# meyer-lab/cmtf-pls

Hardware: AMD Instinct MI355X
Metric: nipals_iters_per_sec (higher is better)
Workload: dtype f32

## Files before the change

cmtf_pls_amd/_lib.py:

```python
from __future__ import annotations

import ctypes
import os
from ctypes import c_char_p, c_double, c_int, c_int64, c_size_t, c_uint32, c_uint64, c_void_p

_HERE = os.path.dirname(os.path.abspath(__file__))
LIB_PATH = os.environ.get("CMTFPLS_LIB") or os.path.join(_HERE, "lib", "libcmtfpls.so")

_P = c_void_p

class XcovBlock(ctypes.Structure):
    _fields_ = [("S", _P), ("S2", _P), ("colcnt", _P), ("n_samples", c_double), ("order", c_int), ("A", c_int), ("B", c_int),
                ("n_squarings", c_int), ("Z", _P), ("wA", _P), ("wB", _P), ("info", _P)]


class KfoldState(ctypes.Structure):
    _fields_ = [("I", c_int), ("A", c_int), ("B", c_int), ("M", c_int), ("K", c_int), ("R", c_int)] + [
        (name, _P) for name in ("fold_of", "S", "mean", "Yk", "Gy", "WA", "WB", "Q", "Wa", "Wb", "T", "Gt", "coef", "Rm", "tm",
                                "Tout", "vec", "n_iter", "status", "part")]


class CvCoupledBlock(ctypes.Structure):
    _fields_ = [("X", _P), ("order", c_int), ("A", c_int), ("B", c_int)]


class LooCoupledBlock(ctypes.Structure):
    _fields_ = [("X", _P), ("colsum", _P), ("order", c_int), ("A", c_int), ("B", c_int)]


SIGNATURES = {
    "cmtfpls_xcov_iterate_blocks_f64": (c_int, [ctypes.POINTER(XcovBlock), c_int, c_int, _P, _P, _P, _P, _P, c_int, _P, c_size_t, _P]),
    "cmtfpls_abi_version": (c_int, []),
    "cmtfpls_last_error": (c_char_p, []),
    "cmtfpls_clear_error": (c_int, []),
    "cmtfpls_status_to_host": (c_int, [_P, _P, c_size_t, _P, _P]),
    "cmtfpls_colstats_workspace_bytes": (c_size_t, [c_int64, c_int64]),
    "cmtfpls_colstats_f32": (c_int, [_P, c_int64, c_int64, _P, _P, _P, c_size_t, _P]),
    "cmtfpls_colstats_f64": (c_int, [_P, c_int64, c_int64, _P, _P, _P, c_size_t, _P]),
    "cmtfpls_sweep_partials": (c_int, []),
    "cmtfpls_center_f32": (c_int, [_P, c_int64, c_int64, _P, _P, _P, _P]),
    "cmtfpls_center_f64": (c_int, [_P, c_int64, c_int64, _P, _P, _P, _P]),
    "cmtfpls_mode0_contract_workspace_bytes": (c_size_t, [c_int64, c_int64]),
    "cmtfpls_mode0_contract_f32": (c_int, [_P, c_int64, c_int64, _P, _P, c_int, _P, c_size_t, _P]),
    "cmtfpls_mode0_contract_f64": (c_int, [_P, c_int64, c_int64, _P, _P, c_int, _P, c_size_t, _P]),
    "cmtfpls_mode0_contract_yq_f32": (c_int, [_P, c_int64, c_int64, _P, c_int, c_int, _P, _P, c_int, _P, c_size_t, _P]),
    "cmtfpls_mode0_contract_yq_f64": (c_int, [_P, c_int64, c_int64, _P, c_int, c_int, _P, _P, c_int, _P, c_size_t, _P]),
    "cmtfpls_colscale_f64": (c_int, [_P, c_int64, _P, c_double, _P]),
    "cmtfpls_rank1_workspace_bytes": (c_size_t, [c_int, c_int]),
    "cmtfpls_rank1_score_f64": (c_int, [_P, c_int, c_int, _P, _P, _P, c_int, _P, c_int, _P, _P, c_size_t, _P]),
    "cmtfpls_rank1_f64": (c_int, [_P, c_int, c_int, _P, _P, _P, _P, c_int, _P, c_size_t, _P]),
    "cmtfpls_rank1_launches_f64": (c_int, [_P, c_int, c_int, _P, _P, _P, _P, c_int, _P, c_size_t, _P]),
    "cmtfpls_rank1_chain_enable": (None, [c_int]),
    "cmtfpls_rank1_chain_enabled": (c_int, []),
    "cmtfpls_normalize_f64": (c_int, [_P, c_int64, _P, _P]),
    "cmtfpls_rank1_tensor_workspace_bytes": (c_size_t, [_P, c_int]),
    "cmtfpls_rank1_tensor_f64": (c_int, [_P, _P, c_int, c_double, _P, c_int, _P, c_int, _P, c_size_t, _P]),
    "cmtfpls_kron_f64": (c_int, [_P, c_int, _P, c_int, _P, _P]),
    "cmtfpls_xcov_workspace_bytes": (c_size_t, [c_int64, c_int64, c_int]),
    "cmtfpls_xcov_f32": (c_int, [_P, c_int64, c_int64, _P, c_int, c_int, _P, c_int, _P, c_size_t, _P]),
    "cmtfpls_xcov_f64": (c_int, [_P, c_int64, c_int64, _P, c_int, c_int, _P, c_int, _P, c_size_t, _P]),
    "cmtfpls_xcov_bf16": (c_int, [_P, c_int64, c_int64, _P, c_int, c_int, _P, c_int, _P, c_size_t, _P]),
    "cmtfpls_xcov_f16": (c_int, [_P, c_int64, c_int64, _P, c_int, c_int, _P, c_int, _P, c_size_t, _P]),
    "cmtfpls_quadform_f64": (c_int, [_P, c_int, _P, _P, _P, _P]),
    "cmtfpls_xcov_iterate_f64": (c_int, [_P, c_int, c_int, c_int, _P, _P, _P, _P, _P, c_int, _P, _P, _P, c_int, _P, c_size_t, _P, c_size_t, _P]),
    "cmtfpls_s_downdate_f64": (c_int, [_P, c_int, c_int, c_int, _P, _P, _P, _P, _P, _P]),
    "cmtfpls_project_rows_f32": (c_int, [_P, c_int64, c_int, c_int, c_int, _P, _P, _P, _P, c_int, _P]),
    "cmtfpls_project_rows_f64": (c_int, [_P, c_int64, c_int, c_int, c_int, _P, _P, _P, _P, c_int, _P]),
    "cmtfpls_project_rows2_f32": (c_int, [_P, c_int, c_int, _P, _P, _P, _P, c_int, c_int, _P, _P, _P, c_int64, c_int, _P, c_int, _P]),
    "cmtfpls_project_rows2_f64": (c_int, [_P, c_int, c_int, _P, _P, _P, _P, c_int, c_int, _P, _P, _P, c_int64, c_int, _P, c_int, _P]),
    "cmtfpls_project_rows_idx_f32": (c_int, [_P, _P, c_int64, c_int, c_int, c_int, _P, _P, _P, _P, c_int, _P]),
    "cmtfpls_project_rows_idx_f64": (c_int, [_P, _P, c_int64, c_int, c_int, c_int, _P, _P, _P, _P, c_int, _P]),
    "cmtfpls_project_rows2_idx_f32": (c_int, [_P, c_int, c_int, _P, _P, _P, _P, c_int, c_int, _P, _P, _P, _P, c_int64, c_int, _P, c_int, _P]),
    "cmtfpls_project_rows2_idx_f64": (c_int, [_P, c_int, c_int, _P, _P, _P, _P, c_int, c_int, _P, _P, _P, _P, c_int64, c_int, _P, c_int, _P]),
    "cmtfpls_allreduce_sum_f64": (c_int, [_P, _P, c_size_t, _P]),
    "cmtfpls_allreduce_sum_f32": (c_int, [_P, _P, c_size_t, _P]),
    "cmtfpls_axpy_scalar_f64": (c_int, [_P, c_int64, _P, _P, _P]),
    "cmtfpls_xcov_deflate_f32": (c_int, [_P, c_int64, c_int, c_int, _P, c_int, c_int, _P, _P, _P, _P, _P, _P, c_size_t, _P]),
    "cmtfpls_xcov_deflate_f64": (c_int, [_P, c_int64, c_int, c_int, _P, c_int, c_int, _P, _P, _P, _P, _P, _P, c_size_t, _P]),
    "cmtfpls_xcov_stats_workspace_bytes": (c_size_t, [c_int64, c_int64, c_int]),
    "cmtfpls_xcov_stats_f32": (c_int, [_P, c_int64, c_int64, _P, c_int, c_int, _P, _P, _P, c_size_t, _P]),
    "cmtfpls_xcov_stats_f64": (c_int, [_P, c_int64, c_int64, _P, c_int, c_int, _P, _P, _P, c_size_t, _P]),
    "cmtfpls_xcov_stats_bf16": (c_int, [_P, c_int64, c_int64, _P, c_int, c_int, _P, _P, _P, c_size_t, _P]),
    "cmtfpls_xcov_stats_f16": (c_int, [_P, c_int64, c_int64, _P, c_int, c_int, _P, _P, _P, c_size_t, _P]),
    "cmtfpls_xcov_ssq_workspace_bytes": (c_size_t, [c_int64, c_int64, c_int]),
    "cmtfpls_xcov_ssq_f32": (c_int, [_P, c_int64, c_int64, _P, c_int, c_int, _P, _P, _P, _P, c_size_t, _P]),
    "cmtfpls_xcov_ssq_f64": (c_int, [_P, c_int64, c_int64, _P, c_int, c_int, _P, _P, _P, _P, c_size_t, _P]),
    "cmtfpls_score_contract_workspace_bytes": (c_size_t, [c_int64, c_int64]),
    "cmtfpls_score_contract_f32": (c_int, [_P, c_int64, c_int, c_int, _P, _P, _P, _P, _P, c_double, _P, _P, _P, _P, c_size_t, _P]),
    "cmtfpls_score_contract_f64": (c_int, [_P, c_int64, c_int, c_int, _P, _P, _P, _P, _P, c_double, _P, _P, _P, _P, c_size_t, _P]),
    "cmtfpls_score_contract_bf16": (c_int, [_P, c_int64, c_int, c_int, _P, _P, _P, _P, _P, c_double, _P, _P, _P, _P, c_size_t, _P]),
    "cmtfpls_score_contract_f16": (c_int, [_P, c_int64, c_int, c_int, _P, _P, _P, _P, _P, c_double, _P, _P, _P, _P, c_size_t, _P]),
    "cmtfpls_kr_axpy_f64": (c_int, [_P, c_int, c_int, _P, _P, c_int, c_int, _P, _P]),
    "cmtfpls_xcov_f32_mixed": (c_int, [_P, c_int64, c_int64, _P, c_int, c_int, _P, c_int, _P, c_size_t, _P]),
    "cmtfpls_mttkrp_f32_mixed": (c_int, [_P, c_int64, c_int, c_int, _P, _P, c_int, _P, c_int, _P]),
    "cmtfpls_mttkrp_f32": (c_int, [_P, c_int64, c_int, c_int, _P, _P, c_int, _P, c_int, _P]),
    "cmtfpls_mttkrp_f64": (c_int, [_P, c_int64, c_int, c_int, _P, _P, c_int, _P, c_int, _P]),
    "cmtfpls_mttkrp_bf16": (c_int, [_P, c_int64, c_int, c_int, _P, _P, c_int, _P, c_int, _P]),
    "cmtfpls_mttkrp_f16": (c_int, [_P, c_int64, c_int, c_int, _P, _P, c_int, _P, c_int, _P]),
    "cmtfpls_score_f32": (c_int, [_P, c_int64, c_int, c_int, _P, _P, _P, _P, _P]),
    "cmtfpls_score_f64": (c_int, [_P, c_int64, c_int, c_int, _P, _P, _P, _P, _P]),
    "cmtfpls_score_s_f64": (c_int, [_P, c_int, c_int, c_int, _P, _P, _P, _P]),
    "cmtfpls_deflate_contract_workspace_bytes": (c_size_t, [c_int64, c_int64]),
    "cmtfpls_deflate_contract_yq_f32": (c_int, [_P, c_int64, c_int, c_int, _P, _P, _P, _P, c_int, c_int, _P, _P, c_int, _P, _P, c_size_t, _P]),
    "cmtfpls_deflate_contract_yq_f64": (c_int, [_P, c_int64, c_int, c_int, _P, _P, _P, _P, c_int, c_int, _P, _P, c_int, _P, _P, c_size_t, _P]),
    "cmtfpls_score_gram_f32": (c_int, [_P, c_int64, c_int, c_int, _P, _P, _P, _P, _P, c_int, c_int, _P, _P]),
    "cmtfpls_score_gram_f64": (c_int, [_P, c_int64, c_int, c_int, _P, _P, _P, _P, _P, c_int, c_int, _P, _P]),
    "cmtfpls_q_update_f64": (c_int, [_P, c_int, c_int, _P, c_int, _P, _P, _P, _P]),
    "cmtfpls_deflate_f32": (c_int, [_P, c_int64, c_int, c_int, _P, _P, _P, _P, _P]),
    "cmtfpls_deflate_f64": (c_int, [_P, c_int64, c_int, c_int, _P, _P, _P, _P, _P]),
    "cmtfpls_score_deflate_f32": (c_int, [_P, c_int64, c_int, c_int, _P, _P, _P, _P, _P, _P]),
    "cmtfpls_score_deflate_f64": (c_int, [_P, c_int64, c_int, c_int, _P, _P, _P, _P, _P, _P]),
    "cmtfpls_sweep_form": (c_int, [c_char_p, c_int, c_int64, c_int, c_int, c_int, c_int, c_int, c_char_p, c_size_t]),
    "cmtfpls_sweep_form_list": (c_int, [c_char_p, c_int, c_char_p, c_size_t]),
    "cmtfpls_small_workspace_bytes": (c_size_t, []),
    "cmtfpls_gram_tn_f64": (c_int, [_P, c_int, c_int, _P, c_int, c_int, c_int64, _P, _P, c_size_t, _P]),
    "cmtfpls_rowdot_f64": (c_int, [_P, c_int, c_int, c_int64, _P, _P, _P, _P, _P, c_size_t, _P]),
    "cmtfpls_scores_mean_f64": (c_int, [_P, c_int, c_int64, _P, _P]),
    "cmtfpls_y_deflate_f64": (c_int, [_P, c_int, c_int, c_int64, _P, c_int, c_int, _P, _P, _P, _P, c_size_t, _P]),
    "cmtfpls_sum_f64": (c_int, [_P, c_int64, _P, _P]),
    "cmtfpls_normal_solve_f64": (c_int, [_P, _P, c_int, _P, c_int, _P]),
    "cmtfpls_normal_solve_workspace_bytes": (c_size_t, [c_int]),
    "cmtfpls_normal_solve_ws_f64": (c_int, [_P, _P, c_int, _P, c_int, _P, c_size_t, _P]),
    "cmtfpls_unit_upper_solve_rows_f64": (c_int, [_P, c_int64, c_int, c_int, _P, _P, _P, _P]),
    "cmtfpls_kr_gram_row_f64": (c_int, [_P, c_int, c_int, c_int, _P, c_int, _P]),
    "cmtfpls_kr_gram_f64": (c_int, [_P, c_int, c_int, _P, c_int, c_double, _P]),
    "cmtfpls_khatri_rao_f64": (c_int, [_P, c_int, _P, c_int, c_int, _P, _P]),
    "cmtfpls_predict_rows_f64": (c_int, [_P, c_int64, c_int, c_int, _P, c_int, _P, _P, c_int, _P]),
    "cmtfpls_recon_f32": (c_int, [_P, c_int64, c_int, c_int, _P, _P, c_int, c_int, _P, _P, _P]),
    "cmtfpls_recon_f64": (c_int, [_P, c_int64, c_int, c_int, _P, _P, c_int, c_int, _P, _P, _P]),
    "cmtfpls_recon_r2_workspace_bytes": (c_size_t, [c_int64, c_int64]),
    "cmtfpls_recon_r2_f32": (c_int, [_P, _P, c_int64, c_int, c_int, _P, _P, c_int, c_int, _P, _P, _P, c_size_t, _P]),
    "cmtfpls_recon_r2_f64": (c_int, [_P, _P, c_int64, c_int, c_int, _P, _P, c_int, c_int, _P, _P, _P, c_size_t, _P]),
    "cmtfpls_recon_r2_bf16": (c_int, [_P, _P, c_int64, c_int, c_int, _P, _P, c_int, c_int, _P, _P, _P, c_size_t, _P]),
    "cmtfpls_recon_r2_f16": (c_int, [_P, _P, c_int64, c_int, c_int, _P, _P, c_int, c_int, _P, _P, _P, c_size_t, _P]),
    "cmtfpls_resid_rows_workspace_bytes": (c_size_t, [c_int64, c_int64]),
    "cmtfpls_resid_rows_f32": (c_int, [_P, _P, c_int64, c_int, c_int, _P, _P, c_int, c_int, _P, _P, _P, _P, c_size_t, _P]),
    "cmtfpls_resid_rows_f64": (c_int, [_P, _P, c_int64, c_int, c_int, _P, _P, c_int, c_int, _P, _P, _P, _P, c_size_t, _P]),
    "cmtfpls_resid_rows_bf16": (c_int, [_P, _P, c_int64, c_int, c_int, _P, _P, c_int, c_int, _P, _P, _P, _P, c_size_t, _P]),
    "cmtfpls_resid_rows_f16": (c_int, [_P, _P, c_int64, c_int, c_int, _P, _P, c_int, c_int, _P, _P, _P, _P, c_size_t, _P]),
    "cmtfpls_contrib_rows_f32": (c_int, [_P, c_int64, _P, c_int, _P, c_int, c_int, _P, _P, c_int, c_int, _P, _P, c_int64, _P, _P, _P, _P, _P]),
    "cmtfpls_contrib_rows_f64": (c_int, [_P, c_int64, _P, c_int, _P, c_int, c_int, _P, _P, c_int, c_int, _P, _P, c_int64, _P, _P, _P, _P, _P]),
    "cmtfpls_contrib_rows_bf16": (c_int, [_P, c_int64, _P, c_int, _P, c_int, c_int, _P, _P, c_int, c_int, _P, _P, c_int64, _P, _P, _P, _P, _P]),
    "cmtfpls_contrib_rows_f16": (c_int, [_P, c_int64, _P, c_int, _P, c_int, c_int, _P, _P, c_int, c_int, _P, _P, c_int64, _P, _P, _P, _P, _P]),
    "cmtfpls_selectivity_cols_workspace_bytes": (c_size_t, [c_int64, c_int64, c_int]),
    "cmtfpls_selectivity_cols_f32": (c_int, [_P, c_int64, c_int64, _P, c_int, c_int, _P, c_int, _P, _P, _P, _P, _P, c_size_t, _P]),
    "cmtfpls_selectivity_cols_f64": (c_int, [_P, c_int64, c_int64, _P, c_int, c_int, _P, c_int, _P, _P, _P, _P, _P, c_size_t, _P]),
    "cmtfpls_selectivity_cols_bf16": (c_int, [_P, c_int64, c_int64, _P, c_int, c_int, _P, c_int, _P, _P, _P, _P, _P, c_size_t, _P]),
    "cmtfpls_selectivity_cols_f16": (c_int, [_P, c_int64, c_int64, _P, c_int, c_int, _P, c_int, _P, _P, _P, _P, _P, c_size_t, _P]),
    "cmtfpls_holdout_mask_workspace_bytes": (c_size_t, [c_int64]),
    "cmtfpls_holdout_mask_f32": (c_int, [_P, _P, c_int64, c_double, c_uint64, c_uint32, c_uint64, _P, _P, c_size_t, _P]),
    "cmtfpls_holdout_mask_f64": (c_int, [_P, _P, c_int64, c_double, c_uint64, c_uint32, c_uint64, _P, _P, c_size_t, _P]),
    "cmtfpls_heldout_resid_workspace_bytes": (c_size_t, [c_int64, c_int64, c_int]),
    "cmtfpls_heldout_resid_f32": (c_int, [_P, c_int64, c_int, c_int, _P, c_int, c_int, _P, _P, _P, c_double, c_uint64, c_uint32, c_uint64,
                                          _P, _P, c_size_t, _P]),
    "cmtfpls_heldout_resid_f64": (c_int, [_P, c_int64, c_int, c_int, _P, c_int, c_int, _P, _P, _P, c_double, c_uint64, c_uint32, c_uint64,
                                          _P, _P, c_size_t, _P]),
    "cmtfpls_impute_workspace_bytes": (c_size_t, [c_int64, c_int64]),
    "cmtfpls_impute_f32": (c_int, [_P, _P, c_int64, c_int, c_int, _P, c_int, c_int, _P, _P, _P, _P, _P, c_size_t, _P]),
    "cmtfpls_impute_f64": (c_int, [_P, _P, c_int64, c_int, c_int, _P, c_int, c_int, _P, _P, _P, _P, _P, c_size_t, _P]),
    "cmtfpls_loo_fold_workspace_bytes": (c_size_t, [c_int, c_int, c_int, c_int, c_int]),
    "cmtfpls_loo_tpls_f64": (c_int, [_P, _P, _P, _P, c_int, c_int, c_int, c_int, c_int, c_double, c_int, c_int, c_int, _P, _P, _P, c_size_t, _P]),
    "cmtfpls_loo_xcov_fold_workspace_bytes": (c_size_t, [c_int, c_int, c_int, c_int, c_int]),
    "cmtfpls_kfold_xcov_workspace_bytes": (c_size_t, [c_int64, c_int64, c_int, c_int]),
    "cmtfpls_kfold_xcov_f32": (c_int, [_P, c_int64, c_int, c_int, _P, c_int, _P, _P, c_int, _P, _P, _P, _P, _P, c_size_t, _P]),
    "cmtfpls_kfold_xcov_f64": (c_int, [_P, c_int64, c_int, c_int, _P, c_int, _P, _P, c_int, _P, _P, _P, _P, _P, c_size_t, _P]),
    "cmtfpls_kfold_xcov_bf16": (c_int, [_P, c_int64, c_int, c_int, _P, c_int, _P, _P, c_int, _P, _P, _P, _P, _P, c_size_t, _P]),
    "cmtfpls_kfold_xcov_f16": (c_int, [_P, c_int64, c_int, c_int, _P, c_int, _P, _P, c_int, _P, _P, _P, _P, _P, c_size_t, _P]),
    "cmtfpls_kfold_row_tiles": (c_int, [c_int64]),
    "cmtfpls_kfold_part_stride": (c_int, []),
    "cmtfpls_kfold_inner_workspace_bytes": (c_size_t, [c_int, c_int, c_int]),
    "cmtfpls_kfold_inner_f64": (c_int, [ctypes.POINTER(KfoldState), c_int, c_double, c_int, _P, c_size_t, _P]),
    "cmtfpls_kfold_inner_tensor_workspace_bytes": (c_size_t, [c_int, c_int, c_int, c_int]),
    "cmtfpls_kfold_inner_tensor_lds_bytes": (c_size_t, [c_int, c_int, c_int, c_int]),
    "cmtfpls_kfold_inner_tensor_f64": (c_int, [ctypes.POINTER(KfoldState), _P, c_int, c_int, c_int, c_int, c_double, c_int, _P, _P, _P,
                                       c_size_t, _P]),
    "cmtfpls_kfold_epilogue_f64": (c_int, [ctypes.POINTER(KfoldState), c_int, c_int, _P, _P]),
    "cmtfpls_kfold_inner_coupled_workspace_bytes": (c_size_t, [ctypes.POINTER(KfoldState), c_int]),
    "cmtfpls_kfold_inner_coupled_f64": (c_int, [ctypes.POINTER(KfoldState), c_int, c_int, c_double, c_int, _P, c_size_t, _P]),
    "cmtfpls_kfold_inner_coupled_tensor_workspace_bytes": (c_size_t, [ctypes.POINTER(KfoldState), c_int, ctypes.POINTER(c_int)]),
    "cmtfpls_kfold_inner_coupled_tensor_lds_bytes": (c_size_t, [ctypes.POINTER(KfoldState), c_int, ctypes.POINTER(c_int)]),
    "cmtfpls_kfold_inner_coupled_tensor_f64": (c_int, [ctypes.POINTER(KfoldState), c_int, ctypes.POINTER(c_int), _P, c_int, c_int, c_double,
                                                       c_int, _P, _P, _P, c_size_t, _P]),
    "cmtfpls_kfold_combine_scores_f64": (c_int, [_P, c_int, c_int64, _P, _P]),
    "cmtfpls_kfold_wide_xcov_workspace_bytes": (c_size_t, [c_int64, c_int64, c_int, c_int]),
    "cmtfpls_kfold_wide_xcov_f32": (c_int, [_P, c_int64, c_int, c_int, _P, c_int, _P, _P, c_int, _P, _P, _P, _P, _P, c_size_t, _P]),
    "cmtfpls_kfold_wide_xcov_f64": (c_int, [_P, c_int64, c_int, c_int, _P, c_int, _P, _P, c_int, _P, _P, _P, _P, _P, c_size_t, _P]),
    "cmtfpls_kfold_wide_xcov_bf16": (c_int, [_P, c_int64, c_int, c_int, _P, c_int, _P, _P, c_int, _P, _P, _P, _P, _P, c_size_t, _P]),
    "cmtfpls_kfold_wide_xcov_f16": (c_int, [_P, c_int64, c_int, c_int, _P, c_int, _P, _P, c_int, _P, _P, _P, _P, _P, c_size_t, _P]),
    "cmtfpls_kfold_inner_grouped_f64": (c_int, [ctypes.POINTER(KfoldState), _P, c_int, c_int, c_double, c_int, _P, c_size_t, _P]),
    "cmtfpls_kfold_inner_coupled_grouped_f64": (c_int, [ctypes.POINTER(KfoldState), c_int, _P, c_int, c_int, c_double, c_int, _P, c_size_t,
                                                        _P]),
    "cmtfpls_kfold_epilogue_grouped_f64": (c_int, [ctypes.POINTER(KfoldState), _P, c_int, c_int, c_int, _P, _P]),
    "cmtfpls_kfold_epilogue_splits_f64": (c_int, [ctypes.POINTER(KfoldState), c_int, c_int, c_int, _P, _P]),
    "cmtfpls_kfold_weighted_xcov_workspace_bytes": (c_size_t, [c_int64, c_int64, c_int, c_int]),
    "cmtfpls_kfold_weighted_xcov_f32": (c_int, [_P, c_int64, c_int, c_int, _P, c_int, c_int, _P, _P, _P, _P, c_size_t, _P]),
    "cmtfpls_kfold_weighted_xcov_f64": (c_int, [_P, c_int64, c_int, c_int, _P, c_int, c_int, _P, _P, _P, _P, c_size_t, _P]),
    "cmtfpls_kfold_weighted_xcov_bf16": (c_int, [_P, c_int64, c_int, c_int, _P, c_int, c_int, _P, _P, _P, _P, c_size_t, _P]),
    "cmtfpls_kfold_weighted_xcov_f16": (c_int, [_P, c_int64, c_int, c_int, _P, c_int, c_int, _P, _P, _P, _P, c_size_t, _P]),
    "cmtfpls_kfold_epilogue_weighted_f64": (c_int, [ctypes.POINTER(KfoldState), c_int, c_int, _P, _P]),
    "cmtfpls_press_rows_workspace_bytes": (c_size_t, [c_int, c_int64, c_int, c_int]),
    "cmtfpls_press_rows_f64": (c_int, [_P, _P, _P, _P, _P, _P, c_int, c_int64, c_int, c_int, _P, _P, _P, c_size_t, _P]),
    "cmtfpls_loo_xcov_f64": (c_int, [_P, _P, _P, _P, c_int, c_int, c_int, c_int, c_int, c_double, c_int, c_int, c_int, _P, _P, _P, c_size_t, _P]),
    "cmtfpls_loo_xcov_tensor_fold_workspace_bytes": (c_size_t, [c_int, c_int, c_int, c_int, c_int, c_int]),
    "cmtfpls_loo_xcov_tensor_lds_bytes": (c_size_t, [c_int, c_int, c_int, c_int, c_int]),
    "cmtfpls_loo_xcov_tensor_f64": (c_int, [_P, _P, _P, _P, c_int, c_int, c_int, c_int, c_int, c_int, c_double, c_int, c_int, c_int, _P, _P, _P,
                                            c_size_t, _P]),
    "cmtfpls_loo_xcov_coupled_fold_workspace_bytes": (c_size_t, [ctypes.POINTER(LooCoupledBlock), c_int, c_int, c_int, c_int]),
    "cmtfpls_loo_xcov_coupled_lds_bytes": (c_size_t, [ctypes.POINTER(LooCoupledBlock), c_int, c_int, c_int, c_int]),
    "cmtfpls_loo_xcov_coupled_f64": (c_int, [ctypes.POINTER(LooCoupledBlock), c_int, _P, _P, c_int, c_int, c_int, c_double, c_int, c_int, c_int,
                                             _P, _P, _P, c_size_t, _P]),
    "cmtfpls_loo_xcov_coupled_tensor_fold_workspace_bytes": (c_size_t, [ctypes.POINTER(LooCoupledBlock), c_int, ctypes.POINTER(c_int), c_int,
                                                                       c_int, c_int]),
    "cmtfpls_loo_xcov_coupled_tensor_lds_bytes": (c_size_t, [ctypes.POINTER(LooCoupledBlock), c_int, ctypes.POINTER(c_int), c_int, c_int,
                                                            c_int]),
    "cmtfpls_loo_xcov_coupled_tensor_f64": (c_int, [ctypes.POINTER(LooCoupledBlock), c_int, ctypes.POINTER(c_int), _P, _P, c_int, c_int, c_int,
                                                    c_double, c_int, c_int, c_int, _P, _P, _P, c_size_t, _P]),
    "cmtfpls_cv_masked_fold_workspace_bytes": (c_size_t, [c_int, c_int, c_int, c_int, c_int]),
    "cmtfpls_cv_masked_f64": (c_int, [_P, _P, _P, c_int, _P, _P, _P, c_int, c_int, c_int, c_int, c_int, c_double, c_int, c_int,
                                      c_int, _P, _P, _P, _P, _P, c_size_t, _P]),
    "cmtfpls_cv_masked_model_workspace_bytes": (c_size_t, [c_int, c_int, c_int, c_int, c_int]),
    "cmtfpls_cv_masked_models_f64": (c_int, [_P, _P, _P, _P, c_int, c_int, c_int, c_int, c_int, c_int, c_double, c_int, c_int, c_int]
                                     + [_P] * 8 + [_P, c_size_t, _P]),
    "cmtfpls_cv_masked_tensor_fold_workspace_bytes": (c_size_t, [c_int] * 6),
    "cmtfpls_cv_masked_tensor_lds_bytes": (c_size_t, [c_int] * 6),
    "cmtfpls_cv_masked_tensor_f64": (c_int, [_P, _P, _P, c_int, _P, _P, _P, c_int, c_int, c_int, c_int, c_int, c_int, c_double, c_int,
                                             c_int, c_int, _P, _P, _P, _P, _P, c_size_t, _P]),
    "cmtfpls_cv_masked_tensor_model_workspace_bytes": (c_size_t, [c_int] * 6),
    "cmtfpls_cv_masked_tensor_models_f64": (c_int, [_P, _P, _P, _P, c_int, c_int, c_int, c_int, c_int, c_int, c_int, c_double, c_int,
                                                    c_int, c_int] + [_P] * 9 + [_P, c_size_t, _P]),
    "cmtfpls_cv_masked_coupled_workspace_bytes": (c_size_t, [ctypes.POINTER(CvCoupledBlock), c_int, c_int, c_int, c_int]),
    "cmtfpls_cv_masked_coupled_lds_bytes": (c_size_t, [ctypes.POINTER(CvCoupledBlock), c_int, c_int, c_int, c_int]),
    "cmtfpls_cv_masked_coupled_f64": (c_int, [ctypes.POINTER(CvCoupledBlock), c_int, _P, _P, _P, c_int, c_int, c_int, c_int, c_double,
                                              c_int, c_int, c_int] + [_P] * 8 + [_P, c_size_t, _P]),
    "cmtfpls_cv_masked_coupled_tensor_workspace_bytes": (c_size_t, [ctypes.POINTER(CvCoupledBlock), c_int, _P, c_int, c_int, c_int]),
    "cmtfpls_cv_masked_coupled_tensor_lds_bytes": (c_size_t, [ctypes.POINTER(CvCoupledBlock), c_int, _P, c_int, c_int, c_int]),
    "cmtfpls_cv_masked_coupled_tensor_f64": (c_int, [ctypes.POINTER(CvCoupledBlock), c_int, _P, _P, _P, _P, c_int, c_int, c_int, c_int,
                                                     c_double, c_int, c_int, c_int] + [_P] * 10 + [_P, c_size_t, _P]),
    "cmtfpls_fit_small_workspace_bytes": (c_size_t, [c_int, c_int, c_int, c_int]),
    "cmtfpls_fit_small_f64": (c_int, [_P, _P, c_int, c_int, c_int, c_int, c_int, c_double, c_int] + [_P] * 11 + [_P, c_size_t, _P]),
    "cmtfpls_add_noise_f32": (c_int, [_P, c_int64, c_double, c_uint64, c_uint64, c_double, _P]),
    "cmtfpls_add_noise_f64": (c_int, [_P, c_int64, c_double, c_uint64, c_uint64, c_double, _P]),
    "cmtfpls_ceiling_max_blocks": (c_int, []),
    "cmtfpls_ceiling_read": (c_int, [_P, c_size_t, c_int64, c_int, _P, c_int, _P]),
    "cmtfpls_ceiling_rmw": (c_int, [_P, c_size_t, c_int64, c_int, c_int, _P]),
    "cmtfpls_ceiling_copy": (c_int, [_P, _P, c_size_t, c_int64, c_int, c_int, _P]),
}

_lib = None


class CmtfplsError(RuntimeError):
    pass


def load():
    global _lib
    if _lib is not None:
        return _lib
    if not os.path.exists(LIB_PATH):
        raise CmtfplsError(
            f"{LIB_PATH} not found: build the HIP extension first (python -c 'import __graft_entry__ as g; g.build()'). "
            "cmtf_pls_amd has no CPU fallback."
        )
    lib = ctypes.CDLL(LIB_PATH)
    for name, (res, args) in SIGNATURES.items():
        fn = getattr(lib, name)
        fn.restype = res
        fn.argtypes = args
    _lib = lib
    return lib


# ... 5 lines not shown
```

cmtf_pls_amd/backend.py:

```python
from __future__ import annotations

import ctypes
from typing import Optional, Tuple

import torch

from . import _lib
from .storage import HALF_DTYPES, HALF_ENTRIES, SUFFIX, entry_name

_HALF_ENTRIES = tuple(dict.fromkeys(e for group in HALF_ENTRIES.values() for e in group))


def _ptr(t: Optional[torch.Tensor]):
    return None if t is None else t.data_ptr()


def _int_pairs(pairs):
    flat = [int(v) for p in pairs for v in p]
    return (ctypes.c_int * len(flat))(*flat)


def _scratch(nbytes: int, device) -> torch.Tensor:
    return torch.empty(max(int(nbytes), 256), dtype=torch.uint8, device=device)

# ... 152 lines not shown
              info: Optional[torch.Tensor] = None, n_squarings: Optional[int] = None, launches: bool = False) -> None:
        ws = self._workspace("rank1", self.lib.cmtfpls_rank1_workspace_bytes(A, B))
        fn = self.lib.cmtfpls_rank1_launches_f64 if launches else self.lib.cmtfpls_rank1_f64
        _lib.check(fn(_ptr(Z), A, B, _ptr(wA), _ptr(wB), None, _ptr(info), int(n_squarings or self.rank1_squarings),
                      _ptr(ws), ws.numel(), self._stream()), "rank1")

    def rank1_chain_gave_up(self) -> None:
        self.lib.cmtfpls_rank1_chain_enable(0)
        self.rank1_chain_side = 0

    def rank1_tensor(self, Z: torch.Tensor, dims, tol: float, factors: torch.Tensor,
                     info: Optional[torch.Tensor] = None, n_squarings: Optional[int] = None) -> None:
        arr = (ctypes.c_int * len(dims))(*[int(d) for d in dims])
        ws = self._workspace("rank1t", self.lib.cmtfpls_rank1_tensor_workspace_bytes(arr, len(dims)))
        _lib.check(self.lib.cmtfpls_rank1_tensor_f64(_ptr(Z), arr, len(dims), float(tol), _ptr(factors), factors.stride(0), _ptr(info),
                                                     int(n_squarings or self.rank1_squarings), _ptr(ws), ws.numel(), self._stream()),
                   "rank1_tensor")

    def kron(self, a: torch.Tensor, b: torch.Tensor, out: torch.Tensor) -> torch.Tensor:
        _lib.check(self.lib.cmtfpls_kron_f64(_ptr(a), a.numel(), _ptr(b), b.numel(), _ptr(out), self._stream()), "kron")
        return out

    def normalize(self, v: torch.Tensor) -> None:
        _lib.check(self.lib.cmtfpls_normalize_f64(_ptr(v), v.numel(), None, self._stream()), "normalize")

    def xcov(self, X2: torch.Tensor, Y: torch.Tensor, masked: bool, out: Optional[torch.Tensor] = None,
             mixed: bool = False) -> Optional[torch.Tensor]:
        I, P = X2.shape
        M = Y.shape[1]
        fn = self._read_fn("xcov", X2, mixed)
        if fn is None:
            return None
        ws = self._workspace("contract", self.lib.cmtfpls_xcov_workspace_bytes(I, P, M))
        S = out if out is not None else self.empty(M, P)
        _lib.check(fn(_ptr(X2), I, P, _ptr(Y), Y.stride(0), M, _ptr(S), int(masked), _ptr(ws), ws.numel(), self._stream()), "xcov")
        return S

    def xcov_deflate(self, X2: torch.Tensor, A: int, B: int, Y: torch.Tensor, t: torch.Tensor, wA: torch.Tensor, wB: torch.Tensor,
                     out: torch.Tensor) -> Optional[torch.Tensor]:
        I, P = X2.shape
        M = Y.shape[1]
        if M > 64 or P % 4 != 0 or P != A * B:
            return None
        ws = self._workspace("contract", self.lib.cmtfpls_xcov_ssq_workspace_bytes(I, P, M))
        ssq = self.empty(1)
        rc = self._fn("xcov_deflate", X2)(_ptr(X2), I, A, B, _ptr(Y), Y.stride(0), M, _ptr(t), _ptr(wA), _ptr(wB), _ptr(out), _ptr(ssq),
                                          _ptr(ws), ws.numel(), self._stream())
        return self._form(rc, "xcov_deflate", ssq)

    def rank1_score(self, Z: torch.Tensor, A: int, B: int, wA: torch.Tensor, wB: torch.Tensor, S: torch.Tensor, tq: torch.Tensor,
                    info: Optional[torch.Tensor] = None, n_squarings: Optional[int] = None) -> torch.Tensor:
        M = S.shape[0]
        assert S.is_contiguous() and S.shape[1] == A * B and tq.numel() >= M
        ws = self._workspace("rank1", self.lib.cmtfpls_rank1_workspace_bytes(A, B))
        _lib.check(self.lib.cmtfpls_rank1_score_f64(_ptr(Z), A, B, _ptr(wA), _ptr(wB), _ptr(info),
                                                    int(n_squarings if n_squarings is not None else self.rank1_squarings),
                                                    _ptr(S), M, _ptr(tq), _ptr(ws), ws.numel(), self._stream()), "rank1_score")
        return tq

    def xcov_ssq(self, X2: torch.Tensor, Y: torch.Tensor, mean: torch.Tensor, out: torch.Tensor):
        I, P = X2.shape
        M = Y.shape[1]
        ws = self._workspace("contract", self.lib.cmtfpls_xcov_ssq_workspace_bytes(I, P, M))
        ssq = self.empty(1)
        assert mean.is_contiguous() and mean.numel() == P and mean.dtype == torch.float64
        _lib.check(self._fn("xcov_ssq", X2)(_ptr(X2), I, P, _ptr(Y), Y.stride(0), M, _ptr(out), _ptr(mean), _ptr(ssq), _ptr(ws), ws.numel(),
                                            self._stream()), "xcov_ssq")
        return out, ssq

    def xcov_stats(self, X2: torch.Tensor, Y: torch.Tensor, out: torch.Tensor):
        I, P = X2.shape
        M = Y.shape[1]
        fn = self._read_fn("xcov_stats", X2) if M <= 64 and X2.is_contiguous() else None
        if fn is None:
            return None
        ws = self._workspace("contract", self.lib.cmtfpls_xcov_stats_workspace_bytes(I, P, M))
        stats = self.empty(2 * P)
        rc = fn(_ptr(X2), I, P, _ptr(Y), Y.stride(0), M, _ptr(out), _ptr(stats), _ptr(ws), ws.numel(), self._stream())
        return self._form(rc, "xcov_stats", (out, stats))

    def status_snapshot(self, status: torch.Tensor, slot: int, slots: Optional[dict] = None):
        slots = self._status_slots if slots is None else slots
        ent = slots.get((slot, status.numel()))
        if ent is None:
            host, ev = torch.empty(status.numel(), dtype=torch.float64, pin_memory=True), torch.cuda.Event()
            ev.record(torch.cuda.current_stream(self.device))
            ent = slots[(slot, status.numel())] = (host, ev, host.numpy(), host.data_ptr(), ev.cuda_event, status.numel() * 8)
        rc = self.lib.cmtfpls_status_to_host(status.data_ptr(), ent[3], ent[5], ent[4], self._stream())
        if rc:
            _lib.check(rc, "status_to_host")
        return ent

    def status_wait(self, token) -> "np.ndarray":
        token[1].synchronize()
        return token[2]

    def xcov_iterate_plan(self, S: torch.Tensor, A: int, B: int, q_cur: torch.Tensor, Z: torch.Tensor, wA: torch.Tensor,
                          wB: torch.Tensor, status: torch.Tensor, q_new: torch.Tensor, G: torch.Tensor):
        M, P = S.shape
        wc = self._workspace("contract", self.lib.cmtfpls_mode0_contract_workspace_bytes(M, P))
        wr = self._workspace("rank1", self.lib.cmtfpls_rank1_workspace_bytes(A, B))
        keep = (S, q_cur, Z, wA, wB, status, q_new, G, wc, wr)
        fn = self.lib.cmtfpls_xcov_iterate_f64
        head = (_ptr(S), M, A, B, _ptr(q_cur), _ptr(Z), _ptr(wA), _ptr(wB), status[1:3].data_ptr())
        tail = (_ptr(wc), wc.numel(), _ptr(wr), wr.numel())
        qn, Gp, du2 = _ptr(q_new), _ptr(G), status[0:1].data_ptr()
        stream = self._stream

        def enqueue(n_squarings: int, first: bool, _keep=keep) -> None:
            rc = fn(*head, n_squarings, qn, Gp, du2, 1 if first else 0, *tail, stream())
            if rc:
                _lib.check(rc, "xcov_iterate")
        return enqueue

    def xcov_iterate(self, S: torch.Tensor, A: int, B: int, q_cur: torch.Tensor, Z: torch.Tensor, wA: torch.Tensor,
                     wB: torch.Tensor, info: torch.Tensor, n_squarings: int, q_new: torch.Tensor, G: torch.Tensor,
                     du2: torch.Tensor, first: bool) -> None:
        M, P = S.shape
        wc = self._workspace("contract", self.lib.cmtfpls_mode0_contract_workspace_bytes(M, P))
        wr = self._workspace("rank1", self.lib.cmtfpls_rank1_workspace_bytes(A, B))
        _lib.check(self.lib.cmtfpls_xcov_iterate_f64(_ptr(S), M, A, B, _ptr(q_cur), _ptr(Z), _ptr(wA), _ptr(wB), _ptr(info),
                                                     int(n_squarings), _ptr(q_new), _ptr(G), _ptr(du2), int(first),
                                                     _ptr(wc), wc.numel(), _ptr(wr), wr.numel(), self._stream()), "xcov_iterate")

    def xcov_blocks_plan(self, blocks, M: int, q_cur: torch.Tensor, tq: torch.Tensor, q_new: torch.Tensor, G: torch.Tensor,
                         status: torch.Tensor):
        nb = len(blocks)
        if M > 64 or any(b["order"] not in (2, 3) for b in blocks) or tq.numel() != nb * M or not tq.is_contiguous():
            return None
        arr = (_lib.XcovBlock * nb)()
        need = 256
        for i, b in enumerate(blocks):
            for name in ("S", "S2", "colcnt", "Z", "wA", "wB"):
                t = b.get(name)
                assert t is None or (t.is_contiguous() and t.dtype == torch.float64 and t.device == self.device), name
                setattr(arr[i], name, _ptr(t))
            arr[i].n_samples, arr[i].order, arr[i].A, arr[i].B = float(b["n_samples"]), int(b["order"]), int(b["A"]), int(b["B"])
            arr[i].info = status[1 + 2 * i: 3 + 2 * i].data_ptr()
            if b["order"] == 3:
                need = max(need, self.lib.cmtfpls_rank1_workspace_bytes(b["A"], b["B"]))
        wr = self._workspace("rank1", need)
        keep = (blocks, q_cur, tq, q_new, G, status, wr, arr)
        fn, stream = self.lib.cmtfpls_xcov_iterate_blocks_f64, self._stream
        args = (nb, M, _ptr(q_cur), _ptr(tq), _ptr(q_new), _ptr(G), status[0:1].data_ptr())
        tail = (_ptr(wr), wr.numel())

        def enqueue(n_squarings, first: bool, _keep=keep) -> None:
            for i in range(nb):
                arr[i].n_squarings = int(n_squarings[i])
            rc = fn(arr, *args, 1 if first else 0, *tail, stream())
            if rc:
                _lib.check(rc, "xcov_iterate_blocks")
        return enqueue

    def s_downdate(self, S: torch.Tensor, A: int, B: int, ya: torch.Tensor, wA: torch.Tensor, wB: torch.Tensor,
                   q: torch.Tensor, v: torch.Tensor) -> None:
        assert S.is_contiguous() and S.shape[1] == A * B
        _lib.check(self.lib.cmtfpls_s_downdate_f64(_ptr(S), S.shape[0], A, B, _ptr(ya), _ptr(wA), _ptr(wB), _ptr(q), _ptr(v),
                                                   self._stream()), "s_downdate")

    def kr_axpy(self, v: torch.Tensor, A: int, B: int, WA: torch.Tensor, WB: torch.Tensor, k: int, coef: torch.Tensor) -> torch.Tensor:
        assert WA.is_contiguous() and WB.is_contiguous() and WA.shape[1] == WB.shape[1] and coef.numel() >= k
        _lib.check(self.lib.cmtfpls_kr_axpy_f64(_ptr(v), A, B, _ptr(WA), _ptr(WB), WA.shape[1], int(k), _ptr(coef), self._stream()), "kr_axpy")
        return v

    def axpy_scalar(self, y: torch.Tensor, a: torch.Tensor, x: Optional[torch.Tensor] = None) -> torch.Tensor:
        assert y.is_contiguous() and y.dtype == torch.float64 and a.numel() >= 1 and (x is None or (x.is_contiguous() and x.numel() == y.numel()))
        _lib.check(self.lib.cmtfpls_axpy_scalar_f64(_ptr(y), y.numel(), _ptr(a), _ptr(x), self._stream()), "axpy_scalar")
        return y

    def total(self, v: torch.Tensor) -> torch.Tensor:
        assert v.is_contiguous() and v.dtype == torch.float64
        return self._close_partials(v)

    def quadform(self, G: torch.Tensor, q: torch.Tensor, q_old: torch.Tensor, out: torch.Tensor) -> torch.Tensor:
        _lib.check(self.lib.cmtfpls_quadform_f64(_ptr(G), G.shape[0], _ptr(q), _ptr(q_old), _ptr(out), self._stream()), "quadform")
        return out

    def mttkrp(self, X2: torch.Tensor, A: int, B: int, WA: torch.Tensor, WB: torch.Tensor, out: torch.Tensor,
               mixed: bool = False) -> Optional[torch.Tensor]:
        R = WA.shape[1]
        assert WA.is_contiguous() and WB.is_contiguous() and out.stride(1) == 1
        fn = self._read_fn("mttkrp", X2, mixed)
        if fn is None:
            return None
        rc = fn(_ptr(X2), X2.shape[0], A, B, _ptr(WA), _ptr(WB), R, _ptr(out), out.stride(0), self._stream())
        return self._form(rc, "mttkrp", out)

    def score(self, X2, A, B, wA, wB, rowcnt, out) -> torch.Tensor:
        _lib.check(self._fn("score", X2)(_ptr(X2), X2.shape[0], A, B, _ptr(wA), _ptr(wB), _ptr(rowcnt), _ptr(out), self._stream()), "score")
        return out

    def score_s(self, S, A, B, wA, wB, out) -> torch.Tensor:
        assert S.dtype == torch.float64 and S.is_contiguous()
        _lib.check(self.lib.cmtfpls_score_s_f64(_ptr(S), S.shape[0], A, B, _ptr(wA), _ptr(wB), _ptr(out), self._stream()), "score_s")
        return out

    def score_contract(self, X2, A, B, wA, wB, shift, t, Z, sub_own=None, add_other=None, alpha: float = 1.0,
                       csum: Optional[torch.Tensor] = None) -> Optional[torch.Tensor]:
        I, P = X2.shape
        fn = self._read_fn("score_contract", X2) if X2.is_contiguous() and P == A * B else None
        if fn is None:
            return None
        for v in (sub_own, add_other):
            assert v is None or (v.is_contiguous() and v.numel() == I and v.dtype == torch.float64)
        nbytes = self.lib.cmtfpls_score_contract_workspace_bytes(I, P)
        ws = self._workspace("score_contract", max(nbytes, 256))
        rc = fn(_ptr(X2), I, A, B, _ptr(wA), _ptr(wB), _ptr(shift), _ptr(sub_own), _ptr(add_other), float(alpha),
                                            _ptr(t), _ptr(Z), _ptr(csum), _ptr(ws), ws.numel(), self._stream())
        return self._form(rc, "score_contract", Z)

    def score_gram(self, X2, A, B, wA, wB, rowcnt, out, Y: torch.Tensor, qpart: torch.Tensor) -> Optional[torch.Tensor]:
        assert qpart.numel() >= self.n_partials * Y.shape[1] and qpart.is_contiguous()
        rc = self._fn("score_gram", X2)(_ptr(X2), X2.shape[0], A, B, _ptr(wA), _ptr(wB), _ptr(rowcnt), _ptr(out),
                                        _ptr(Y), Y.stride(0), Y.shape[1], _ptr(qpart), self._stream())
        return self._form(rc, "score_gram", out)

    def q_update(self, q: torch.Tensor, qpart: Optional[torch.Tensor] = None, normalize: bool = True,
                 G: Optional[torch.Tensor] = None, q_prev: Optional[torch.Tensor] = None,
                 du2: Optional[torch.Tensor] = None, nparts: Optional[int] = None) -> None:
        M = q.numel()
        nrows = (nparts or self.n_partials) if qpart is not None else 0
        assert qpart is None or (qpart.is_contiguous() and qpart.numel() >= nrows * M)
        _lib.check(self.lib.cmtfpls_q_update_f64(_ptr(qpart), nrows, M, _ptr(q), int(normalize),
                                                 _ptr(G), _ptr(q_prev), _ptr(du2), self._stream()), "q_update")

    def deflate(self, X2, A, B, t, wA, wB) -> torch.Tensor:
        part = self.empty(self.n_partials)
        _lib.check(self._fn("deflate", X2)(_ptr(X2), X2.shape[0], A, B, _ptr(t), _ptr(wA), _ptr(wB), _ptr(part), self._stream()), "deflate")
        return self._close_partials(part)

    def deflate_contract_yq(self, X2, A, B, t, wA, wB, Y: torch.Tensor, q: torch.Tensor, masked: bool,
                            out: torch.Tensor) -> Optional[torch.Tensor]:
        I, P = X2.shape
        ws = self._workspace("deflate_contract", self.lib.cmtfpls_deflate_contract_workspace_bytes(I, P))
        ssq = self.empty(1)
        rc = self._fn("deflate_contract_yq", X2)(_ptr(X2), I, A, B, _ptr(t), _ptr(wA), _ptr(wB), _ptr(Y), Y.stride(0), Y.shape[1],
                                                 _ptr(q), _ptr(out), int(masked), _ptr(ssq), _ptr(ws), ws.numel(), self._stream())
        return self._form(rc, "deflate_contract_yq", ssq)

    def score_deflate(self, X2, A, B, wA, wB, rowcnt, out) -> Optional[torch.Tensor]:
        part = self.empty(self.n_partials)
        rc = self._fn("score_deflate", X2)(_ptr(X2), X2.shape[0], A, B, _ptr(wA), _ptr(wB), _ptr(rowcnt), _ptr(out), _ptr(part), self._stream())
        if self._form(rc, "score_deflate") is None:
            return None
        return self._close_partials(part)

    def gram_tn(self, A: torch.Tensor, B: torch.Tensor, out: Optional[torch.Tensor] = None) -> torch.Tensor:
        if A.dim() == 1:
            A = A.unsqueeze(1)
        if B.dim() == 1:
            B = B.unsqueeze(1)
        assert A.stride(1) == 1 and B.stride(1) == 1 and A.shape[0] == B.shape[0]
        a, b = A.shape[1], B.shape[1]
        ws = self._workspace("small", self.lib.cmtfpls_small_workspace_bytes())
        C = out if out is not None else self.empty(a, b)
        assert C.numel() == a * b and C.is_contiguous()
        _lib.check(self.lib.cmtfpls_gram_tn_f64(_ptr(A), A.stride(0), a, _ptr(B), B.stride(0), b, A.shape[0], _ptr(C),
                                                _ptr(ws), ws.numel(), self._stream()), "gram_tn")
        return C

    def rowdot(self, Y: torch.Tensor, q: torch.Tensor, u_out: torch.Tensor, u_old: Optional[torch.Tensor],
               du2: Optional[torch.Tensor] = None) -> Optional[torch.Tensor]:
        ws = self._workspace("small", self.lib.cmtfpls_small_workspace_bytes())
        if u_old is not None and du2 is None:
            du2 = self.empty(1)
        _lib.check(self.lib.cmtfpls_rowdot_f64(_ptr(Y), Y.stride(0), Y.shape[1], Y.shape[0], _ptr(q), _ptr(u_out), _ptr(u_old),
                                               _ptr(du2) if u_old is not None else None,
                                               _ptr(ws), ws.numel(), self._stream()), "rowdot")
        return du2 if u_old is not None else None

    def normal_solve(self, G: torch.Tensor, g: torch.Tensor, out: Optional[torch.Tensor] = None) -> torch.Tensor:
        k = G.shape[0]
        assert G.is_contiguous() and G.shape == (k, k) and g.numel() == k
        b = out if out is not None else self.empty(k)
        if k <= 64:
            _lib.check(self.lib.cmtfpls_normal_solve_f64(_ptr(G), _ptr(g), k, _ptr(b), 1, self._stream()), "normal_solve")
        else:
            ws = self._workspace("normal_solve", self.lib.cmtfpls_normal_solve_workspace_bytes(k))
            _lib.check(self.lib.cmtfpls_normal_solve_ws_f64(_ptr(G), _ptr(g), k, _ptr(b), 1, _ptr(ws), ws.numel(), self._stream()),
                       "normal_solve")
        return b

    def unit_upper_solve_rows(self, M: torch.Tensor, U: torch.Tensor, shift: Optional[torch.Tensor] = None,
                              nan_flag: Optional[torch.Tensor] = None) -> torch.Tensor:
        I, R = M.shape
        assert M.stride(1) == 1 and U.is_contiguous() and U.shape == (R, R)
        assert shift is None or (shift.is_contiguous() and shift.numel() == R and shift.dtype == torch.float64)
        assert nan_flag is None or nan_flag.dtype == torch.int32
        _lib.check(self.lib.cmtfpls_unit_upper_solve_rows_f64(_ptr(M), I, M.stride(0), R, _ptr(U), _ptr(shift), _ptr(nan_flag),
                                                              self._stream()), "unit_upper_solve_rows")
        return M

    def kr_gram_row(self, L: torch.Tensor, a: int, g: torch.Tensor, first: bool) -> torch.Tensor:
        assert L.is_contiguous() and g.is_contiguous() and g.numel() >= a
        _lib.check(self.lib.cmtfpls_kr_gram_row_f64(_ptr(L), L.shape[0], L.shape[1], int(a), _ptr(g), int(first), self._stream()), "kr_gram_row")
        return g

    def kr_gram(self, L: torch.Tensor, G: torch.Tensor, first: bool) -> torch.Tensor:
        n, R = L.shape
        assert L.is_contiguous() and G.is_contiguous() and G.numel() == R * R
        _lib.check(self.lib.cmtfpls_kr_gram_f64(_ptr(L), n, R, _ptr(G), int(first), 1.0, self._stream()), "kr_gram")
        return G

    def khatri_rao(self, Am: torch.Tensor, Bm: torch.Tensor) -> torch.Tensor:
        na, R = Am.shape
# ... 489 lines not shown
```

cmtf_pls_amd/csrc/small.hip:

```cpp
#include "common.hpp"

namespace cmtfpls {

void launch_reduce_rows(const double* part, int nrows, int64_t P, double* out, hipStream_t st);

constexpr int kSmallBlocks = 128;
constexpr int kMaxGramDim = 64;
constexpr size_t kSmallWsBytes = (size_t)kSmallBlocks * kMaxGramDim * kMaxGramDim * sizeof(double);

__global__ __launch_bounds__(256) void gram_tn_kernel(const double* __restrict__ A, int lda, int a,
                                                     const double* __restrict__ B, int ldb, int b,
                                                     int64_t I, double* __restrict__ part, int TR) {
  extern __shared__ double lds[];
  double* As = lds;
  double* Bs = lds + TR * a;
  const int ab = a * b;
  const int64_t rows_per = (I + gridDim.x - 1) / gridDim.x;
  const int64_t r0 = (int64_t)blockIdx.x * rows_per;
  const int64_t r1 = (r0 + rows_per < I) ? r0 + rows_per : I;
  double acc[16];
#pragma unroll
  for (int s = 0; s < 16; ++s) acc[s] = 0.0;
  for (int64_t rb = r0; rb < r1; rb += TR) {
    const int nr = (int)((r1 - rb < TR) ? r1 - rb : TR);
    if (lda == a) {
      for (int idx = threadIdx.x; idx < nr * a; idx += 256) As[idx] = A[rb * a + idx];
    } else {
      for (int idx = threadIdx.x; idx < nr * a; idx += 256) As[idx] = A[(rb + idx / a) * lda + idx % a];
    }
    if (ldb == b) {
      for (int idx = threadIdx.x; idx < nr * b; idx += 256) Bs[idx] = B[rb * b + idx];
    } else {
      for (int idx = threadIdx.x; idx < nr * b; idx += 256) Bs[idx] = B[(rb + idx / b) * ldb + idx % b];
    }
    __syncthreads();
#pragma unroll
    for (int s = 0; s < 16; ++s) {
      const int o = threadIdx.x + s * 256;
      if (o < ab) {
        const int p = o / b, q = o % b;
        double v = acc[s];
        for (int r = 0; r < nr; ++r) v = fma(As[r * a + p], Bs[r * b + q], v);
        acc[s] = v;
      }
    }
    __syncthreads();
  }
#pragma unroll
  for (int s = 0; s < 16; ++s) {
    const int o = threadIdx.x + s * 256;
    if (o < ab) part[(int64_t)blockIdx.x * ab + o] = acc[s];
  }
}

__global__ __launch_bounds__(256) void reduce_block_kernel(const double* __restrict__ part, int nblk, int ac, int bc,
                                                          double* __restrict__ C, int ldc) {
  const int o = blockIdx.x * 4 + (threadIdx.x >> 6);
  const int lane = threadIdx.x & 63;
  if (o >= ac * bc) return;
  double s = 0.0;
  for (int r = lane; r < nblk; r += 64) s += part[(int64_t)r * ac * bc + o];
  s = wave_sum(s);
  if (lane == 0) C[(int64_t)(o / bc) * ldc + (o % bc)] = s;
}

__global__ __launch_bounds__(256) void gemv_t_kernel(const double* __restrict__ A, int lda, int a0, int ac,
                                                    const double* __restrict__ v, int ldv, int64_t I,
                                                    double* __restrict__ part, int a_total) {
  __shared__ double red[4][16];
  double acc[16];
#pragma unroll
  for (int e = 0; e < 16; ++e) acc[e] = 0.0;
  for (int64_t i = (int64_t)blockIdx.x * 256 + threadIdx.x; i < I; i += (int64_t)gridDim.x * 256) {
    const double vi = v[i * ldv];
    const double* ar = A + i * lda + a0;
#pragma unroll
    for (int e = 0; e < 16; ++e)
      if (e < ac) acc[e] = fma(ar[e], vi, acc[e]);
  }
  const int lane = threadIdx.x & 63, wv = threadIdx.x >> 6;
#pragma unroll
  for (int e = 0; e < 16; ++e) {
    const double w = wave_sum(acc[e]);
    if (lane == 0) red[wv][e] = w;
  }
  __syncthreads();
  if (threadIdx.x < ac) {
    const int e = threadIdx.x;
    part[(int64_t)blockIdx.x * a_total + a0 + e] = ((red[0][e] + red[1][e]) + red[2][e]) + red[3][e];
  }
}

__global__ __launch_bounds__(256) void rowdot_kernel(const double* __restrict__ Y, int ldy, int M, int64_t I,
                                                    const double* __restrict__ q, double* __restrict__ u,
                                                    const double* __restrict__ u_old, double* __restrict__ part) {
  __shared__ double red[16];
  double d2 = 0.0;
  for (int64_t i = (int64_t)blockIdx.x * 256 + threadIdx.x; i < I; i += (int64_t)gridDim.x * 256) {
    const double* yr = Y + i * ldy;
    double s = 0.0;
    for (int m = 0; m < M; ++m) s = fma(yr[m], q[m], s);
    if (u_old) { const double d = u_old[i] - s; d2 = fma(d, d, d2); }
    u[i] = s;
  }
  if (part) {
    const double s = block_sum(d2, red);
    if (threadIdx.x == 0) part[blockIdx.x] = s;
  }
}

__global__ __launch_bounds__(256) void y_deflate_kernel(double* __restrict__ Y, int ldy, int M, int64_t I,
                                                       const double* __restrict__ T, int ldt, int R,
                                                       const double* __restrict__ b, const double* __restrict__ q,
                                                       double* __restrict__ part) {
  __shared__ double red[16];
  double ssq = 0.0;
  for (int64_t i = (int64_t)blockIdx.x * 256 + threadIdx.x; i < I; i += (int64_t)gridDim.x * 256) {
    double s = 0.0;
    for (int r = 0; r < R; ++r) s = fma(T[i * ldt + r], b[r], s);
    double* yr = Y + i * ldy;
    for (int m = 0; m < M; ++m) {
      const double v = yr[m] - s * q[m];
      yr[m] = v;
      ssq = fma(v, v, ssq);
    }
  }
  const double s = block_sum(ssq, red);
  if (threadIdx.x == 0) part[blockIdx.x] = s;
}

__global__ __launch_bounds__(1024) void sum_kernel(const double* __restrict__ in, int64_t n, double* __restrict__ out) {
  __shared__ double red[16];
  double s = 0.0;
  for (int64_t i = threadIdx.x; i < n; i += 1024) s += in[i];
  s = block_sum(s, red);
  if (threadIdx.x == 0) out[0] = s;
}

__global__ __launch_bounds__(1024) void normalize_kernel(double* __restrict__ v, int64_t n, double* __restrict__ nrm) {
  __shared__ double red[16];
  double s = 0.0;
  for (int64_t i = threadIdx.x; i < n; i += 1024) s = fma(v[i], v[i], s);
  s = sqrt(block_sum(s, red));
  for (int64_t i = threadIdx.x; i < n; i += 1024) v[i] = v[i] / s;
  if (nrm && threadIdx.x == 0) nrm[0] = s;
}

__global__ __launch_bounds__(1024) void normalize_to_kernel(const double* __restrict__ in, double* __restrict__ out, int64_t n) {
  __shared__ double red[16];
  double s = 0.0;
  for (int64_t i = threadIdx.x; i < n; i += 1024) s = fma(in[i], in[i], s);
  s = sqrt(block_sum(s, red));
  for (int64_t i = threadIdx.x; i < n; i += 1024) out[i] = in[i] / s;
}

__global__ __launch_bounds__(1024) void s_vector_block_kernel(const double* __restrict__ S, const double* __restrict__ S2,
                                                            const double* __restrict__ colcnt, double n_samples, int M, int P,
                                                            const double* __restrict__ q, double* __restrict__ Z,
                                                            double* __restrict__ wB, double* __restrict__ tq) {
  extern __shared__ double wl[];
  __shared__ double red[16];
  const int lane = threadIdx.x & 63, wv = threadIdx.x >> 6;
  double ssq = 0.0;
  for (int c = threadIdx.x; c < P; c += 1024) {
    double z = 0.0;
#pragma unroll 8
    for (int m = 0; m < M; ++m) z = fma(q[m], S[(int64_t)m * P + c], z);
    if (colcnt) z = (colcnt[c] > 0.0) ? z / colcnt[c] * n_samples : 0.0;
    Z[c] = z;
    wl[c] = z;
    ssq = fma(z, z, ssq);
  }
  const double nrm = sqrt(block_sum(ssq, red));
  for (int c = threadIdx.x; c < P; c += 1024) {
    const double w = wl[c] / nrm;
    wl[c] = w;
    wB[c] = w;
  }
  __syncthreads();
  for (int m = wv; m < M; m += 16) {
    double acc = 0.0;
    for (int c = lane; c < P; c += 64) acc = fma(S2[(int64_t)m * P + c], wl[c], acc);
    acc = wave_sum(acc);
    if (lane == 0) tq[m] = acc;
  }
}

__global__ __launch_bounds__(1024) void q_update_kernel(const double* __restrict__ qpart, int nblk, int M,
                                                       double* __restrict__ q, int normalize,
                                                       const double* __restrict__ G, const double* __restrict__ q_prev,
                                                       double* __restrict__ du2) {
  __shared__ double part[64][17];
  __shared__ double qs[64];
  __shared__ double dq[64];
  __shared__ double red[16];
  const int tid = threadIdx.x, lane = tid & 63;
  const int Mp = (M <= 16) ? 16 : (M <= 32) ? 32 : 64;
  const int ngrp = 1024 / Mp;
  const int m = tid & (Mp - 1), grp = tid / Mp;
  double* pflat = &part[0][0];
  if (qpart) {
    double sacc = 0.0;
    const int msafe = (m < M) ? m : 0;
    for (int b0 = grp; b0 < nblk; b0 += 16 * ngrp) {
      double v[16];
#pragma unroll
      for (int k = 0; k < 16; ++k) {
        const int b = b0 + k * ngrp;
        v[k] = qpart[(int64_t)((b < nblk) ? b : nblk - 1) * M + msafe];
      }
#pragma unroll
      for (int k = 0; k < 16; ++k) sacc += (b0 + k * ngrp < nblk) ? v[k] : 0.0;
    }
    if (m >= M) sacc = 0.0;
    pflat[grp * (Mp + 1) + m] = sacc;
    __syncthreads();
    if (tid < M) {
      double tot = 0.0;
      for (int g = 0; g < ngrp; ++g) tot += pflat[g * (Mp + 1) + tid];
      qs[tid] = tot;
    }
  } else if (tid < M) {
    qs[tid] = q[tid];
  }
  __syncthreads();
  if (tid < 64) {
    double v = (lane < M) ? qs[lane] : 0.0;
    if (normalize) {
      const double nrm = sqrt(wave_sum(v * v));
      v = v / nrm;
    }
    if (lane < M) {
      q[lane] = v;
      if (G) dq[lane] = v - q_prev[lane];
    }
  }
  if (G) {
    __syncthreads();
    double sacc = 0.0;
    for (int idx = tid; idx < M * M; idx += 1024) {
      const int i = idx / M, j = idx - i * M;
      sacc = fma(dq[i] * G[idx], dq[j], sacc);
    }
    sacc = block_sum(sacc, red);
    if (tid == 0) du2[0] = sacc;
  }
}

__global__ __launch_bounds__(256) void s_downdate_kernel(double* __restrict__ S, int M, int64_t P, int B,
                                                        const double* __restrict__ ya, const double* __restrict__ wA,
                                                        const double* __restrict__ wB, const double* __restrict__ q,
                                                        const double* __restrict__ v) {
  const int64_t c = (int64_t)blockIdx.x * 256 + threadIdx.x;
  if (c >= P) return;
  const double w = wA[c / B] * wB[c % B];
  const double vc = v[c];
  for (int m = 0; m < M; ++m) {
    double sv = S[(int64_t)m * P + c];
    sv = fma(-ya[m], w, sv);
    sv = fma(-q[m], vc, sv);
    S[(int64_t)m * P + c] = sv;
  }
}

__global__ __launch_bounds__(256) void s_contract_kernel(const double* __restrict__ S, int M, int64_t P, const double* __restrict__ q,
                                                        double* __restrict__ Z) {
  const int64_t c = (int64_t)blockIdx.x * 256 + threadIdx.x;
  if (c >= P) return;
  double acc = 0.0;
#pragma unroll 8
  for (int m = 0; m < M; ++m) acc = fma(q[m], S[(int64_t)m * P + c], acc);
  Z[c] = acc;
}

__global__ __launch_bounds__(256) void axpy_scalar_kernel(double* __restrict__ y, int64_t n, const double* __restrict__ a,
                                                         const double* __restrict__ x) {
  const double av = a[0];
  for (int64_t i = (int64_t)blockIdx.x * 256 + threadIdx.x; i < n; i += (int64_t)gridDim.x * 256) y[i] = fma(-av, x ? x[i] : 1.0, y[i]);
}

__global__ __launch_bounds__(256) void kr_axpy_kernel(double* __restrict__ v, int64_t P, int B, const double* __restrict__ WA,
                                                     const double* __restrict__ WB, int ld, int k, const double* __restrict__ coef) {
  __shared__ double cs[64];
  for (int j = threadIdx.x; j < k; j += 256) cs[j] = coef[j];
  __syncthreads();
  const int64_t c = (int64_t)blockIdx.x * 256 + threadIdx.x;
  if (c >= P) return;
  const double* __restrict__ wa = WA + (c / B) * ld;
  const double* __restrict__ wb = WB + (c % B) * ld;
  double s = 0.0;
  for (int j = 0; j < k; ++j) s = fma(cs[j] * wa[j], wb[j], s);
  v[c] -= s;
}

__global__ __launch_bounds__(256) void colscale_kernel(double* __restrict__ Z, int64_t P, const double* __restrict__ cnt, double n_samples) {
  const int64_t c = (int64_t)blockIdx.x * 256 + threadIdx.x;
  if (c < P) Z[c] = (cnt[c] > 0.0) ? Z[c] / cnt[c] * n_samples : 0.0;
}

__global__ __launch_bounds__(256) void scores_mean_kernel(const double* __restrict__ Ts, int nb, int64_t I, double* __restrict__ out) {
  const int64_t i = (int64_t)blockIdx.x * 256 + threadIdx.x;
  if (i >= I) return;
  double s = Ts[i];
  for (int b = 1; b < nb; ++b) s += Ts[(int64_t)b * I + i];
  out[i] = s / (double)nb;
}

}

using namespace cmtfpls;

extern "C" {

size_t cmtfpls_small_workspace_bytes(void) { return kSmallWsBytes; }

int cmtfpls_gram_tn_f64(const double* A, int lda, int a, const double* B, int ldb, int b, int64_t I,
                        double* C, void* ws, size_t ws_bytes, void* stream) {
  if (!A || !B || !C || a <= 0 || b <= 0 || lda < a || ldb < b || I <= 0) {
    set_error("gram_tn: bad argument");
    return CMTFPLS_EINVAL;
  }
  if (!ws || ws_bytes < kSmallWsBytes) { set_error("gram_tn: workspace too small"); return CMTFPLS_EWORKSPACE; }
  hipStream_t st = (hipStream_t)stream;
  double* part = static_cast<double*>(ws);
  if (b == 1 && (size_t)kSmallBlocks * a * sizeof(double) <= kSmallWsBytes) {
    for (int a0 = 0; a0 < a; a0 += 16) {
      const int ac = (a - a0 < 16) ? a - a0 : 16;
      hipLaunchKernelGGL(gemv_t_kernel, dim3(kSmallBlocks), dim3(256), 0, st, A, lda, a0, ac, B, ldb, I, part, a);
    }
    hipLaunchKernelGGL(reduce_block_kernel, dim3((a + 3) / 4), dim3(256), 0, st, part, kSmallBlocks, a, 1, C, 1);
    return check_launch("gram_tn");
  }
  for (int a0 = 0; a0 < a; a0 += kMaxGramDim)
    for (int b0 = 0; b0 < b; b0 += kMaxGramDim) {
      const int ac = (a - a0 < kMaxGramDim) ? a - a0 : kMaxGramDim;
      const int bc = (b - b0 < kMaxGramDim) ? b - b0 : kMaxGramDim;
      const int tr = (ac + bc <= 32) ? 128 : (ac + bc <= 64) ? 64 : 32;
      const size_t lds = (size_t)tr * (ac + bc) * sizeof(double);
      hipLaunchKernelGGL(gram_tn_kernel, dim3(kSmallBlocks), dim3(256), lds, st, A + a0, lda, ac, B + b0, ldb, bc, I, part, tr);
      hipLaunchKernelGGL(reduce_block_kernel, dim3((ac * bc + 3) / 4), dim3(256), 0, st, part, kSmallBlocks, ac, bc,
                         C + (size_t)a0 * b + b0, b);
    }
  return check_launch("gram_tn");
}

int cmtfpls_rowdot_f64(const double* Y, int ldy, int M, int64_t I, const double* q, double* u,
                       const double* u_old, double* du2, void* ws, size_t ws_bytes, void* stream) {
  if (!Y || !q || !u || M <= 0 || ldy < M || I <= 0 || (u_old && !du2)) { set_error("rowdot: bad argument"); return CMTFPLS_EINVAL; }
  if (u_old && (!ws || ws_bytes < kSmallBlocks * sizeof(double))) { set_error("rowdot: workspace too small"); return CMTFPLS_EWORKSPACE; }
  hipStream_t st = (hipStream_t)stream;
  double* part = u_old ? static_cast<double*>(ws) : nullptr;
  hipLaunchKernelGGL(rowdot_kernel, dim3(kSmallBlocks), dim3(256), 0, st, Y, ldy, M, I, q, u, u_old, part);
  if (u_old) hipLaunchKernelGGL(sum_kernel, dim3(1), dim3(1024), 0, st, part, (int64_t)kSmallBlocks, du2);
  return check_launch("rowdot");
}

int cmtfpls_y_deflate_f64(double* Y, int ldy, int M, int64_t I, const double* T, int ldt, int R,
                          const double* b, const double* q, double* ssq, void* ws, size_t ws_bytes, void* stream) {
  if (!Y || !T || !b || !q || !ssq || M <= 0 || ldy < M || R <= 0 || ldt < R || I <= 0) { set_error("y_deflate: bad argument"); return CMTFPLS_EINVAL; }
  if (!ws || ws_bytes < kSmallBlocks * sizeof(double)) { set_error("y_deflate: workspace too small"); return CMTFPLS_EWORKSPACE; }
  hipStream_t st = (hipStream_t)stream;
  double* part = static_cast<double*>(ws);
  hipLaunchKernelGGL(y_deflate_kernel, dim3(kSmallBlocks), dim3(256), 0, st, Y, ldy, M, I, T, ldt, R, b, q, part);
  hipLaunchKernelGGL(sum_kernel, dim3(1), dim3(1024), 0, st, part, (int64_t)kSmallBlocks, ssq);
  return check_launch("y_deflate");
}

int cmtfpls_sum_f64(const double* in, int64_t n, double* out, void* stream) {
  if (!in || !out || n <= 0) { set_error("sum: bad argument"); return CMTFPLS_EINVAL; }
  hipLaunchKernelGGL(sum_kernel, dim3(1), dim3(1024), 0, (hipStream_t)stream, in, n, out);
  return check_launch("sum");
}

int cmtfpls_normalize_f64(double* v, int64_t n, double* nrm, void* stream) {
  if (!v || n <= 0) { set_error("normalize: bad argument"); return CMTFPLS_EINVAL; }
  hipLaunchKernelGGL(normalize_kernel, dim3(1), dim3(1024), 0, (hipStream_t)stream, v, n, nrm);
  return check_launch("normalize");
}

int cmtfpls_q_update_f64(const double* qpart, int nblk, int M, double* q, int normalize, const double* G, const double* q_prev,
                         double* du2, void* stream) {
  if (!q || M <= 0 || (qpart && nblk <= 0) || (G && (!q_prev || !du2))) { set_error("q_update: bad argument"); return CMTFPLS_EINVAL; }
  if (M > 64) { set_error("q_update: more than 64 responses; use gram_tn + normalize + rowdot"); return CMTFPLS_EUNSUPPORTED; }
  hipLaunchKernelGGL(q_update_kernel, dim3(1), dim3(1024), 0, (hipStream_t)stream, qpart, nblk, M, q, normalize, G, q_prev, du2);
  return check_launch("q_update");
}

int cmtfpls_s_downdate_f64(double* S, int M, int A, int B, const double* ya, const double* wA, const double* wB,
                           const double* q, const double* v, void* stream) {
  if (!S || !ya || !wA || !wB || !q || !v || M <= 0 || A <= 0 || B <= 0) { set_error("s_downdate: bad argument"); return CMTFPLS_EINVAL; }
  const int64_t P = (int64_t)A * B;
  hipLaunchKernelGGL(s_downdate_kernel, dim3((unsigned)((P + 255) / 256)), dim3(256), 0, (hipStream_t)stream, S, M, P, B, ya, wA, wB, q, v);
  return check_launch("s_downdate");
}

int cmtfpls_axpy_scalar_f64(double* y, int64_t n, const double* a, const double* x, void* stream) {
  if (!y || !a || n <= 0) { set_error("axpy_scalar: bad argument"); return CMTFPLS_EINVAL; }
  int64_t blocks = (n + 255) / 256;
  if (blocks > 1024) blocks = 1024;
  hipLaunchKernelGGL(axpy_scalar_kernel, dim3((unsigned)blocks), dim3(256), 0, (hipStream_t)stream, y, n, a, x);
  return check_launch("axpy_scalar");
}

int cmtfpls_kr_axpy_f64(double* v, int A, int B, const double* WA, const double* WB, int ld, int k, const double* coef, void* stream) {
  if (!v || !WA || !WB || !coef || A <= 0 || B <= 0 || k < 0 || ld < k) { set_error("kr_axpy: bad argument"); return CMTFPLS_EINVAL; }
  if (k > 64) { set_error("kr_axpy: more than 64 terms"); return CMTFPLS_EUNSUPPORTED; }
  if (k == 0) return CMTFPLS_OK;
  const int64_t P = (int64_t)A * B;
  hipLaunchKernelGGL(kr_axpy_kernel, dim3((unsigned)((P + 255) / 256)), dim3(256), 0, (hipStream_t)stream, v, P, B, WA, WB, ld, k, coef);
  return check_launch("kr_axpy");
}

int cmtfpls_xcov_iterate_f64(const double* S, int M, int A, int B, const double* q_cur, double* Z, double* wA, double* wB,
                             double* info, int n_squarings, double* q_new, const double* G, double* du2, int first,
                             void* ws_contract, size_t ws_contract_bytes, void* ws_rank1, size_t ws_rank1_bytes, void* stream) {
  if (!S || !q_cur || !Z || !wA || !wB || !q_new || !G || !du2 || M <= 0 || A <= 0 || B <= 0) {
    set_error("xcov_iterate: bad argument");
    return CMTFPLS_EINVAL;
  }
  if (M > 64) { set_error("xcov_iterate: more than 64 responses"); return CMTFPLS_EUNSUPPORTED; }
  const int64_t P = (int64_t)A * B;
  int rc = CMTFPLS_OK;
  if (first) {
    hipLaunchKernelGGL(s_contract_kernel, dim3((unsigned)((P + 255) / 256)), dim3(256), 0, (hipStream_t)stream, S, M, P, q_cur, Z);
    rc = check_launch("xcov_iterate: s_contract");
  }
  if (rc == CMTFPLS_OK) rc = cmtfpls_rank1_score_f64(Z, A, B, wA, wB, info, n_squarings, S, M, q_new, ws_rank1, ws_rank1_bytes, stream);
  if (rc == CMTFPLS_OK) rc = cmtfpls_q_update_f64(nullptr, 0, M, q_new, 1, G, q_cur, du2, stream);
  return rc;
}

int cmtfpls_xcov_iterate_blocks_f64(const cmtfpls_xcov_block* blocks, int nb, int M, const double* q_cur, double* tq, double* q_new,
                                    const double* G, double* du2, int first, void* ws_rank1, size_t ws_rank1_bytes, void* stream) {
  if (!blocks || nb <= 0 || !q_cur || !tq || !q_new || !G || !du2 || M <= 0) { set_error("xcov_iterate_blocks: bad argument"); return CMTFPLS_EINVAL; }
  if (M > 64) { set_error("xcov_iterate_blocks: more than 64 responses"); return CMTFPLS_EUNSUPPORTED; }
  hipStream_t st = (hipStream_t)stream;
  int rc = CMTFPLS_OK;
  for (int b = 0; b < nb && rc == CMTFPLS_OK; ++b) {
    const cmtfpls_xcov_block& k = blocks[b];
    if (!k.S || !k.Z || !k.wA || !k.wB || k.A <= 0 || k.B <= 0 || (k.order != 2 && k.order != 3) || (k.order == 2 && k.A != 1) ||
        (k.order == 3 && !k.info)) {
      set_error("xcov_iterate_blocks: bad block");
      return CMTFPLS_EINVAL;
    }
    const int64_t P = (int64_t)k.A * k.B;
// ... 40 lines not shown
```

cmtf_pls_amd/csrc/solve.hip:

```cpp
#include "common.hpp"

namespace cmtfpls {

constexpr int kSolveMax = 64;

__global__ __launch_bounds__(kSolveMax) void normal_solve_kernel(const double* __restrict__ G, const double* __restrict__ g, int k,
                                                                double* __restrict__ b, int incb) {
  __shared__ double A[kSolveMax][kSolveMax + 1];
  __shared__ double d[kSolveMax], y[kSolveMax];
  __shared__ int dep[kSolveMax];
  const int i = threadIdx.x;
  if (i < k) {
    const double gii = G[(int64_t)i * k + i];
    d[i] = (gii > 0.0 && isfinite(gii)) ? 1.0 / sqrt(gii) : 0.0;
    dep[i] = 0;
  }
  __syncthreads();
  if (i < k) {
    for (int j = 0; j < k; ++j) A[i][j] = G[(int64_t)i * k + j] * d[i] * d[j];
    y[i] = g[i] * d[i];
  }
  __syncthreads();
  const double tiny = (double)k * 2.220446049250313e-16;
  for (int c = 0; c < k; ++c) {
    const double piv = A[c][c];
    const bool ok = piv > tiny;
    __syncthreads();
    if (ok) {
      const double l = sqrt(piv);
      if (i == c) A[c][c] = l;
      if (i > c && i < k) A[i][c] = A[i][c] / l;
    } else {
      if (i == c) { A[c][c] = 1.0; dep[c] = 1; }
      if (i > c && i < k) A[i][c] = 0.0;
    }
    __syncthreads();
    if (ok && i > c && i < k) {
      const double lic = A[i][c];
      for (int j = c + 1; j <= i; ++j) A[i][j] -= lic * A[j][c];
    }
    __syncthreads();
  }
  if (i == 0) {
    for (int r = 0; r < k; ++r) {
      double s = y[r];
      for (int j = 0; j < r; ++j) s -= A[r][j] * y[j];
      y[r] = dep[r] ? 0.0 : s / A[r][r];
    }
    for (int r = k - 1; r >= 0; --r) {
      double s = y[r];
      for (int j = r + 1; j < k; ++j) s -= A[j][r] * y[j];
      y[r] = dep[r] ? 0.0 : s / A[r][r];
    }
  }
  __syncthreads();
  if (i < k) b[(int64_t)i * incb] = y[i] * d[i];
}

constexpr int kSolveBigMax = 1024;
__global__ __launch_bounds__(256) void normal_solve_big_kernel(const double* __restrict__ G, const double* __restrict__ g, int k,
                                                               double* __restrict__ b, int incb, double* __restrict__ Aw) {
  const int ld = k + 1;
  double* d = Aw + (size_t)k * ld;
  double* y = d + k;
  double* depf = y + k;
  __shared__ double s_piv;
  const int t = threadIdx.x;
  for (int i = t; i < k; i += 256) {
    const double gii = G[(int64_t)i * k + i];
    d[i] = (gii > 0.0 && isfinite(gii)) ? 1.0 / sqrt(gii) : 0.0;
    depf[i] = 0.0;
  }
  __syncthreads();
  for (int i = t; i < k; i += 256) {
    for (int j = 0; j < k; ++j) Aw[(size_t)i * ld + j] = G[(int64_t)i * k + j] * d[i] * d[j];
    y[i] = g[i] * d[i];
  }
  __syncthreads();
  const double tiny = (double)k * 2.220446049250313e-16;
  for (int c = 0; c < k; ++c) {
    if (t == 0) s_piv = Aw[(size_t)c * ld + c];
    __syncthreads();
    const double piv = s_piv;
    const bool ok = piv > tiny;
    const double l = ok ? sqrt(piv) : 1.0;
    for (int i = c + t; i < k; i += 256) {
      if (i == c) { Aw[(size_t)c * ld + c] = l; if (!ok) depf[c] = 1.0; }
      else Aw[(size_t)i * ld + c] = ok ? Aw[(size_t)i * ld + c] / l : 0.0;
    }
    __syncthreads();
    if (ok)
      for (int i = c + 1 + t; i < k; i += 256) {
        const double lic = Aw[(size_t)i * ld + c];
        for (int j = c + 1; j <= i; ++j) Aw[(size_t)i * ld + j] -= lic * Aw[(size_t)j * ld + c];
      }
    __syncthreads();
  }
  for (int r = 0; r < k; ++r) {
    if (t == 0) y[r] = (depf[r] != 0.0) ? 0.0 : y[r] / Aw[(size_t)r * ld + r];
    __syncthreads();
    const double yr = y[r];
    for (int j = r + 1 + t; j < k; j += 256) y[j] -= Aw[(size_t)j * ld + r] * yr;
    __syncthreads();
  }
  for (int r = k - 1; r >= 0; --r) {
    if (t == 0) y[r] = (depf[r] != 0.0) ? 0.0 : y[r] / Aw[(size_t)r * ld + r];
    __syncthreads();
    const double yr = y[r];
    for (int j = t; j < r; j += 256) y[j] -= Aw[(size_t)r * ld + j] * yr;
    __syncthreads();
  }
  for (int i = t; i < k; i += 256) b[(int64_t)i * incb] = y[i] * d[i];
}

__global__ __launch_bounds__(256) void unit_upper_solve_rows_kernel(double* __restrict__ Mx, int64_t I, int ld, int R,
                                                                   const double* __restrict__ U, const double* __restrict__ shift,
                                                                   int* __restrict__ nan_flag) {
  __shared__ double Us[kSolveMax * kSolveMax];
  __shared__ double sh[kSolveMax];
  for (int idx = threadIdx.x; idx < R * R; idx += 256) Us[idx] = U[idx];
  for (int idx = threadIdx.x; idx < R; idx += 256) sh[idx] = shift ? shift[idx] : 0.0;
  __syncthreads();
  const int64_t i = (int64_t)blockIdx.x * 256 + threadIdx.x;
  if (i >= I) return;
  double* row = Mx + i * ld;
  bool bad = false;
#pragma unroll 1
  for (int a = 0; a < R; ++a) {
    double s = row[a];
    bad |= (s != s);
    s -= sh[a];
    for (int j = 0; j < a; ++j) s -= row[j] * Us[j * R + a];
    row[a] = s;
  }
  if (bad && nan_flag) *nan_flag = 1;
}

__global__ __launch_bounds__(256) void kr_gram_kernel(const double* __restrict__ L, int n, int R, double* __restrict__ G,
                                                     int first, double scale) {
  for (int o = threadIdx.x; o < R * R; o += 256) {
    const int r = o / R, s = o % R;
    double acc = 0.0;
    for (int j = 0; j < n; ++j) acc = fma(L[(int64_t)j * R + r], L[(int64_t)j * R + s], acc);
    G[o] = (first ? 1.0 : G[o]) * scale * acc;
  }
}

__global__ __launch_bounds__(256) void kr_gram_row_kernel(const double* __restrict__ L, int n, int R, int a, double* __restrict__ g, int first) {
  for (int j = threadIdx.x; j < a; j += 256) {
    double acc = 0.0;
    int i = 0;
    for (; i + 16 <= n; i += 16) {
      double x[16], y[16];
#pragma unroll
      for (int u = 0; u < 16; ++u) {
        x[u] = L[(int64_t)(i + u) * R + j];
        y[u] = L[(int64_t)(i + u) * R + a];
      }
#pragma unroll
      for (int u = 0; u < 16; ++u) acc = fma(x[u], y[u], acc);
    }
    for (; i < n; ++i) acc = fma(L[(int64_t)i * R + j], L[(int64_t)i * R + a], acc);
    g[j] = (first ? 1.0 : g[j]) * acc;
  }
}

__global__ __launch_bounds__(256) void khatri_rao_kernel(const double* __restrict__ Am, int na, const double* __restrict__ Bm, int nb,
                                                        int R, double* __restrict__ out) {
  const int64_t idx = (int64_t)blockIdx.x * 256 + threadIdx.x;
  const int64_t tot = (int64_t)na * nb * R;
  if (idx >= tot) return;
  const int r = (int)(idx % R);
  const int64_t jk = idx / R;
  out[idx] = Am[(jk / nb) * R + r] * Bm[(jk % nb) * R + r];
}

__global__ __launch_bounds__(256) void predict_rows_kernel(const double* __restrict__ S, int lds_, int R, const double* __restrict__ Bm,
                                                          const double* __restrict__ mean, double* __restrict__ out, int ldo, int64_t I, int M) {
  extern __shared__ double sb[];
  for (int idx = threadIdx.x; idx < R * M; idx += 256) sb[idx] = Bm[idx];
  for (int idx = threadIdx.x; idx < M; idx += 256) sb[R * M + idx] = mean ? mean[idx] : 0.0;
  __syncthreads();
  const int64_t o = (int64_t)blockIdx.x * 256 + threadIdx.x;
  if (o >= I * M) return;
  const int64_t i = o / M;
  const int m = (int)(o % M);
  double acc = 0.0;
  for (int a = 0; a < R; ++a) acc = fma(S[i * lds_ + a], sb[a * M + m], acc);
  out[i * ldo + m] = acc + sb[R * M + m];
}

}

using namespace cmtfpls;

extern "C" {

int cmtfpls_normal_solve_f64(const double* G, const double* g, int k, double* b, int incb, void* stream) {
  if (!G || !g || !b || k <= 0 || incb <= 0) { set_error("normal_solve: bad argument"); return CMTFPLS_EINVAL; }
  if (k > kSolveMax) { set_error("normal_solve: more than 64 components; use cmtfpls_normal_solve_ws_f64"); return CMTFPLS_EUNSUPPORTED; }
  hipLaunchKernelGGL(normal_solve_kernel, dim3(1), dim3(kSolveMax), 0, (hipStream_t)stream, G, g, k, b, incb);
  return check_launch("normal_solve");
}

size_t cmtfpls_normal_solve_workspace_bytes(int k) {
  if (k <= kSolveMax || k > kSolveBigMax) return 0;
  return ((size_t)k * (k + 1) + 3 * (size_t)k) * sizeof(double);
}

int cmtfpls_normal_solve_ws_f64(const double* G, const double* g, int k, double* b, int incb, void* ws, size_t ws_bytes, void* stream) {
  if (k <= kSolveMax) return cmtfpls_normal_solve_f64(G, g, k, b, incb, stream);
  if (!G || !g || !b || incb <= 0) { set_error("normal_solve: bad argument"); return CMTFPLS_EINVAL; }
  if (k > kSolveBigMax) { set_error("normal_solve: more than 1024 components"); return CMTFPLS_EUNSUPPORTED; }
  if (!ws || ws_bytes < cmtfpls_normal_solve_workspace_bytes(k)) { set_error("normal_solve: workspace too small"); return CMTFPLS_EWORKSPACE; }
  hipLaunchKernelGGL(normal_solve_big_kernel, dim3(1), dim3(256), 0, (hipStream_t)stream, G, g, k, b, incb, static_cast<double*>(ws));
  return check_launch("normal_solve");
}

int cmtfpls_unit_upper_solve_rows_f64(double* Mx, int64_t I, int ld, int R, const double* U, const double* shift, int* nan_flag,
                                      void* stream) {
  if (!Mx || !U || I <= 0 || R <= 0 || ld < R) { set_error("unit_upper_solve_rows: bad argument"); return CMTFPLS_EINVAL; }
  if (R > kSolveMax) { set_error("unit_upper_solve_rows: more than 64 components"); return CMTFPLS_EUNSUPPORTED; }
  hipLaunchKernelGGL(unit_upper_solve_rows_kernel, dim3((unsigned)((I + 255) / 256)), dim3(256), 0, (hipStream_t)stream, Mx, I, ld, R, U,
                     shift, nan_flag);
  return check_launch("unit_upper_solve_rows");
}

int cmtfpls_kr_gram_f64(const double* L, int n, int R, double* G, int first, double scale, void* stream) {
  if (!L || !G || n <= 0 || R <= 0) { set_error("kr_gram: bad argument"); return CMTFPLS_EINVAL; }
  hipLaunchKernelGGL(kr_gram_kernel, dim3(1), dim3(256), 0, (hipStream_t)stream, L, n, R, G, first, scale);
  return check_launch("kr_gram");
}

int cmtfpls_kr_gram_row_f64(const double* L, int n, int R, int a, double* g, int first, void* stream) {
  if (!L || !g || n <= 0 || R <= 0 || a < 0 || a >= R) { set_error("kr_gram_row: bad argument"); return CMTFPLS_EINVAL; }
  if (a == 0) return CMTFPLS_OK;
  hipLaunchKernelGGL(kr_gram_row_kernel, dim3(1), dim3(256), 0, (hipStream_t)stream, L, n, R, a, g, first);
  return check_launch("kr_gram_row");
}

int cmtfpls_predict_rows_f64(const double* S, int64_t I, int lds_, int R, const double* Bm, int M, const double* mean, double* out, int ldo,
                             void* stream) {
  if (!S || !Bm || !out || I <= 0 || R <= 0 || M <= 0 || lds_ < R || ldo < M) { set_error("predict_rows: bad argument"); return CMTFPLS_EINVAL; }
  const size_t lds_bytes = ((size_t)R * M + M) * sizeof(double);
  if (lds_bytes > 64 * 1024) { set_error("predict_rows: coef_ Q^T does not fit the LDS"); return CMTFPLS_EUNSUPPORTED; }
  const int64_t tot = I * M;
  hipLaunchKernelGGL(predict_rows_kernel, dim3((unsigned)((tot + 255) / 256)), dim3(256), lds_bytes, (hipStream_t)stream, S, lds_, R, Bm, mean,
                     out, ldo, I, M);
  return check_launch("predict_rows");
}

int cmtfpls_khatri_rao_f64(const double* Am, int na, const double* Bm, int nb, int R, double* out, void* stream) {
  if (!Am || !Bm || !out || na <= 0 || nb <= 0 || R <= 0) { set_error("khatri_rao: bad argument"); return CMTFPLS_EINVAL; }
  const int64_t tot = (int64_t)na * nb * R;
  hipLaunchKernelGGL(khatri_rao_kernel, dim3((unsigned)((tot + 255) / 256)), dim3(256), 0, (hipStream_t)stream, Am, na, Bm, nb, R, out);
  return check_launch("khatri_rao");
}

}
```

cmtf_pls_amd/fitrun.py:

```python
from __future__ import annotations

import math
from typing import Dict, List, Optional

import numpy as np
import torch

from .fitrun_xcov import XcovMixin
from .state import BlockState, FitState, split_trailing, validate_limits
from .storage import HALF_DTYPES, HALF_ENTRIES, dtype_name, fallback_text, half_route


class FitRun(XcovMixin):

    def __init__(self, eng: NipalsEngine, Xs: List[torch.Tensor], Y: torch.Tensor, n_components: int, coupled: bool,
                 algorithm: str = "direct", owned: Optional[List[bool]] = None, allow_raw: bool = True):
        be, comm = eng.be, eng.comm
        Xs = list(Xs)
        owned = [True] * len(Xs) if owned is None else list(owned)
        if algorithm not in ("direct", "xcov"):
            raise ValueError("algorithm must be 'direct' or 'xcov'")
        self.algorithm_requested = self.algorithm = algorithm
        self.notes: List[str] = []
        validate_limits([tuple(X.shape) for X in Xs], n_components)
# ... 118 lines not shown
        self._z_ready = False
        self._fused = (algorithm == "direct" and M <= 64
                       and all(hasattr(be, f) for f in ("mode0_contract_yq", "score_gram", "q_update")))
        if self._fused:
            self.Gy = be.empty(M, M)
            self.qbuf = [be.zeros(M), be.zeros(M)]
            self.qpart = be.empty(len(self.blocks), int(be.n_partials) * M)
        elif algorithm == "direct" and comm.sharded:
            self.Gy = be.empty(M, M)
            self.q_prev = be.zeros(M)
        if algorithm == "xcov":
            nb = len(self.blocks)
            self._s_pair = 2 * M <= 64 and eng.opt.xcov_pair_build
            self.S, self.S2, self.S12 = [], [], []
            for blk in self.blocks:
                if blk.has_miss and self._s_pair:
                    both = be.empty(2 * M, blk.A * blk.B)
                    self.S12.append(both)
                    self.S.append(both[:M])
                    self.S2.append(both[M:])
                else:
                    self.S12.append(None)
                    pre = self._s_prebuilt.get(len(self.S))
                    self.S.append(pre if pre is not None else be.empty(M, blk.A * blk.B))
                    self.S2.append(be.empty(M, blk.A * blk.B) if blk.has_miss else None)
            self.rowscale = [(float(blk.A * blk.B) / blk.rowcnt) if blk.has_miss else None for blk in self.blocks]
            any_miss = any(blk.has_miss for blk in self.blocks)
            self.Yw = be.empty(I, 2 * M if self._s_pair else M) if any_miss else None
            self.Gy = be.empty(M, M)
            self.Tq = be.empty(nb, M)
            self.qx = [be.zeros(M), be.zeros(M)]
            self.qc = self.qx[0]
            self.qn = self.Tq[0] if (nb == 1 and not coupled) else be.empty(M)
            self._s_carry = (not any(blk.has_miss for blk in self.blocks)
                             and all(hasattr(be, f) for f in ("s_downdate", "deflate_contract_yq")))
            self._s_ready = False
            self._nowrite = False
            if self.raw:
                self.zM = be.zeros(M)
                self.zA = [be.zeros(blk.A) for blk in self.blocks]
                self.zB = [be.zeros(blk.B) for blk in self.blocks]
            if self._s_carry:
                self.yhat = be.empty(I, 1)
                self.one = be.empty(1)
                self.one.fill_(1.0)
                self.vs = [be.empty(blk.A * blk.B) for blk in self.blocks]
                self._nowrite = eng.opt.xcov_nowrite and hasattr(be, "kr_axpy") and R <= 64
                if self._nowrite:
                    self.dot_log = be.zeros(R, 1 + len(self.blocks))
                    self.Gw = be.empty(R * R)
                    self._G_last = None
                    self._one_read = R > 1 and eng.opt.xcov_one_read and hasattr(be, "score_contract")
                    if self._one_read:
                        self._fused_b = max(range(len(self.blocks)), key=lambda b: self.blocks[b].A * self.blocks[b].B)
                        P0 = self.blocks[self._fused_b].A * self.blocks[self._fused_b].B
                        self.ps = be.empty(P0)
                        self.Rm = be.zeros(P0, R)
                        self.corr = be.empty(I)
                        self.csum = be.empty(1)
            assert self._nowrite or not self.raw, "an uncentred X needs the form of the loop that never writes it"

    def _half_declined(self, want_raw: bool, allow_raw: bool, shapes, M: int) -> Optional[str]:
        eng, be = self.eng, self.eng.be
        if self.algorithm != "xcov":
            return 'algorithm="direct" centres and deflates X in place'
        if not half_route(eng, None, HALF_ENTRIES["fit"])[0]:
            return "the backend has no 16-bit entries"
        if self.R > 64:
            return "more than 64 components"
        if M > 64:
            return "more than 64 responses (the statistics come out of the read that builds S, 64 responses per pass)"
        if not allow_raw:
            return "f32 matrix precision"
        if not (want_raw and eng.opt.xcov_ssq_with_s and eng.opt.xcov_stats_with_s and hasattr(be, "xcov_ssq")):
            return "the options switch off the uncentred cross-covariance form that never writes X"
        for shape, d in zip(shapes, self.half_storage):
            A, B = split_trailing(shape)
            if d is not None and (A + B) * 16 * 8 > 152 * 1024:
                return f"a block of trailing extents {A} x {B}: loadings beyond the LDS of the 16-bit score pass (MTTKRP)"
        return None

    def _half_reads_form(self, b: int) -> str:
        seen = self.half_reads.get(b, set())
        if "score_contract" in seen:
            return "one-read (score_contract)"
        if {"mttkrp", "xcov"} <= seen:
            return "two-read (mttkrp + xcov)"
        if "mttkrp" in seen:
            return "one read (mttkrp: a single component needs no down-date of S)"
        return "none"

    def _blocks_from_one_read(self, Xs: List[torch.Tensor]) -> Optional[List[BlockState]]:
        be, comm = self.eng.be, self.eng.comm
        blocks, n = [], float(self.n_total)
        for b, X in enumerate(Xs):
            I = X.shape[0]
            X2 = X.view(I, -1)
            P = X2.shape[1]
            out = be.xcov_stats(X2, self.Y, out=be.empty(self.M, P))
            if out is None:
                return None
            S, stats = out
            comm.allreduce(stats)
            colsum, colsq = stats[:P], stats[P:]
            ssq = (colsq - colsum * colsum / n).sum().reshape(1)
            if not bool(torch.isfinite(ssq).all().item()):
                return None
            A, B = split_trailing(X.shape)
            blocks.append(BlockState(shape=tuple(X.shape), A=A, B=B, mean=colsum / n, has_miss=False, colcnt=None, rowcnt=None,
                                     ssq0=float("nan"), dtype=X.dtype))
            self._s_prebuilt[b] = S
            self._ssq0_dev[b] = ssq
        return blocks

    def start_component(self, a: int) -> None:
        self._executed = 0
        be, comm = self.eng.be, self.eng.comm
        if self.algorithm == "direct":
            self.u.copy_(self.Y[:, 0])
            self._parity = 0
            if self._fused:
                self.qbuf[0].zero_()
                self.qbuf[0][0] = 1.0
            if self._fused or comm.sharded:
                be.gram_tn(self.Y, self.Y, out=self.Gy)
                comm.allreduce(self.Gy)
            return
        for b, blk in enumerate(self.blocks):
            if self._s_ready:
                break
            if self.S12[b] is not None:
                self.Yw[:, :self.M].copy_(self.Y)
                torch.mul(self.Y, self.rowscale[b][:, None], out=self.Yw[:, self.M:])
                be.xcov(self.X2[b], self.Yw, True, out=self.S12[b], mixed=self.mixed)
                comm.allreduce(self.S12[b])
                continue
            if b in self._s_prebuilt:
                del self._s_prebuilt[b]
            elif self.raw and self._ssq_with_s and b not in self._ssq0_dev:
                _, ssq = be.xcov_ssq(self.X2[b], self.Y, blk.mean, out=self.S[b])
                self._ssq0_dev[b] = comm.allreduce(ssq)
            else:
                be.xcov(self.X2[b], self.Y, blk.has_miss, out=self.S[b], mixed=self.mixed)
            comm.allreduce(self.S[b])
            if self.raw:
                ysum, _ = be.colstats(self.Y)
                comm.allreduce(ysum)
                be.s_downdate(self.S[b], blk.A, blk.B, self.zM, self.zA[b], self.zB[b], ysum, blk.mean)
            if blk.has_miss:
                torch.mul(self.Y, self.rowscale[b][:, None], out=self.Yw)
                be.xcov(self.X2[b], self.Yw, True, out=self.S2[b], mixed=self.mixed)
                comm.allreduce(self.S2[b])
        self._s_ready = False
        be.gram_tn(self.Y, self.Y, out=self.Gy)
        comm.allreduce(self.Gy)
        self._parity = 0
        self.qc = self.qx[0]
        self.qc.zero_()
        self.qc[0] = 1.0

    def inner_loop(self, a: int, max_iter: int, tol: float, verbose: int = 0) -> None:
        if max_iter > 0 and self._pipeline_ok():
            self._pipelined = True
            self._inner_loop_xcov_pipelined(a, max_iter, tol, verbose)
            return
        for it in range(max_iter):
            du = self.iterate(it)
            if du is not None and du < tol:
                if verbose:
                    print("Comp {}: converged after {} iterations".format(a, it))
                break

    def _update_budgets(self, host) -> bool:
        retry = False
        for b in range(len(self.blocks)):
            conv, used = host[1 + 2 * b] > 0.5, int(host[2 + 2 * b])
            if used < 0:
                self._chain_gave_up()
                retry = True
                continue
            if not conv and self.sq_budget[b] < self.sq_max:
                self.sq_budget[b] = self.sq_max
                retry = True
            elif conv and len(self.blocks[b].shape) == 3:
                if not self.use_graphs or used + 1 > self.sq_budget[b] or used + 3 < self.sq_budget[b]:
                    self.sq_budget[b] = min(self.sq_max, used + (1 if self.use_graphs else self.sq_spare[b]))
        return retry

    def _peer_failed(self, host, first_attempt: bool) -> bool:
        if not self.eng.comm.sharded:
            return False
        if first_attempt:
            self._nan_tails = 0
        if np.isfinite(float(host[0])) or self._nan_tails > int(getattr(self.eng.comm, "world", 1)):
            return False
        self._nan_tails += 1
        return True

    def _chain_gave_up(self) -> None:
        be = self.eng.be
        if hasattr(be, "rank1_chain_gave_up"):
            be.rank1_chain_gave_up()
        self._graphs.clear()
        self.sq_spare = [1] * len(self.blocks)
        note = "rank-1 chain of squarings in one launch switched off: a workgroup never became resident (GPU shared with another process)"
        if note not in self.notes:
            self.notes.append(note)

    def _read_status(self) -> np.ndarray:
        if self.status_host is None:
            return self.status.cpu().numpy()
        self.status_host.copy_(self.status, non_blocking=True)
        torch.cuda.current_stream(self.status.device).synchronize()
        return self.status_host.numpy()

    def _run(self, key, fn) -> None:
        if not self.use_graphs:
            fn()
            return
        g = self._graphs.get(key)
        if g is not None:
            g.replay()
            return
        fn()
        try:
            g = torch.cuda.CUDAGraph()
            with torch.cuda.graph(g, capture_error_mode="thread_local"):
                fn()
            self._graphs[key] = g
        except Exception as e:
            self.use_graphs = False
            self._graph_error = repr(e)
            self._after_failed_capture()

    def _run_with_collectives(self, key, fn) -> bool:
        if not (self.use_graphs and self.eng.opt.capture_collectives and self._collectives_captured is not False):
            return False
        if not getattr(self.eng.comm, "capturable", False):
            self._collectives_captured = False
            self.notes.append(f"all-reduces not captured into the iteration's graph: the {getattr(self.eng.comm, 'backend', None)} "
                              "backend stages through the host (only RCCL collectives are stream-ordered kernels)")
            return False
        g = self._graphs.get(key)
        if g is not None:
            g.replay()
            return True
        fn()
        try:
            torch.cuda.current_stream().synchronize()
            g = torch.cuda.CUDAGraph()
            with torch.cuda.graph(g, capture_error_mode="thread_local"):
                fn()
            self._graphs[key] = g
            self._collectives_captured = True
        except Exception as e:
            self._collectives_captured = False
            self.notes.append("all-reduces not captured into the iteration's graph: " + repr(e)[:200])
            self._after_failed_capture()
        return True

    def _after_failed_capture(self) -> None:
        try:
            torch.cuda.synchronize()
        except Exception:
            pass
        if hasattr(self.eng.be, "clear_error"):
            self.eng.be.clear_error()

    def iterate(self, it: int) -> Optional[float]:
        if self.algorithm == "xcov":
            return self._iterate_xcov(it)
        be, comm = self.eng.be, self.eng.comm
        if self._fused:
            return self._iterate_fused(it)
        self._executed += 1
        sharded = comm.sharded
        par = self._parity
        u, u_new = (self.u, self.u_new) if par == 0 else (self.u_new, self.u)

        def seg_contract():
            for b, blk in enumerate(self.blocks):
                be.mode0_contract(self.X2[b], u, blk.has_miss, out=self.Zs[b])

        def seg_colscale():
            for b, blk in enumerate(self.blocks):
                if blk.has_miss:
                    be.colscale(self.Zs[b], blk.colcnt, self.n_total)

        def seg_loadings_scores():
            for b, blk in enumerate(self.blocks):
                self.eng._rank1(blk, self.Zs[b], self.wA[b], self.wB[b], info=self.status[1 + 2 * b: 3 + 2 * b],
                                n_squarings=self.sq_budget[b], fac=self.fac[b], tol=self.tol)
                be.score(self.X2[b], blk.A, blk.B, self.wA[b], self.wB[b],
                         blk.rowcnt if blk.has_miss else None, self.Ts[b])
            if self.t.data_ptr() != self.Ts.data_ptr():
                be.scores_mean(self.Ts, self.t)
            be.gram_tn(self.Y, self.t, out=self.q)

        def seg_y_update():
            be.normalize(self.q)
            if sharded:
                be.rowdot(self.Y, self.q, u_new, None)
                be.quadform(self.Gy, self.q, self.q_prev if it > 0 else self.q, self.status[0:1])
            else:
                be.rowdot(self.Y, self.q, u_new, u if it > 0 else None, du2=self.status[0:1])

        first = True
        while True:
            budgets = tuple(self.sq_budget)
            if not sharded:
# ... 151 lines not shown
                blk.loadings[0][:, a].copy_(self.wA[b])
                blk.loadings[1][:, a].copy_(self.wB[b])
            else:
                for m, d in enumerate(blk.shape[1:]):
                    blk.loadings[m][:, a].copy_(self.fac[b][m, :d])
            if self.algorithm == "direct" and not self._fused:
                ssqs.append(be.deflate(self.X2[b], blk.A, blk.B, self.t, self.wA[b], self.wB[b]))
        if self.algorithm == "direct" and self._fused:
            self._finish_fused(a)
            return
        b_dev, _ = self._inner_regression(a)
        for b in range(len(self.blocks)):
            self.ssq_log[a, b].copy_(ssqs[b].reshape(()))
        ssqy = be.y_deflate(self.Y, self.T, a + 1, b_dev, self.q)
        self.ssq_log[a, len(self.blocks)].copy_(ssqy.reshape(()))

    def _inner_regression(self, a: int, extra: Optional[torch.Tensor] = None):
        be, comm = self.eng.be, self.eng.comm
        k = a + 1
        Ta = self.T[:, :k]
        G = be.gram_tn(Ta, Ta)
        g = be.gram_tn(Ta, self.u)
        if comm.sharded:
            packed = torch.cat([G.reshape(-1), g.reshape(-1)] + ([extra.reshape(-1)] if extra is not None else []))
            comm.allreduce(packed)
            G, g = packed[: k * k].view(k, k), packed[k * k: k * k + k]
            extra = packed[k * k + k:] if extra is not None else None
        b_dev = be.normal_solve(G, g.reshape(-1), out=self.b_dev[:k])
        self.coef_dev[:k, a].copy_(b_dev)
        self._G_last = G
        return b_dev, extra

    def _finish_fused(self, a: int) -> None:
        be, comm = self.eng.be, self.eng.comm
        k = a + 1
        b_dev, _ = self._inner_regression(a)
        ssqy = be.y_deflate(self.Y, self.T, k, b_dev, self.q)
        ssqs = []
        self._z_ready = False
        if k < self.R:
            q0 = self.qbuf[0]
            q0.zero_()
            q0[0] = 1.0
            ready = True
            for b, blk in enumerate(self.blocks):
                s_b = be.deflate_contract_yq(self.X2[b], blk.A, blk.B, self.t, self.wA[b], self.wB[b], self.Y, q0,
                                             blk.has_miss, out=self.Zs[b])
                if s_b is None:
                    s_b = be.deflate(self.X2[b], blk.A, blk.B, self.t, self.wA[b], self.wB[b])
                    ready = False
                ssqs.append(s_b)
            self._z_ready = ready
        else:
            for b, blk in enumerate(self.blocks):
                ssqs.append(be.deflate(self.X2[b], blk.A, blk.B, self.t, self.wA[b], self.wB[b]))
        self._log_ssq(a, ssqs, ssqy)

    def _log_ssq(self, a: int, ssqs, ssqy) -> None:
        for b in range(len(self.blocks)):
            self.ssq_log[a, b].copy_(ssqs[b].reshape(()))
        self.ssq_log[a, len(self.blocks)].copy_(ssqy.reshape(()))

    def _store_component(self, a: int) -> None:
        self.T[:, a].copy_(self.t)
        self.U[:, a].copy_(self.u)
        self.Q[:, a].copy_(self.q)
        self._store_loadings(a)

    def _store_loadings(self, a: int) -> None:
        for b, blk in enumerate(self.blocks):
            if len(blk.shape) == 2:
                blk.loadings[0][:, a].copy_(self.wB[b])
            elif len(blk.shape) == 3:
                blk.loadings[0][:, a].copy_(self.wA[b])
                blk.loadings[1][:, a].copy_(self.wB[b])
            else:
                for m, d in enumerate(blk.shape[1:]):
                    blk.loadings[m][:, a].copy_(self.fac[b][m, :d])

    def result(self) -> FitState:
        if getattr(self, "_state", None) is not None:
            return self._state
        nb = len(self.blocks)
        nowrite = self.algorithm == "xcov" and getattr(self, "_nowrite", False)
        for b, ssq in getattr(self, "_ssq0_dev", {}).items():
            self.blocks[b].ssq0 = float(ssq.item())
        self.eng.comm.allreduce(self.ssq_log)
        parts = [self.coef_dev.reshape(-1), self.ssq_log.reshape(-1)]
        if nowrite:
            self.eng.comm.allreduce(self.dot_log)
            parts.append(self.dot_log.reshape(-1))
        host = torch.cat(parts).cpu().numpy()
        R = self.R
        self.coef[...] = host[: R * R].reshape(R, R)
        ssq = host[R * R: R * R + R * (nb + 1)].reshape(R, nb + 1).copy()
        if nowrite:
            dots = host[R * R + R * (nb + 1):].reshape(R, 1 + nb)
            for b, blk in enumerate(self.blocks):
                run = blk.ssq0
                for a in range(len(self.n_iter)):
                    run = run - 2.0 * dots[a, 1 + b] + dots[a, 0]
                    ssq[a, b] = run
        for a in range(len(self.n_iter)):
            for b, blk in enumerate(self.blocks):
                blk.r2x[a] = 1.0 - ssq[a, b] / blk.ssq0
            self.r2y[a] = 1.0 - ssq[a, nb] / self.ssqy0
        self._state = FitState(coupled=self.coupled, n_components=self.R, blocks=self.blocks, T=self.T, U=self.U, Q=self.Q,
                               coef=self.coef, r2y=self.r2y, y_mean=self.y_mean, n_iter=self.n_iter,
                               n_samples_total=self.n_total, report=self.build_report())
        return self._state

    def build_report(self) -> Dict[str, object]:
        eng, comm, nb = self.eng, self.eng.comm, len(self.blocks)
        rep: Dict[str, object] = {
            "form": "regular", "algorithm_requested": self.algorithm_requested, "algorithm": self.algorithm,
            "shapes": [tuple(b.shape) for b in self.blocks], "storage": [dtype_name(b.dtype) for b in self.blocks],
            "missing": [bool(b.has_miss) for b in self.blocks], "responses": self.M,
            "sharded": bool(comm.sharded), "world": int(comm.world),
            "graphs": bool(self.use_graphs and self._graphs), "graph_error": self._graph_error,
            "collectives_in_graph": self._collectives_captured is True,
            "backend": getattr(eng.be, "name", type(eng.be).__name__),
        }
        if self.algorithm == "direct":
            rep["y_side"] = "fused into the sweeps" if self._fused else "separate launches"
            if not self._fused and self.M > 64:
                self.notes.append("Y side not fused into the sweeps: more than 64 responses")
            rep["x_passes_per_iteration"] = "2 reads"
            rep["x_passes_per_component"] = ("1 read + write (deflation fused with the next contraction)" if self._fused
                                             else "1 read + write (deflation)")
            rep["x_copy"] = "centred private copy"
        else:
            nowrite = bool(getattr(self, "_nowrite", False))
            one_read = nowrite and bool(getattr(self, "_one_read", False))
            any_miss = any(b.has_miss for b in self.blocks)
            rep["x_copy"] = "none: the caller's uncentred tensor is read in place" if self.raw else "centred private copy"
            rep["raw"] = bool(self.raw)
            rep["x_written"] = not nowrite
            rep["s_carried"] = bool(self._s_carry)
            rep["s_build"] = ("per component (missing values)" if any_miss else "first component only") + \
                             (f", {(self.M + 63) // 64} response tiles of <= 64" if self.M > 64 else "") + \
                             (", [Y, Y * rowscale] in one pass" if any(x is not None for x in self.S12) else "")
            rep["one_read"] = one_read
            rep["stats_with_s"] = bool(getattr(self, "_stats_with_s", False))
            if nowrite:
                rep["x_passes_per_component"] = ("1 read (largest block); 2 reads (other blocks)" if one_read and nb > 1 else
                                                 "1 read" if one_read else "2 reads")
            elif any_miss and nb == 1 and getattr(self, "_deflate_build_ok", True) and self.S12[0] is not None and eng.opt.xcov_deflate_build:
                rep["x_passes_per_component"] = "1 read + 1 read + write (deflation inside the rebuild of S)"
            elif any_miss:
                rep["x_passes_per_component"] = "1 read + write (score + deflation) + S rebuild reads"
            else:
                rep["x_passes_per_component"] = "1 read + 1 read + write"
            rep["pipelined"] = bool(getattr(self, "_pipelined", False))
            if rep["pipelined"]:
                rep["pipeline"] = dict(self.pipeline_stats)
            if not rep["pipelined"] and eng.opt.xcov_pipeline:
                why = ("graph replay requested" if self.use_graphs else "more than 64 responses" if self.M > 64 else
                       "a block of order > 3 or a backend without the single-call iteration")
                self.notes.append("inner loop on S not pipelined: " + why)
            if self.algorithm_requested == "xcov" and not self.raw and eng.opt.xcov_raw and not any_miss and not any("uncentred" in n for n in self.notes):
                self.notes.append("uncentred xcov form declined: " + ("more than 64 components" if self.R > 64 else
                                                                      "f32 matrix precision or a backend without its kernels"))
            if nowrite and eng.opt.xcov_one_read and self.R > 1 and not one_read:
                self.notes.append("one read per component declined: the row does not fit the registers of 1..16 workgroups "
                                  "(rows of 2048..131072 f32 -- 262144 when the last mode divides 4096 -- / 1024..131072 f64 elements, "
                                  "last mode a multiple of 4 / 2)")
        if any(d is not None for d in self.half_storage):
            rep["half_storage"] = {
                "in_place": self.half_fallback is None,
                "fallback": self.half_fallback,
                "reads": [None if d is None or self.half_fallback is not None else self._half_reads_form(b)
                          for b, d in enumerate(self.half_storage)],
            }
        rep["rank1_one_launch_chain"] = bool(getattr(eng.be, "rank1_chain_side", 0)) and any(
            len(blk.shape) == 3 and min(blk.A, blk.B) <= int(getattr(eng.be, "rank1_chain_side", 0)) for blk in self.blocks)
        rep["declined"] = list(self.notes)
        return rep
```

cmtf_pls_amd/fitrun_xcov.py:

```python
from __future__ import annotations

import math
from typing import Optional

import torch

from .storage import HALF_DTYPES


class XcovMixin:
    def _score_x0(self, b: int, out: torch.Tensor) -> None:
        be, blk, X2 = self.eng.be, self.blocks[b], self.X2[b]
        if X2.dtype in HALF_DTYPES:
            self.half_reads.setdefault(b, set()).add("mttkrp")
            if be.mttkrp(X2, blk.A, blk.B, self.wA[b].view(-1, 1), self.wB[b].view(-1, 1), out.view(-1, 1)) is None:
                raise RuntimeError("mttkrp refused a shape the 16-bit fit was planned for")
        else:
            be.score(X2, blk.A, blk.B, self.wA[b], self.wB[b], None, out)

    def _contract_x0(self, b: int, v: torch.Tensor, out: torch.Tensor) -> None:
        be, X2 = self.eng.be, self.X2[b]
        if X2.dtype in HALF_DTYPES:
            self.half_reads.setdefault(b, set()).add("xcov")
            if be.xcov(X2, v.view(-1, 1), False, out=out.view(1, -1)) is None:
# ... 59 lines not shown
            return False
        return self._single_composite() or (hasattr(be, "xcov_blocks_plan") and all(len(blk.shape) in (2, 3) for blk in self.blocks))

    def _inner_loop_xcov_pipelined(self, a: int, max_iter: int, tol: float, verbose: int) -> None:
        be = self.eng.be
        nb = len(self.blocks)
        single = self._single_composite()
        pp = getattr(self, "_pipe", None)
        if pp is None:
            M = self.M
            second = {"Z": [], "wA": [], "wB": []}
            for b, blk in enumerate(self.blocks):
                second["Z"].append(be.empty(blk.A * blk.B))
                second["wA"].append(self.wA[b].clone())
                second["wB"].append(be.empty(blk.B))
            pp = self._pipe = {
                "q": [self.qx[0], self.qx[1], be.zeros(M)],
                "Z": [list(self.Zs), second["Z"]], "wA": [list(self.wA), second["wA"]], "wB": [list(self.wB), second["wB"]],
                "status": [be.zeros(1 + 2 * nb), be.zeros(1 + 2 * nb)],
                "plans": {}, "slots": {},
            }
            for st in pp["status"]:
                st[1::2] = 1.0
        plans = pp["plans"]

        def make_plan(it: int):
            s = it & 1
            st, q_cur, q_new = pp["status"][s], pp["q"][it % 3], pp["q"][(it + 1) % 3]
            if single:
                blk0 = self.blocks[0]
                if hasattr(be, "xcov_iterate_plan"):
                    one = be.xcov_iterate_plan(self.S[0], blk0.A, blk0.B, q_cur, pp["Z"][s][0], pp["wA"][s][0], pp["wB"][s][0], st,
                                               q_new, self.Gy)
                    return lambda nsq, first: one(nsq[0], first)
                return lambda nsq, first: be.xcov_iterate(self.S[0], blk0.A, blk0.B, q_cur, pp["Z"][s][0], pp["wA"][s][0],
                                                          pp["wB"][s][0], st[1:3], nsq[0], q_new, self.Gy, st[0:1], first)
            descr = [dict(S=self.S[b], S2=self.S2[b] if blk.has_miss else None, colcnt=blk.colcnt if blk.has_miss else None,
                          n_samples=self.n_total, order=len(blk.shape), A=blk.A, B=blk.B,
                          Z=pp["Z"][s][b], wA=pp["wA"][s][b], wB=pp["wB"][s][b]) for b, blk in enumerate(self.blocks)]
            return be.xcov_blocks_plan(descr, self.M, q_cur, self.Tq, q_new, self.Gy, st)

        def enqueue(it: int, first: bool = True):
            plan = plans.get(it % 6)
            if plan is None:
                plan = plans[it % 6] = make_plan(it)
            plan([n if it > 0 else min(self.sq_max, n + 4) for n in self.sq_budget], first)
            return be.status_snapshot(pp["status"][it & 1], it & 1, slots=pp["slots"])

        stats = self.pipeline_stats
        it, tok = 0, enqueue(0)
        du_prev = du = None
        while True:
            ahead = None
            if it + 1 < max_iter:
                predicted = None if (du is None or du_prev is None or du_prev <= 0.0) else du * (du / du_prev)
                if it == 0 or predicted is None or predicted >= tol:
                    ahead = enqueue(it + 1)
                    stats["ahead"] += 1
            host = be.status_wait(tok)
            short = [b for b in range(nb) if not host[1 + 2 * b] > 0.5 and self.sq_budget[b] < self.sq_max]
            if any(host[2 + 2 * b] < 0 for b in range(nb)):
                self._chain_gave_up()
                pp["plans"].clear()
                tok = enqueue(it, first=False)
                stats["redone"] += 1
                continue
            if short:
                for b in short:
                    self.sq_budget[b] = self.sq_max
                tok = enqueue(it, first=False)
                stats["redone"] += 1
                continue
            for b, blk in enumerate(self.blocks):
                if len(blk.shape) == 3 and host[1 + 2 * b] > 0.5:
                    self.sq_budget[b] = min(self.sq_max, int(host[2 + 2 * b]) + self.sq_spare[b])
            self._executed += 1
            stats["iterations"] += 1
            du_prev, du = du, (None if it == 0 else math.sqrt(max(float(host[0]), 0.0)))
            if (du is not None and du < tol) or it + 1 >= max_iter:
                if verbose and du is not None and du < tol:
                    print("Comp {}: converged after {} iterations".format(a, it))
                stats["unused"] += ahead is not None
                break
            it += 1
            stats["waited"] += ahead is None
            tok = ahead if ahead is not None else enqueue(it)
        if it & 1:
            for b in range(nb):
                self.wA[b].copy_(pp["wA"][1][b])
                self.wB[b].copy_(pp["wB"][1][b])
        self.qc = pp["q"][(it + 1) % 3]
        self._parity = 0

    def _finish_xcov_masked_fused(self, a: int) -> bool:
        be, comm = self.eng.be, self.eng.comm
        blk, M = self.blocks[0], self.M
        if blk.A * blk.B % 4 != 0:
            self._deflate_build_ok = False
            return False
        self.q = self.qc
        be.score(self.X2[0], blk.A, blk.B, self.wA[0], self.wB[0], blk.rowcnt, self.t)
        be.rowdot(self.Y, self.q, self.u, None)
        self._store_component(a)
        b_dev, _ = self._inner_regression(a)
        ssqy = be.y_deflate(self.Y, self.T, a + 1, b_dev, self.q)
        self.Yw[:, :M].copy_(self.Y)
        torch.mul(self.Y, self.rowscale[0][:, None], out=self.Yw[:, M:])
        ssq = be.xcov_deflate(self.X2[0], blk.A, blk.B, self.Yw, self.t, self.wA[0], self.wB[0], out=self.S12[0])
        if ssq is None:
            self._deflate_build_ok = False
            ssq = be.deflate(self.X2[0], blk.A, blk.B, self.t, self.wA[0], self.wB[0])
        else:
            comm.allreduce(self.S12[0])
            self._s_ready = True
        self._log_ssq(a, [ssq], ssqy)
        return True

    def _finish_xcov_carry(self, a: int) -> None:
        be, comm = self.eng.be, self.eng.comm
        self.q = self.qc
        for b, blk in enumerate(self.blocks):
            be.score(self.X2[b], blk.A, blk.B, self.wA[b], self.wB[b], None, self.Ts[b])
        if self.t.data_ptr() != self.Ts.data_ptr():
            be.scores_mean(self.Ts, self.t)
        be.rowdot(self.Y, self.q, self.u, None)
        self._store_component(a)
        k = a + 1
        Ta = self.T[:, :k]
        ya = be.gram_tn(self.Y, self.t).reshape(-1)
        b_dev, ya_g = self._inner_regression(a, extra=ya)
        ssqs = []
        if k < self.R:
            be.rowdot(Ta, b_dev, self.yhat.view(-1), None)
        ssqy = be.y_deflate(self.Y, self.T, k, b_dev, self.q)
        if k < self.R:
            carried = True
            for b, blk in enumerate(self.blocks):
                s_b = be.deflate_contract_yq(self.X2[b], blk.A, blk.B, self.t, self.wA[b], self.wB[b], self.yhat, self.one,
                                             False, out=self.vs[b])
                if s_b is None:
                    s_b = be.deflate(self.X2[b], blk.A, blk.B, self.t, self.wA[b], self.wB[b])
                    carried = False
                ssqs.append(s_b)
            if carried:
                for b, blk in enumerate(self.blocks):
                    comm.allreduce(self.vs[b])
                    be.s_downdate(self.S[b], blk.A, blk.B, ya_g, self.wA[b], self.wB[b], self.q, self.vs[b])
            self._s_ready = carried
        else:
            for b, blk in enumerate(self.blocks):
                ssqs.append(be.deflate(self.X2[b], blk.A, blk.B, self.t, self.wA[b], self.wB[b]))
        self._log_ssq(a, ssqs, ssqy)

    def _finish_xcov_nowrite(self, a: int) -> None:
        be, comm = self.eng.be, self.eng.comm
        self.q = self.qc
        I, R, k = self.I, self.R, a + 1
        nb = len(self.blocks)
        self._store_loadings(a)
        fused_b = self._fused_b if (getattr(self, "_one_read", False) and k < R) else -1
        one_read = False
        for b in [x for x in range(nb) if x != fused_b] + ([fused_b] if fused_b >= 0 else []):
            blk = self.blocks[b]
            mw = None
            if self.raw:
                mw = be.score_s(blk.mean.view(1, -1), blk.A, blk.B, self.wA[b], self.wB[b], be.empty(1))
            g = None
            if a > 0 and hasattr(be, "kr_gram_row"):
                for m, L in enumerate(blk.loadings):
                    be.kr_gram_row(L, a, self.Gw, first=(m == 0))
                g = self.Gw[:a]
            elif a > 0:
                for m, L in enumerate(blk.loadings):
                    be.kr_gram(L, self.Gw, first=(m == 0))
                g = self.Gw.view(R, R)[a, :a]
            if b == fused_b:
                corr = others = None
                if a > 0:
                    be.rowdot(self.T[:, :a], g, self.corr, None)
                    corr = self.corr
                if nb == 2:
                    others = self.Ts[1 - b]
                elif nb > 2:
                    others = self.Ts[[x for x in range(nb) if x != b]].sum(dim=0)
                one_read = be.score_contract(self.X2[b], blk.A, blk.B, self.wA[b], self.wB[b], mw, self.Ts[b], self.ps,
                                             sub_own=corr, add_other=others, alpha=1.0 / nb,
                                             csum=self.csum if self.raw else None) is not None
                if one_read:
                    if self.X2[b].dtype in HALF_DTYPES:
                        self.half_reads.setdefault(b, set()).add("score_contract")
                    continue
                self._one_read = False
            self._score_x0(b, self.Ts[b])
            if mw is not None:
                be.axpy_scalar(self.Ts[b], mw)
            if a > 0:
                be.y_deflate(self.Ts[b].view(I, 1), self.T, a, g, self.one)
        single = self.t.data_ptr() == self.Ts.data_ptr()
        if not single:
            be.scores_mean(self.Ts, self.t)
        if one_read:
            comm.allreduce(self.ps)
            if self.raw:
                be.axpy_scalar(self.ps, comm.allreduce(self.csum), self.blocks[fused_b].mean)
            self.Rm[:, a].copy_(self.ps)
        be.rowdot(self.Y, self.q, self.u, None)
        be.gram_tn(self.t, self.t, out=self.dot_log[a, 0:1])
        for b in range(nb):
            if single:
                self.dot_log[a, 1 + b].copy_(self.dot_log[a, 0])
            else:
                be.gram_tn(self.Ts[b], self.t, out=self.dot_log[a, 1 + b: 2 + b])
        self.T[:, a].copy_(self.t)
        self.U[:, a].copy_(self.u)
        self.Q[:, a].copy_(self.q)
        Ta = self.T[:, :k]
        ya = be.gram_tn(self.Y, self.t).reshape(-1)
        b_dev, ya_g = self._inner_regression(a, extra=ya)
        if k < R and not (one_read and nb == 1):
            be.rowdot(Ta, b_dev, self.yhat.view(-1), None)
        ssqy = be.y_deflate(self.Y, self.T, k, b_dev, self.q)
        if k < R:
            c = be.gram_tn(self._G_last, b_dev).reshape(-1)
            for b, blk in enumerate(self.blocks):
                WA, WB = self.eng._kr_operands(blk, R)
                if one_read and b == fused_b:
                    be.rowdot(self.Rm[:, :k], b_dev, self.vs[b], None)
                else:
                    self._contract_x0(b, self.yhat.view(-1), self.vs[b])
                    comm.allreduce(self.vs[b])
                    if self.raw:
                        be.axpy_scalar(self.vs[b], comm.allreduce(be.total(self.yhat.view(-1))), blk.mean)
                be.kr_axpy(self.vs[b], blk.A, blk.B, WA, WB, k, c)
                be.s_downdate(self.S[b], blk.A, blk.B, ya_g, self.wA[b], self.wB[b], self.q, self.vs[b])
            self._s_ready = True
        self.ssq_log[a, nb].copy_(ssqy.reshape(()))
```

cmtf_pls_amd/options.py:

```python
from __future__ import annotations

from dataclasses import dataclass, replace
from typing import Optional


@dataclass(frozen=True)
class EngineOptions:
    small_fit: bool = True
    small_fit_elements: int = 1 << 15
    xcov_nowrite: bool = True
    xcov_raw: bool = True
    xcov_raw_max_offset: float = 1e4
    project_raw_max_offset: float = 1e4
    xcov_one_read: bool = True
    xcov_pair_build: bool = True
    xcov_ssq_with_s: bool = True
    xcov_stats_with_s: bool = True
    xcov_deflate_build: bool = True
    xcov_pipeline: bool = True
    capture_collectives: bool = False
    project_split_rows: bool = True
    masked_folds: bool = False
    masked_folds_coupled: bool = False
    coupled_permutations: bool = False
    tensor_folds: bool = False
    tensor_folds_coupled: bool = False
    masked_tensor_folds: bool = False
    tensor_resamples_coupled: bool = False
    masked_tensor_folds_coupled: bool = False
    half_folds: bool = False
    half_diagnostics: bool = False

    def but(self, **changes) -> "EngineOptions":
        return replace(self, **changes)


_DEFAULT_OPTIONS = EngineOptions()


def default_options() -> EngineOptions:
    return _DEFAULT_OPTIONS


def set_default_options(options: Optional[EngineOptions]) -> EngineOptions:
    global _DEFAULT_OPTIONS
    old, _DEFAULT_OPTIONS = _DEFAULT_OPTIONS, (options if options is not None else EngineOptions())
    return old
```

include/cmtfpls.h:

```cpp
#ifndef CMTFPLS_H
#define CMTFPLS_H

#include <stddef.h>
#include <stdint.h>

#ifdef __cplusplus
extern "C" {
#endif

#define CMTFPLS_OK 0
#define CMTFPLS_EINVAL 1
#define CMTFPLS_EWORKSPACE 2
#define CMTFPLS_EHIP 3
#define CMTFPLS_EUNSUPPORTED 4

int cmtfpls_abi_version(void);
const char* cmtfpls_last_error(void);
int cmtfpls_clear_error(void);
int cmtfpls_status_to_host(const void* src, void* dst_host, size_t bytes, void* event, void* stream);

size_t cmtfpls_colstats_workspace_bytes(int64_t I, int64_t P);
int cmtfpls_colstats_f32(const float* X, int64_t I, int64_t P, double* colsum, double* colcnt,
                         void* ws, size_t ws_bytes, void* stream);
int cmtfpls_colstats_f64(const double* X, int64_t I, int64_t P, double* colsum, double* colcnt,
// ... 4 lines not shown
int cmtfpls_center_f64(double* X, int64_t I, int64_t P, const double* mean, double* rowcnt,
                       double* ssq_part, void* stream);

size_t cmtfpls_mode0_contract_workspace_bytes(int64_t I, int64_t P);
int cmtfpls_mode0_contract_f32(const float* X, int64_t I, int64_t P, const double* u, double* Z,
                               int masked, void* ws, size_t ws_bytes, void* stream);
int cmtfpls_mode0_contract_f64(const double* X, int64_t I, int64_t P, const double* u, double* Z,
                               int masked, void* ws, size_t ws_bytes, void* stream);
int cmtfpls_mode0_contract_yq_f32(const float* X, int64_t I, int64_t P, const double* Y, int ldy, int M,
                                  const double* q, double* Z, int masked, void* ws, size_t ws_bytes, void* stream);
int cmtfpls_mode0_contract_yq_f64(const double* X, int64_t I, int64_t P, const double* Y, int ldy, int M,
                                  const double* q, double* Z, int masked, void* ws, size_t ws_bytes, void* stream);
int cmtfpls_colscale_f64(double* Z, int64_t P, const double* colcnt, double n_samples, void* stream);

size_t cmtfpls_rank1_workspace_bytes(int A, int B);
int cmtfpls_rank1_f64(const double* Z, int A, int B, double* wA, double* wB, double* sigma, double* info,
                      int n_squarings, void* ws, size_t ws_bytes, void* stream);
int cmtfpls_rank1_launches_f64(const double* Z, int A, int B, double* wA, double* wB, double* sigma, double* info,
                               int n_squarings, void* ws, size_t ws_bytes, void* stream);
void cmtfpls_rank1_chain_enable(int on);
int cmtfpls_rank1_chain_enabled(void);
int cmtfpls_rank1_score_f64(const double* Z, int A, int B, double* wA, double* wB, double* info, int n_squarings,
                            const double* S, int M, double* tq, void* ws, size_t ws_bytes, void* stream);
int cmtfpls_normalize_f64(double* v, int64_t n, double* nrm, void* stream);
size_t cmtfpls_rank1_tensor_workspace_bytes(const int* dims, int n);
int cmtfpls_rank1_tensor_f64(const double* Z, const int* dims, int n, double tol, double* factors, int ld,
                             double* info, int n_squarings, void* ws, size_t ws_bytes, void* stream);
int cmtfpls_kron_f64(const double* a, int na, const double* b, int nb, double* out, void* stream);

size_t cmtfpls_xcov_workspace_bytes(int64_t I, int64_t P, int M);
int cmtfpls_xcov_f32(const float* X, int64_t I, int64_t P, const double* Y, int ldy, int M, double* S,
                     int masked, void* ws, size_t ws_bytes, void* stream);
int cmtfpls_xcov_f64(const double* X, int64_t I, int64_t P, const double* Y, int ldy, int M, double* S,
                     int masked, void* ws, size_t ws_bytes, void* stream);
int cmtfpls_quadform_f64(const double* G, int M, const double* q, const double* q_old, double* out, void* stream);
int cmtfpls_xcov_bf16(const uint16_t* X, int64_t I, int64_t P, const double* Y, int ldy, int M, double* S,
                      int masked, void* ws, size_t ws_bytes, void* stream);
int cmtfpls_xcov_f16(const uint16_t* X, int64_t I, int64_t P, const double* Y, int ldy, int M, double* S,
                     int masked, void* ws, size_t ws_bytes, void* stream);
int cmtfpls_xcov_deflate_f32(float* X, int64_t I, int A, int B, const double* Y, int ldy, int M, const double* t, const double* wA,
                             const double* wB, double* S, double* ssq, void* ws, size_t ws_bytes, void* stream);
int cmtfpls_xcov_deflate_f64(double* X, int64_t I, int A, int B, const double* Y, int ldy, int M, const double* t, const double* wA,
                             const double* wB, double* S, double* ssq, void* ws, size_t ws_bytes, void* stream);
size_t cmtfpls_xcov_ssq_workspace_bytes(int64_t I, int64_t P, int M);
size_t cmtfpls_xcov_stats_workspace_bytes(int64_t I, int64_t P, int M);
int cmtfpls_xcov_stats_f32(const float* X, int64_t I, int64_t P, const double* Y, int ldy, int M, double* S, double* stats,
                           void* ws, size_t ws_bytes, void* stream);
int cmtfpls_xcov_stats_f64(const double* X, int64_t I, int64_t P, const double* Y, int ldy, int M, double* S, double* stats,
                           void* ws, size_t ws_bytes, void* stream);
int cmtfpls_xcov_stats_bf16(const uint16_t* X, int64_t I, int64_t P, const double* Y, int ldy, int M, double* S, double* stats,
                            void* ws, size_t ws_bytes, void* stream);
int cmtfpls_xcov_stats_f16(const uint16_t* X, int64_t I, int64_t P, const double* Y, int ldy, int M, double* S, double* stats,
                           void* ws, size_t ws_bytes, void* stream);
int cmtfpls_xcov_ssq_f32(const float* X, int64_t I, int64_t P, const double* Y, int ldy, int M, double* S, const double* mean,
                         double* ssq, void* ws, size_t ws_bytes, void* stream);
int cmtfpls_xcov_ssq_f64(const double* X, int64_t I, int64_t P, const double* Y, int ldy, int M, double* S, const double* mean,
                         double* ssq, void* ws, size_t ws_bytes, void* stream);
int cmtfpls_xcov_iterate_f64(const double* S, int M, int A, int B, const double* q_cur, double* Z, double* wA,
                             double* wB, double* info, int n_squarings, double* q_new, const double* G, double* du2,
                             int first, void* ws_contract, size_t ws_contract_bytes, void* ws_rank1,
                             size_t ws_rank1_bytes, void* stream);
typedef struct {
  const double* S;
  const double* S2;
  const double* colcnt;
  double n_samples;
  int order;
  int A, B;
  int n_squarings;
  double* Z;
  double* wA;
  double* wB;
  double* info;
} cmtfpls_xcov_block;
int cmtfpls_xcov_iterate_blocks_f64(const cmtfpls_xcov_block* blocks, int nb, int M, const double* q_cur, double* tq, double* q_new,
                                    const double* G, double* du2, int first, void* ws_rank1, size_t ws_rank1_bytes, void* stream);
int cmtfpls_s_downdate_f64(double* S, int M, int A, int B, const double* ya, const double* wA, const double* wB,
                           const double* q, const double* v, void* stream);
int cmtfpls_kr_axpy_f64(double* v, int A, int B, const double* WA, const double* WB, int ld, int k, const double* coef, void* stream);
int cmtfpls_axpy_scalar_f64(double* y, int64_t n, const double* a, const double* x, void* stream);
size_t cmtfpls_score_contract_workspace_bytes(int64_t I, int64_t P);
int cmtfpls_score_contract_f32(const float* X, int64_t I, int A, int B, const double* wA, const double* wB, const double* shift,
                               const double* sub_own, const double* add_other, double alpha, double* t, double* Z, double* csum,
                               void* ws, size_t ws_bytes, void* stream);
int cmtfpls_score_contract_f64(const double* X, int64_t I, int A, int B, const double* wA, const double* wB, const double* shift,
                               const double* sub_own, const double* add_other, double alpha, double* t, double* Z, double* csum,
                               void* ws, size_t ws_bytes, void* stream);
int cmtfpls_score_contract_bf16(const uint16_t* X, int64_t I, int A, int B, const double* wA, const double* wB, const double* shift,
                                const double* sub_own, const double* add_other, double alpha, double* t, double* Z, double* csum,
                                void* ws, size_t ws_bytes, void* stream);
int cmtfpls_score_contract_f16(const uint16_t* X, int64_t I, int A, int B, const double* wA, const double* wB, const double* shift,
                               const double* sub_own, const double* add_other, double alpha, double* t, double* Z, double* csum,
                               void* ws, size_t ws_bytes, void* stream);
int cmtfpls_xcov_f32_mixed(const float* X, int64_t I, int64_t P, const double* Y, int ldy, int M, double* S,
                           int masked, void* ws, size_t ws_bytes, void* stream);
int cmtfpls_mttkrp_f32_mixed(const float* X, int64_t I, int A, int B, const double* WA, const double* WB, int R,
                             double* out, int ldo, void* stream);

int cmtfpls_mttkrp_f32(const float* X, int64_t I, int A, int B, const double* WA, const double* WB, int R,
                       double* out, int ldo, void* stream);
int cmtfpls_mttkrp_f64(const double* X, int64_t I, int A, int B, const double* WA, const double* WB, int R,
                       double* out, int ldo, void* stream);
int cmtfpls_mttkrp_bf16(const uint16_t* X, int64_t I, int A, int B, const double* WA, const double* WB, int R,
                        double* out, int ldo, void* stream);
int cmtfpls_mttkrp_f16(const uint16_t* X, int64_t I, int A, int B, const double* WA, const double* WB, int R,
                       double* out, int ldo, void* stream);

int cmtfpls_score_f32(const float* X, int64_t I, int A, int B, const double* wA, const double* wB,
                      const double* rowcnt, double* t, void* stream);
int cmtfpls_score_f64(const double* X, int64_t I, int A, int B, const double* wA, const double* wB,
                      const double* rowcnt, double* t, void* stream);
int cmtfpls_score_s_f64(const double* S, int M, int A, int B, const double* wA, const double* wB, double* tq, void* stream);

size_t cmtfpls_deflate_contract_workspace_bytes(int64_t I, int64_t P);
int cmtfpls_deflate_contract_yq_f32(float* X, int64_t I, int A, int B, const double* t, const double* wA,
                                    const double* wB, const double* Y, int ldy, int M, const double* q, double* Z,
                                    int masked, double* ssq, void* ws, size_t ws_bytes, void* stream);
int cmtfpls_deflate_contract_yq_f64(double* X, int64_t I, int A, int B, const double* t, const double* wA,
                                    const double* wB, const double* Y, int ldy, int M, const double* q, double* Z,
                                    int masked, double* ssq, void* ws, size_t ws_bytes, void* stream);
int cmtfpls_score_gram_f32(const float* X, int64_t I, int A, int B, const double* wA, const double* wB,
                           const double* rowcnt, double* t, const double* Y, int ldy, int M, double* qpart,
                           void* stream);
int cmtfpls_score_gram_f64(const double* X, int64_t I, int A, int B, const double* wA, const double* wB,
                           const double* rowcnt, double* t, const double* Y, int ldy, int M, double* qpart,
                           void* stream);
int cmtfpls_q_update_f64(const double* qpart, int nblk, int M, double* q, int normalize, const double* G,
                         const double* q_prev, double* du2, void* stream);

int cmtfpls_deflate_f32(float* X, int64_t I, int A, int B, const double* t, const double* wA,
                        const double* wB, double* ssq_part, void* stream);
int cmtfpls_deflate_f64(double* X, int64_t I, int A, int B, const double* t, const double* wA,
                        const double* wB, double* ssq_part, void* stream);

int cmtfpls_score_deflate_f32(float* X, int64_t I, int A, int B, const double* wA, const double* wB,
                              const double* rowcnt, double* t, double* ssq_part, void* stream);
int cmtfpls_score_deflate_f64(double* X, int64_t I, int A, int B, const double* wA, const double* wB,
                              const double* rowcnt, double* t, double* ssq_part, void* stream);

int cmtfpls_sweep_form(const char* op, int elem_bytes, int64_t I, int A, int B, int masked, int M,
                       int aligned16, char* out, size_t n);
int cmtfpls_sweep_form_list(const char* op, int elem_bytes, char* out, size_t n);

size_t cmtfpls_small_workspace_bytes(void);
int cmtfpls_gram_tn_f64(const double* A, int lda, int a, const double* B, int ldb, int b, int64_t I,
                        double* C, void* ws, size_t ws_bytes, void* stream);
int cmtfpls_rowdot_f64(const double* Y, int ldy, int M, int64_t I, const double* q, double* u,
                       const double* u_old, double* du2, void* ws, size_t ws_bytes, void* stream);
int cmtfpls_scores_mean_f64(const double* Ts, int nb, int64_t I, double* out, void* stream);
int cmtfpls_y_deflate_f64(double* Y, int ldy, int M, int64_t I, const double* T, int ldt, int R,
                          const double* b, const double* q, double* ssq, void* ws, size_t ws_bytes,
                          void* stream);
int cmtfpls_sum_f64(const double* in, int64_t n, double* out, void* stream);

int cmtfpls_project_rows_f32(const float* X, int64_t I, int A, int B, int R, const double* WA, const double* WB,
                             const double* mean, double* scores, int ld, void* stream);
int cmtfpls_project_rows_f64(const double* X, int64_t I, int A, int B, int R, const double* WA, const double* WB,
                             const double* mean, double* scores, int ld, void* stream);
int cmtfpls_project_rows2_f32(const float* X0, int A0, int B0, const double* WA0, const double* WB0, const double* mean0,
                              const float* X1, int A1, int B1, const double* WA1, const double* WB1, const double* mean1,
                              int64_t I, int R, double* scores, int ld, void* stream);
int cmtfpls_project_rows2_f64(const double* X0, int A0, int B0, const double* WA0, const double* WB0, const double* mean0,
                              const double* X1, int A1, int B1, const double* WA1, const double* WB1, const double* mean1,
                              int64_t I, int R, double* scores, int ld, void* stream);
int cmtfpls_project_rows_idx_f32(const float* X, const int64_t* rows, int64_t n_rows, int A, int B, int R, const double* WA,
                                 const double* WB, const double* mean, double* scores, int ld, void* stream);
int cmtfpls_project_rows_idx_f64(const double* X, const int64_t* rows, int64_t n_rows, int A, int B, int R, const double* WA,
                                 const double* WB, const double* mean, double* scores, int ld, void* stream);
int cmtfpls_project_rows2_idx_f32(const float* X0, int A0, int B0, const double* WA0, const double* WB0, const double* mean0,
                                  const float* X1, int A1, int B1, const double* WA1, const double* WB1, const double* mean1,
                                  const int64_t* rows, int64_t n_rows, int R, double* scores, int ld, void* stream);
int cmtfpls_project_rows2_idx_f64(const double* X0, int A0, int B0, const double* WA0, const double* WB0, const double* mean0,
                                  const double* X1, int A1, int B1, const double* WA1, const double* WB1, const double* mean1,
                                  const int64_t* rows, int64_t n_rows, int R, double* scores, int ld, void* stream);

int cmtfpls_allreduce_sum_f64(void* comm, double* buf, size_t count, void* stream);
int cmtfpls_allreduce_sum_f32(void* comm, float* buf, size_t count, void* stream);

int cmtfpls_normal_solve_f64(const double* G, const double* g, int k, double* b, int incb, void* stream);
size_t cmtfpls_normal_solve_workspace_bytes(int k);
int cmtfpls_normal_solve_ws_f64(const double* G, const double* g, int k, double* b, int incb, void* ws, size_t ws_bytes,
                                void* stream);
int cmtfpls_unit_upper_solve_rows_f64(double* M, int64_t I, int ld, int R, const double* U, const double* shift, int* nan_flag,
                                      void* stream);
int cmtfpls_kr_gram_f64(const double* L, int n, int R, double* G, int first, double scale, void* stream);
int cmtfpls_kr_gram_row_f64(const double* L, int n, int R, int a, double* g, int first, void* stream);
int cmtfpls_khatri_rao_f64(const double* Am, int na, const double* Bm, int nb, int R, double* out, void* stream);
int cmtfpls_predict_rows_f64(const double* S, int64_t I, int lds, int R, const double* Bm, int M, const double* mean,
                             double* out, int ldo, void* stream);
int cmtfpls_recon_f32(const double* T, int64_t I, int ldt, int R, const double* WA, const double* WB, int A, int B,
                      const double* mean, float* out, void* stream);
int cmtfpls_recon_f64(const double* T, int64_t I, int ldt, int R, const double* WA, const double* WB, int A, int B,
                      const double* mean, double* out, void* stream);
size_t cmtfpls_recon_r2_workspace_bytes(int64_t I, int64_t P);
int cmtfpls_recon_r2_f32(const float* X, const double* T, int64_t I, int ldt, int R, const double* WA, const double* WB,
                         int A, int B, const double* mean, double* out, void* ws, size_t ws_bytes, void* stream);
int cmtfpls_recon_r2_f64(const double* X, const double* T, int64_t I, int ldt, int R, const double* WA, const double* WB,
                         int A, int B, const double* mean, double* out, void* ws, size_t ws_bytes, void* stream);
int cmtfpls_recon_r2_bf16(const uint16_t* X, const double* T, int64_t I, int ldt, int R, const double* WA, const double* WB,
                          int A, int B, const double* mean, double* out, void* ws, size_t ws_bytes, void* stream);
int cmtfpls_recon_r2_f16(const uint16_t* X, const double* T, int64_t I, int ldt, int R, const double* WA, const double* WB,
                         int A, int B, const double* mean, double* out, void* ws, size_t ws_bytes, void* stream);

size_t cmtfpls_resid_rows_workspace_bytes(int64_t I, int64_t P);
int cmtfpls_resid_rows_f32(const float* X, const double* T, int64_t I, int ldt, int R, const double* WA, const double* WB,
                           int A, int B, const double* mean, double* rows, double* cols, void* ws, size_t ws_bytes, void* stream);
int cmtfpls_resid_rows_f64(const double* X, const double* T, int64_t I, int ldt, int R, const double* WA, const double* WB,
                           int A, int B, const double* mean, double* rows, double* cols, void* ws, size_t ws_bytes, void* stream);
int cmtfpls_resid_rows_bf16(const uint16_t* X, const double* T, int64_t I, int ldt, int R, const double* WA, const double* WB,
                            int A, int B, const double* mean, double* rows, double* cols, void* ws, size_t ws_bytes, void* stream);
int cmtfpls_resid_rows_f16(const uint16_t* X, const double* T, int64_t I, int ldt, int R, const double* WA, const double* WB,
                           int A, int B, const double* mean, double* rows, double* cols, void* ws, size_t ws_bytes, void* stream);

int cmtfpls_contrib_rows_f32(const float* X, int64_t I, const double* T, int ldt, const double* H, int ldh, int R, const double* WA,
                             const double* WB, int A, int B, const double* mean, const int64_t* rows, int64_t n, double* speA, double* speB,
                             double* t2A, double* t2B, void* stream);
int cmtfpls_contrib_rows_f64(const double* X, int64_t I, const double* T, int ldt, const double* H, int ldh, int R, const double* WA,
                             const double* WB, int A, int B, const double* mean, const int64_t* rows, int64_t n, double* speA, double* speB,
                             double* t2A, double* t2B, void* stream);
int cmtfpls_contrib_rows_bf16(const uint16_t* X, int64_t I, const double* T, int ldt, const double* H, int ldh, int R, const double* WA,
                              const double* WB, int A, int B, const double* mean, const int64_t* rows, int64_t n, double* speA, double* speB,
                              double* t2A, double* t2B, void* stream);
int cmtfpls_contrib_rows_f16(const uint16_t* X, int64_t I, const double* T, int ldt, const double* H, int ldh, int R, const double* WA,
                             const double* WB, int A, int B, const double* mean, const int64_t* rows, int64_t n, double* speA, double* speB,
                             double* t2A, double* t2B, void* stream);

size_t cmtfpls_selectivity_cols_workspace_bytes(int64_t I, int64_t P, int M);
int cmtfpls_selectivity_cols_f32(const float* X, int64_t I, int64_t P, const double* Tau, int ldtau, int M, const double* mean,
                                 int masked, double* a, double* d, double* s, double* n, void* ws, size_t ws_bytes, void* stream);
int cmtfpls_selectivity_cols_f64(const double* X, int64_t I, int64_t P, const double* Tau, int ldtau, int M, const double* mean,
                                 int masked, double* a, double* d, double* s, double* n, void* ws, size_t ws_bytes, void* stream);
int cmtfpls_selectivity_cols_bf16(const uint16_t* X, int64_t I, int64_t P, const double* Tau, int ldtau, int M, const double* mean,
                                  int masked, double* a, double* d, double* s, double* n, void* ws, size_t ws_bytes, void* stream);
int cmtfpls_selectivity_cols_f16(const uint16_t* X, int64_t I, int64_t P, const double* Tau, int ldtau, int M, const double* mean,
                                 int masked, double* a, double* d, double* s, double* n, void* ws, size_t ws_bytes, void* stream);

size_t cmtfpls_holdout_mask_workspace_bytes(int64_t n);
int cmtfpls_holdout_mask_f32(const float* X, float* out, int64_t n, double fraction, uint64_t seed, uint32_t stream, uint64_t offset,
                             double* counts, void* ws, size_t ws_bytes, void* hipstream);
int cmtfpls_holdout_mask_f64(const double* X, double* out, int64_t n, double fraction, uint64_t seed, uint32_t stream, uint64_t offset,
                             double* counts, void* ws, size_t ws_bytes, void* hipstream);
size_t cmtfpls_heldout_resid_workspace_bytes(int64_t I, int64_t P, int R);
int cmtfpls_heldout_resid_f32(const float* X, int64_t I, int A, int B, const double* T, int ldt, int R, const double* WA, const double* WB,
                              const double* mean, double fraction, uint64_t seed, uint32_t stream, uint64_t offset, double* out,
                              void* ws, size_t ws_bytes, void* hipstream);
int cmtfpls_heldout_resid_f64(const double* X, int64_t I, int A, int B, const double* T, int ldt, int R, const double* WA, const double* WB,
                              const double* mean, double fraction, uint64_t seed, uint32_t stream, uint64_t offset, double* out,
                              void* ws, size_t ws_bytes, void* hipstream);
size_t cmtfpls_impute_workspace_bytes(int64_t I, int64_t P);
int cmtfpls_impute_f32(const float* X, float* out, int64_t I, int A, int B, const double* T, int ldt, int R, const double* WA,
                       const double* WB, const double* mean, double* count, void* ws, size_t ws_bytes, void* hipstream);
int cmtfpls_impute_f64(const double* X, double* out, int64_t I, int A, int B, const double* T, int ldt, int R, const double* WA,
                       const double* WB, const double* mean, double* count, void* ws, size_t ws_bytes, void* hipstream);

size_t cmtfpls_loo_fold_workspace_bytes(int I, int A, int B, int M, int R);
int cmtfpls_loo_tpls_f64(const double* X, const double* Y, const double* colsum_x, const double* colsum_y, int I, int A,
                         int B, int M, int R, double tol, int max_iter, int fold0, int nfolds, double* Ypred,
                         int* n_iter, void* ws, size_t ws_bytes, void* stream);
size_t cmtfpls_loo_xcov_fold_workspace_bytes(int I, int A, int B, int M, int R);
int cmtfpls_loo_xcov_f64(const double* X, const double* Y, const double* colsum_x, const double* colsum_y, int I, int A,
                         int B, int M, int R, double tol, int max_iter, int fold0, int nfolds, double* Ypred,
                         int* n_iter, void* ws, size_t ws_bytes, void* stream);
size_t cmtfpls_loo_xcov_tensor_fold_workspace_bytes(int I, int A, int B1, int B2, int M, int R);
size_t cmtfpls_loo_xcov_tensor_lds_bytes(int A, int B1, int B2, int M, int R);
int cmtfpls_loo_xcov_tensor_f64(const double* X, const double* Y, const double* colsum_x, const double* colsum_y, int I, int A,
                                int B1, int B2, int M, int R, double tol, int max_iter, int fold0, int nfolds, double* Ypred,
                                int* n_iter, void* ws, size_t ws_bytes, void* stream);
typedef struct {
  const double* X;
  const double* colsum;
  int order;
  int A, B;
} cmtfpls_loo_coupled_block;
size_t cmtfpls_loo_xcov_coupled_fold_workspace_bytes(const cmtfpls_loo_coupled_block* blocks, int nb, int I, int M, int R);
size_t cmtfpls_loo_xcov_coupled_lds_bytes(const cmtfpls_loo_coupled_block* blocks, int nb, int I, int M, int R);
int cmtfpls_loo_xcov_coupled_f64(const cmtfpls_loo_coupled_block* blocks, int nb, const double* Y, const double* colsum_y, int I,
                                 int M, int R, double tol, int max_iter, int fold0, int nfolds, double* Ypred, int* n_iter,
                                 void* ws, size_t ws_bytes, void* stream);
size_t cmtfpls_loo_xcov_coupled_tensor_fold_workspace_bytes(const cmtfpls_loo_coupled_block* blocks, int nb, const int* dims, int I,
                                                            int M, int R);
size_t cmtfpls_loo_xcov_coupled_tensor_lds_bytes(const cmtfpls_loo_coupled_block* blocks, int nb, const int* dims, int I, int M, int R);
int cmtfpls_loo_xcov_coupled_tensor_f64(const cmtfpls_loo_coupled_block* blocks, int nb, const int* dims, const double* Y,
                                        const double* colsum_y, int I, int M, int R, double tol, int max_iter, int fold0, int nfolds,
                                        double* Ypred, int* n_iter, void* ws, size_t ws_bytes, void* stream);
size_t cmtfpls_cv_masked_fold_workspace_bytes(int I, int A, int B, int M, int R);
int cmtfpls_cv_masked_f64(const double* X, const double* Y, const int* fold_of, int K, const double* colsum_x,
                          const double* colcnt_x, const double* colsum_y, int I, int A, int B, int M, int R, double tol,
                          int max_iter, int fold0, int nfolds, double* Ypred, int* n_iter, int* status, int* info, void* ws,
                          size_t ws_bytes, void* stream);
size_t cmtfpls_cv_masked_model_workspace_bytes(int I, int A, int B, int M, int R);
int cmtfpls_cv_masked_models_f64(const double* X, const double* Y, const int* counts, const int* yrow, int nm, int I, int A,
                                 int B, int M, int R, double tol, int max_iter, int model0, int nmodels, double* Ypred,
                                 double* Wa, double* Wb, double* coef, double* Q, int* n_iter, int* status, int* info,
                                 void* ws, size_t ws_bytes, void* stream);
size_t cmtfpls_cv_masked_tensor_lds_bytes(int I, int A, int B1, int B2, int M, int R);
size_t cmtfpls_cv_masked_tensor_fold_workspace_bytes(int I, int A, int B1, int B2, int M, int R);
int cmtfpls_cv_masked_tensor_f64(const double* X, const double* Y, const int* fold_of, int K, const double* colsum_x,
                                 const double* colcnt_x, const double* colsum_y, int I, int A, int B1, int B2, int M, int R,
                                 double tol, int max_iter, int fold0, int nfolds, double* Ypred, int* n_iter, int* status,
                                 int* info, void* ws, size_t ws_bytes, void* stream);
size_t cmtfpls_cv_masked_tensor_model_workspace_bytes(int I, int A, int B1, int B2, int M, int R);
int cmtfpls_cv_masked_tensor_models_f64(const double* X, const double* Y, const int* counts, const int* yrow, int nm, int I,
                                        int A, int B1, int B2, int M, int R, double tol, int max_iter, int model0, int nmodels,
                                        double* Ypred, double* Wa, double* Wk, double* Wl, double* coef, double* Q, int* n_iter,
                                        int* status, int* info, void* ws, size_t ws_bytes, void* stream);
typedef struct {
// ... 120 lines not shown
```

Before: 759.3.

## Batch component-boundary small kernels into native dependency-levelled job launches

Adds a native 'component boundary' path that plans the many small per-component operations (loading copies, KR gram row, rowdot, gram partials and reductions, normal solve, Y deflation, S down-date, next-q start) as a job table. Jobs at the same dependency level go into one batched launch, cutting the number of kernel launches and Python/ctypes calls between NIPALS components. It also lets the next component's setup begin in the tail, skipping the separate Gy/q initialisation. It applies only to a single unmasked, unsharded order-3 block with at most 64 responses and components, and adds a large block of planning code that could be wrong.

```diff
diff --git a/cmtf_pls_amd/_lib.py b/cmtf_pls_amd/_lib.py
--- a/cmtf_pls_amd/_lib.py
+++ b/cmtf_pls_amd/_lib.py
@@ -12,6 +12,12 @@
 class XcovBlock(ctypes.Structure):
     _fields_ = [("S", _P), ("S2", _P), ("colcnt", _P), ("n_samples", c_double), ("order", c_int), ("A", c_int), ("B", c_int),
                 ("n_squarings", c_int), ("Z", _P), ("wA", _P), ("wB", _P), ("info", _P)]
+
+
+class XcovBoundary(ctypes.Structure):
+    POINTERS = ("Y", "T", "U", "Q", "LA", "LB", "wA", "wB", "t", "u", "q", "q_next", "mean", "mw", "Gw", "corr", "ps", "csum", "Rm", "vs",
+                "S", "dot_log", "ssq_log", "coef", "b", "G", "g", "ya", "c", "Gy")
+    _fields_ = [("I", c_int64), ("A", c_int), ("B", c_int), ("M", c_int), ("R", c_int)] + [(name, _P) for name in POINTERS]
 
 
 class KfoldState(ctypes.Structure):
@@ -118,6 +124,15 @@
     "cmtfpls_scores_mean_f64": (c_int, [_P, c_int, c_int64, _P, _P]),
     "cmtfpls_y_deflate_f64": (c_int, [_P, c_int, c_int, c_int64, _P, c_int, c_int, _P, _P, _P, _P, c_size_t, _P]),
     "cmtfpls_sum_f64": (c_int, [_P, c_int64, _P, _P]),
+    "cmtfpls_xcov_boundary_launches": (c_int, [c_int, c_int, c_int, c_int, c_int64, c_int, c_int, c_int]),
+    "cmtfpls_xcov_boundary_launch_info": (c_int, [c_int, c_int, c_int, c_int, c_int64, c_int, c_int, c_int, c_int] + [ctypes.POINTER(c_int)] * 4),
+    "cmtfpls_xcov_boundary_job_info": (c_int, [c_int, c_int, c_int, c_int, c_int64, c_int, c_int, c_int, c_int, c_int]
+                                       + [ctypes.POINTER(c_int)] * 6),
+    "cmtfpls_xcov_boundary_buffer_info": (c_int, [c_int, c_char_p, c_size_t] + [ctypes.POINTER(c_int)] * 3),
+    "cmtfpls_xcov_boundary_head_workspace_bytes": (c_size_t, [c_int, c_int]),
+    "cmtfpls_xcov_boundary_tail_workspace_bytes": (c_size_t, [c_int, c_int]),
+    "cmtfpls_xcov_boundary_head_f64": (c_int, [ctypes.POINTER(XcovBoundary), c_int, c_int, _P, c_size_t, _P]),
+    "cmtfpls_xcov_boundary_tail_f64": (c_int, [ctypes.POINTER(XcovBoundary), c_int, c_int, _P, c_size_t, _P]),
     "cmtfpls_normal_solve_f64": (c_int, [_P, _P, c_int, _P, c_int, _P]),
     "cmtfpls_normal_solve_workspace_bytes": (c_size_t, [c_int]),
     "cmtfpls_normal_solve_ws_f64": (c_int, [_P, _P, c_int, _P, c_int, _P, c_size_t, _P]),
diff --git a/cmtf_pls_amd/backend.py b/cmtf_pls_amd/backend.py
--- a/cmtf_pls_amd/backend.py
+++ b/cmtf_pls_amd/backend.py
@@ -328,6 +328,23 @@
             if rc:
                 _lib.check(rc, "xcov_iterate_blocks")
         return enqueue
+
+    def xcov_boundary(self, I: int, A: int, B: int, M: int, R: int, **bufs: torch.Tensor):
+        for name, v in bufs.items():
+            assert name in _lib.XcovBoundary.POINTERS and v.dtype == torch.float64 and v.is_contiguous() and v.device == self.device, name
+        st = _lib.XcovBoundary(I=I, A=A, B=B, M=M, R=R, **{name: _ptr(v) for name, v in bufs.items()})
+        nbytes = max(self.lib.cmtfpls_xcov_boundary_head_workspace_bytes(M, R), self.lib.cmtfpls_xcov_boundary_tail_workspace_bytes(M, R))
+        ws = self._workspace("xcov_boundary", nbytes)
+        fns = (self.lib.cmtfpls_xcov_boundary_head_f64, self.lib.cmtfpls_xcov_boundary_tail_f64)
+        ref, wp, wn, stream = ctypes.byref(st), _ptr(ws), ws.numel(), self._stream
+
+        def call(phase: int, a: int, raw: bool, one_read: bool, q: Optional[torch.Tensor] = None, _keep=(bufs, ws, st)):
+            if q is not None:
+                assert q.dtype == torch.float64 and q.is_contiguous() and q.numel() == M
+                st.q = q.data_ptr()
+            rc = fns[phase](ref, int(a), (1 if raw else 0) | (2 if one_read else 0), wp, wn, stream())
+            return self._form(rc, "xcov_boundary")
+        return call
 
     def s_downdate(self, S: torch.Tensor, A: int, B: int, ya: torch.Tensor, wA: torch.Tensor, wB: torch.Tensor,
                    q: torch.Tensor, v: torch.Tensor) -> None:
diff --git a/cmtf_pls_amd/csrc/boundary.hip b/cmtf_pls_amd/csrc/boundary.hip
--- /dev/null
+++ b/cmtf_pls_amd/csrc/boundary.hip
@@ -0,0 +1,455 @@
+#include <string.h>
+
+#include <vector>
+
+#include "common.hpp"
+#include "small_jobs.hpp"
+
+namespace cmtfpls {
+
+constexpr int kJobBlocks = 128;
+constexpr int kMaxJobs = 24;
+
+enum JobKind {
+  kJobGemvT = 0, kJobGramTile, kJobReduce, kJobRowdot, kJobYDeflate, kJobSum, kJobSolve, kJobKrGramRow, kJobKrAxpy, kJobAxpyScalar,
+  kJobSDowndate, kJobCopy, kJobFill, kJobScoreS , kJobKinds
+};
+
+struct Job {
+  void* p[6];
+  int64_t n;
+  int i[5];
+  int kind;
+};
+struct JobTable {
+  Job job[kMaxJobs];
+  int start[kMaxJobs + 1];
+  int njobs;
+  int pad;
+};
+static_assert(sizeof(JobTable) <= 2048, "the job table travels in the kernel arguments");
+
+template <int THREADS>
+__global__ __launch_bounds__(THREADS) void job_batch_kernel(const JobTable tab) {
+  extern __shared__ double lds[];
+  int j = 0;
+  while (j + 1 < tab.njobs && (int)blockIdx.x >= tab.start[j + 1]) ++j;
+  const Job& jb = tab.job[j];
+  const int bid = (int)blockIdx.x - tab.start[j];
+  const int nblk = tab.start[j + 1] - tab.start[j];
+  const double* p0 = static_cast<const double*>(jb.p[0]);
+  if constexpr (THREADS == 1024) {
+    if (jb.kind == kJobSum) sum_body(p0, jb.n, static_cast<double*>(jb.p[1]), lds);
+  } else {
+    switch (jb.kind) {
+      case kJobGemvT:
+        gemv_t_body(bid, nblk, p0, jb.i[0], jb.i[1], jb.i[2], static_cast<const double*>(jb.p[1]), jb.i[3], jb.n, static_cast<double*>(jb.p[2]),
+                    jb.i[4], reinterpret_cast<double (*)[16]>(lds));
+        break;
+      case kJobGramTile:
+        gram_tn_body(bid, nblk, p0, jb.i[0], jb.i[1], static_cast<const double*>(jb.p[1]), jb.i[2], jb.i[3], jb.n, static_cast<double*>(jb.p[2]),
+                     jb.i[4], lds);
+        break;
+      case kJobReduce:
+        reduce_block_body(bid, p0, jb.i[0], jb.i[1], jb.i[2], static_cast<double*>(jb.p[1]), jb.i[3]);
+        break;
+      case kJobRowdot:
+        rowdot_body(bid, nblk, p0, jb.i[0], jb.i[1], jb.n, static_cast<const double*>(jb.p[1]), static_cast<double*>(jb.p[2]), nullptr, nullptr, lds);
+        break;
+      case kJobYDeflate:
+        y_deflate_body(bid, nblk, static_cast<double*>(jb.p[0]), jb.i[0], jb.i[1], jb.n, static_cast<const double*>(jb.p[1]), jb.i[2], jb.i[3],
+                       static_cast<const double*>(jb.p[2]), static_cast<const double*>(jb.p[3]), static_cast<double*>(jb.p[4]), lds);
+        break;
+      case kJobSolve:
+        normal_solve_body(p0, static_cast<const double*>(jb.p[1]), jb.i[0], static_cast<double*>(jb.p[2]), jb.i[1], lds);
+        break;
+      case kJobKrGramRow:
+        kr_gram_row_body(p0, jb.i[0], jb.i[2], jb.i[3], static_cast<double*>(jb.p[2]), 1);
+        if (jb.p[1]) kr_gram_row_body(static_cast<const double*>(jb.p[1]), jb.i[1], jb.i[2], jb.i[3], static_cast<double*>(jb.p[2]), 0);
+        break;
+      case kJobKrAxpy:
+        kr_axpy_body(bid, static_cast<double*>(jb.p[0]), jb.n, jb.i[0], static_cast<const double*>(jb.p[1]), static_cast<const double*>(jb.p[2]),
+                     jb.i[1], jb.i[2], static_cast<const double*>(jb.p[3]), lds);
+        break;
+      case kJobAxpyScalar:
+        axpy_scalar_body(bid, nblk, static_cast<double*>(jb.p[0]), jb.n, static_cast<const double*>(jb.p[1]), static_cast<const double*>(jb.p[2]));
+        break;
+      case kJobSDowndate:
+        s_downdate_body(bid, static_cast<double*>(jb.p[0]), jb.i[0], jb.n, jb.i[1], static_cast<const double*>(jb.p[1]),
+                        static_cast<const double*>(jb.p[2]), static_cast<const double*>(jb.p[3]), static_cast<const double*>(jb.p[4]),
+                        static_cast<const double*>(jb.p[5]));
+        break;
+      case kJobCopy:
+        copy_strided_body(bid, nblk, static_cast<double*>(jb.p[0]), jb.i[0], static_cast<const double*>(jb.p[1]), jb.i[1], jb.n);
+        break;
+      case kJobFill:
+        fill_unit_body(bid, nblk, static_cast<double*>(jb.p[0]), jb.i[0], jb.n, jb.i[1]);
+        break;
+      default:
+        break;
+    }
+  }
+}
+
+enum Buf {
+  kBwA = 0, kBwB, kBmean, kBmw, kBLA, kBLB, kBGw, kBTprev, kBcorr,
+  kBt, kBq, kBY0, kBY1, kBps0, kBps1, kBcsum, kBu, kBT, kBU, kBQ, kBRm, kBdot0, kBdot1,
+  kBwsTT, kBwsYa, kBwsYa1, kBwsYa2, kBwsYa3, kBya, kBwsG, kBG, kBwsg, kBwsg1, kBwsg2, kBwsg3, kBg, kBb, kBcoef, kBwsYd, kBssq,
+  kBwsC, kBwsC1, kBwsC2, kBwsC3, kBc, kBvs0, kBvs1, kBwsGy, kBGy, kBS0, kBS1,
+  kBqnext, kBufs
+};
+struct BufInfo { const char* name; int storage; int version; int output; };
+static const BufInfo kBufInfo[kBufs] = {
+  {"wA", kBwA, 0, 0}, {"wB", kBwB, 0, 0}, {"mean", kBmean, 0, 0}, {"mw", kBmw, 0, 1}, {"loadings A[:, a]", kBLA, 0, 1},
+  {"loadings B[:, a]", kBLB, 0, 1}, {"Gw[:a]", kBGw, 0, 1}, {"T[:, :a]", kBTprev, 0, 0}, {"corr", kBcorr, 0, 1},
+  {"t", kBt, 0, 0}, {"q", kBq, 0, 0}, {"Y", kBY0, 0, 0}, {"Y deflated", kBY0, 1, 1}, {"ps", kBps0, 0, 0}, {"ps centred", kBps0, 1, 0},
+  {"csum", kBcsum, 0, 0}, {"u", kBu, 0, 1}, {"T[:, a]", kBT, 0, 1}, {"U[:, a]", kBU, 0, 1}, {"Q[:, a]", kBQ, 0, 1}, {"Rm[:, a]", kBRm, 0, 1},
+  {"dot_log[a, 0]", kBdot0, 0, 1}, {"dot_log[a, 1]", kBdot1, 0, 1},
+  {"ws t.t", kBwsTT, 0, 0}, {"ws Y^T t, columns 0..15", kBwsYa, 0, 0}, {"ws Y^T t, columns 16..31", kBwsYa1, 0, 0},
+  {"ws Y^T t, columns 32..47", kBwsYa2, 0, 0}, {"ws Y^T t, columns 48..63", kBwsYa3, 0, 0}, {"Y^T t", kBya, 0, 0}, {"ws T^T T", kBwsG, 0, 0}, {"T^T T", kBG, 0, 1},
+  {"ws T^T u, columns 0..15", kBwsg, 0, 0}, {"ws T^T u, columns 16..31", kBwsg1, 0, 0},
+  {"ws T^T u, columns 32..47", kBwsg2, 0, 0}, {"ws T^T u, columns 48..63", kBwsg3, 0, 0}, {"T^T u", kBg, 0, 0}, {"b", kBb, 0, 1}, {"coef[:k, a]", kBcoef, 0, 1}, {"ws |Y|^2", kBwsYd, 0, 0},
+  {"ssq_log[a, 1]", kBssq, 0, 1}, {"ws (T^T T) b, columns 0..15", kBwsC, 0, 0}, {"ws (T^T T) b, columns 16..31", kBwsC1, 0, 0},
+  {"ws (T^T T) b, columns 32..47", kBwsC2, 0, 0}, {"ws (T^T T) b, columns 48..63", kBwsC3, 0, 0}, {"(T^T T) b", kBc, 0, 0}, {"vs = Rm b", kBvs0, 0, 0},
+  {"vs corrected", kBvs0, 1, 0}, {"ws Y^T Y", kBwsGy, 0, 0}, {"Gy", kBGy, 0, 1}, {"S", kBS0, 0, 0}, {"S down-dated", kBS0, 1, 1},
+  {"q of the next component (may be the buffer of q)", kBq, 1, 1},
+};
+
+struct PlanJob {
+  int kind, threads, blocks, level;
+  int nr, nw;
+  int reads[6], writes[2];
+  size_t lds;
+  Job dev;
+};
+struct Launch { int level, threads; std::vector<int> jobs; };
+struct Plan {
+  std::vector<PlanJob> jobs;
+  std::vector<Launch> launches;
+};
+
+template <typename T>
+static T* off(T* p, int64_t n) { return p ? p + n : nullptr; }
+
+struct Builder {
+  Plan& plan;
+  int level = 0;
+  PlanJob& add(int kind, int threads, int blocks, size_t lds, std::initializer_list<int> reads, std::initializer_list<int> writes) {
+    PlanJob j{};
+    j.kind = kind; j.threads = threads; j.blocks = blocks; j.level = level; j.lds = lds;
+    for (int r : reads) j.reads[j.nr++] = r;
+    for (int w : writes) j.writes[j.nw++] = w;
+    j.dev.kind = kind;
+    plan.jobs.push_back(j);
+    return plan.jobs.back();
+  }
+  void copy(double* dst, int dstride, const double* src, int sstride, int64_t n, int rbuf, int wbuf) {
+    int64_t blocks = (n + 255) / 256;
+    if (blocks > kJobBlocks) blocks = kJobBlocks;
+    Job& d = add(kJobCopy, 256, (int)blocks, 0, {rbuf}, {wbuf}).dev;
+    d.p[0] = dst; d.p[1] = const_cast<double*>(src); d.n = n; d.i[0] = dstride; d.i[1] = sstride;
+  }
+  void gram_partials(const double* A, int lda, int a, const double* B, int ldb, int b, int64_t I, double* part, int rA, int rB, int wbuf) {
+    if (b == 1) {
+      for (int a0 = 0; a0 < a; a0 += 16) {
+        Job& d = add(kJobGemvT, 256, kJobBlocks, 64 * sizeof(double), {rA, rB}, {wbuf + a0 / 16}).dev;
+        d.p[0] = const_cast<double*>(A); d.p[1] = const_cast<double*>(B); d.p[2] = part; d.n = I;
+        d.i[0] = lda; d.i[1] = a0; d.i[2] = (a - a0 < 16) ? a - a0 : 16; d.i[3] = ldb; d.i[4] = a;
+      }
+      return;
+    }
+    const int tr = (a + b <= 32) ? 128 : (a + b <= 64) ? 64 : 32;
+    Job& d = add(kJobGramTile, 256, kJobBlocks, (size_t)tr * (a + b) * sizeof(double), {rA, rB}, {wbuf}).dev;
+    d.p[0] = const_cast<double*>(A); d.p[1] = const_cast<double*>(B); d.p[2] = part; d.n = I;
+    d.i[0] = lda; d.i[1] = a; d.i[2] = ldb; d.i[3] = b; d.i[4] = tr;
+  }
+  void gram_reduce(const double* part, int a, int b, double* C, int rbuf, int wbuf) {
+    PlanJob& pj = add(kJobReduce, 256, (a * b + 3) / 4, 0, {rbuf}, {wbuf});
+    if (b == 1)
+      for (int a0 = 16; a0 < a; a0 += 16) pj.reads[pj.nr++] = rbuf + a0 / 16;
+    Job& d = pj.dev;
+    d.p[0] = const_cast<double*>(part); d.p[1] = C; d.i[0] = kJobBlocks; d.i[1] = a; d.i[2] = b; d.i[3] = b;
+  }
+  void rowdot(const double* Y, int ldy, int M, int64_t I, const double* q, double* u, int rY, int rq, int wbuf) {
+    Job& d = add(kJobRowdot, 256, kJobBlocks, 16 * sizeof(double), {rY, rq}, {wbuf}).dev;
+    d.p[0] = const_cast<double*>(Y); d.p[1] = const_cast<double*>(q); d.p[2] = u; d.n = I; d.i[0] = ldy; d.i[1] = M;
+  }
+  void finish() {
+    for (size_t j = 0; j < plan.jobs.size(); ++j) {
+      const PlanJob& pj = plan.jobs[j];
+      Launch* into = nullptr;
+      if (pj.kind != kJobScoreS)
+        for (Launch& l : plan.launches)
+          if (l.level == pj.level && l.threads == pj.threads && (int)l.jobs.size() < kMaxJobs && plan.jobs[l.jobs[0]].kind != kJobScoreS) into = &l;
+      if (!into) {
+        plan.launches.push_back(Launch{pj.level, pj.threads, {}});
+        into = &plan.launches.back();
+      }
+      into->jobs.push_back((int)j);
+    }
+  }
+};
+
+constexpr int kFlagRaw = CMTFPLS_XCOV_BOUNDARY_RAW, kFlagOneRead = CMTFPLS_XCOV_BOUNDARY_ONE_READ;
+
+static bool shape_ok(int a, int R, int M, int64_t I, int A, int B) {
+  return R >= 1 && R <= 64 && M >= 1 && M <= 64 && a >= 0 && a < R && I > 0 && A > 0 && B > 0 && (int64_t)A * B <= (1 << 30);
+}
+
+struct TailWs { size_t tt, ya, G, g, yd, c, Gy, total; };
+static TailWs tail_ws(int M, int R) {
+  TailWs w{};
+  size_t o = 0;
+  w.tt = o; o += kJobBlocks;
+  w.ya = o; o += (size_t)kJobBlocks * M;
+  w.G = o; o += (size_t)kJobBlocks * R * R;
+  w.g = o; o += (size_t)kJobBlocks * R;
+  w.yd = o; o += kJobBlocks;
+  w.c = o; o += (size_t)kJobBlocks * R;
+  w.Gy = o; o += (size_t)kJobBlocks * M * M;
+  w.total = o;
+  return w;
+}
+
+static void build_head(const cmtfpls_xcov_boundary& s, int a, int flags, Plan& plan) {
+  Builder bd{plan};
+  const int R = s.R;
+  if (flags & kFlagRaw) bd.add(kJobScoreS, 1024, 1, 0, {kBmean, kBwA, kBwB}, {kBmw});
+  bd.copy(off(s.LA, a), R, s.wA, 1, s.A, kBwA, kBLA);
+  bd.copy(off(s.LB, a), R, s.wB, 1, s.B, kBwB, kBLB);
+  if (a > 0) {
+    bd.level = 1;
+    Job& d = bd.add(kJobKrGramRow, 256, 1, 0, {kBLA, kBLB}, {kBGw}).dev;
+    d.p[0] = s.LA; d.p[1] = s.LB; d.p[2] = s.Gw; d.i[0] = s.A; d.i[1] = s.B; d.i[2] = R; d.i[3] = a;
+    if (flags & kFlagOneRead) {
+      bd.level = 2;
+      bd.rowdot(s.T, R, a, s.I, s.Gw, s.corr, kBTprev, kBGw, kBcorr);
+    }
+  }
+  bd.finish();
+}
+
+static void build_tail(const cmtfpls_xcov_boundary& s, int a, int flags, double* ws, Plan& plan) {
+  Builder bd{plan};
+  const int R = s.R, M = s.M, k = a + 1;
+  const int64_t I = s.I, P = (int64_t)s.A * s.B;
+  const bool raw = flags & kFlagRaw, more = k < R;
+  const TailWs w = tail_ws(M, R);
+  double *wsTT = off(ws, w.tt), *wsYa = off(ws, w.ya), *wsG = off(ws, w.G), *wsg = off(ws, w.g), *wsYd = off(ws, w.yd), *wsC = off(ws, w.c),
+         *wsGy = off(ws, w.Gy);
+  if (more && raw) {
+    int64_t blocks = (P + 255) / 256;
+    if (blocks > 1024) blocks = 1024;
+    Job& d = bd.add(kJobAxpyScalar, 256, (int)blocks, 0, {kBps0, kBcsum, kBmean}, {kBps1}).dev;
+    d.p[0] = s.ps; d.p[1] = s.csum; d.p[2] = const_cast<double*>(s.mean); d.n = P;
+  }
+  if (more && !raw) bd.copy(off(s.Rm, a), R, s.ps, 1, P, kBps0, kBRm);
+  bd.rowdot(s.Y, M, M, I, s.q, s.u, kBY0, kBq, kBu);
+  bd.gram_partials(s.t, 1, 1, s.t, 1, 1, I, wsTT, kBt, kBt, kBwsTT);
+  bd.gram_partials(s.Y, M, M, s.t, 1, 1, I, wsYa, kBY0, kBt, kBwsYa);
+  bd.copy(off(s.T, a), R, s.t, 1, I, kBt, kBT);
+  bd.copy(off(s.Q, a), R, s.q, 1, M, kBq, kBQ);
+  bd.level = 1;
+  if (more && raw) bd.copy(off(s.Rm, a), R, s.ps, 1, P, kBps1, kBRm);
+  bd.copy(off(s.U, a), R, s.u, 1, I, kBu, kBU);
+  bd.gram_reduce(wsTT, 1, 1, off(s.dot_log, 2 * a), kBwsTT, kBdot0);
+  bd.gram_reduce(wsYa, M, 1, s.ya, kBwsYa, kBya);
+  bd.gram_partials(s.T, R, k, s.T, R, k, I, wsG, kBT, kBT, kBwsG);
+  bd.gram_partials(s.T, R, k, s.u, 1, 1, I, wsg, kBT, kBu, kBwsg);
+  bd.level = 2;
+  bd.copy(off(s.dot_log, 2 * a + 1), 1, off(s.dot_log, 2 * a), 1, 1, kBdot0, kBdot1);
+  bd.gram_reduce(wsG, k, k, s.G, kBwsG, kBG);
+  bd.gram_reduce(wsg, k, 1, s.g, kBwsg, kBg);
+  bd.level = 3;
+  {
+    Job& d = bd.add(kJobSolve, 256, 1, kSolveLdsDoubles * sizeof(double), {kBG, kBg}, {kBb}).dev;
+    d.p[0] = s.G; d.p[1] = s.g; d.p[2] = s.b; d.i[0] = k; d.i[1] = 1;
+  }
+  bd.level = 4;
+  bd.copy(off(s.coef, a), R, s.b, 1, k, kBb, kBcoef);
+  {
+    Job& d = bd.add(kJobYDeflate, 256, kJobBlocks, 16 * sizeof(double), {kBY0, kBT, kBb, kBq}, {kBY1}).dev;
+    d.p[0] = s.Y; d.p[1] = s.T; d.p[2] = s.b; d.p[3] = s.q; d.p[4] = wsYd; d.n = I; d.i[0] = M; d.i[1] = M; d.i[2] = R; d.i[3] = k;
+    bd.plan.jobs.back().writes[bd.plan.jobs.back().nw++] = kBwsYd;
+  }
+  if (more) {
+    bd.gram_partials(s.G, k, k, s.b, 1, 1, k, wsC, kBG, kBb, kBwsC);
+    bd.rowdot(s.Rm, R, k, P, s.b, s.vs, kBRm, kBb, kBvs0);
+  }
+  bd.level = 5;
+  {
+    Job& d = bd.add(kJobSum, 1024, 1, 16 * sizeof(double), {kBwsYd}, {kBssq}).dev;
+    d.p[0] = wsYd; d.p[1] = off(s.ssq_log, 2 * a + 1); d.n = kJobBlocks;
+  }
+  if (more) {
+    bd.gram_reduce(wsC, k, 1, s.c, kBwsC, kBc);
+    bd.gram_partials(s.Y, M, M, s.Y, M, M, I, wsGy, kBY1, kBY1, kBwsGy);
+    bd.level = 6;
+    {
+      Job& d = bd.add(kJobKrAxpy, 256, (int)((P + 255) / 256), 64 * sizeof(double), {kBvs0, kBLA, kBLB, kBc}, {kBvs1}).dev;
+      d.p[0] = s.vs; d.p[1] = s.LA; d.p[2] = s.LB; d.p[3] = s.c; d.n = P; d.i[0] = s.B; d.i[1] = R; d.i[2] = k;
+    }
+    bd.gram_reduce(wsGy, M, M, s.Gy, kBwsGy, kBGy);
+    bd.level = 7;
+    {
+      Job& d = bd.add(kJobSDowndate, 256, (int)((P + 255) / 256), 0, {kBS0, kBya, kBwA, kBwB, kBq, kBvs1}, {kBS1}).dev;
+      d.p[0] = s.S; d.p[1] = s.ya; d.p[2] = s.wA; d.p[3] = s.wB; d.p[4] = s.q; d.p[5] = s.vs; d.n = P; d.i[0] = M; d.i[1] = s.B;
+    }
+    bd.level = 8;
+    {
+      Job& d = bd.add(kJobFill, 256, 1, 0, {}, {kBqnext}).dev;
+      d.p[0] = s.q_next; d.n = M; d.i[0] = 1; d.i[1] = 0;
+    }
+  }
+  bd.finish();
+}
+
+static int build(int phase, const cmtfpls_xcov_boundary& s, int a, int flags, double* ws, Plan& plan) {
+  if (phase != 0 && phase != 1) { set_error("xcov_boundary: phase is 0 (head) or 1 (tail)"); return CMTFPLS_EINVAL; }
+  if (!shape_ok(a, s.R, s.M, s.I, s.A, s.B)) { set_error("xcov_boundary: one order-3 block, M <= 64, R <= 64, 0 <= a < R"); return CMTFPLS_EUNSUPPORTED; }
+  if (phase == 1 && a + 1 < s.R && !(flags & kFlagOneRead)) {
+    set_error("xcov_boundary: the tail of a component with a down-date takes the one-read form only");
+    return CMTFPLS_EUNSUPPORTED;
+  }
+  if (phase == 0) build_head(s, a, flags, plan);
+  else build_tail(s, a, flags, ws, plan);
+  return CMTFPLS_OK;
+}
+
+static int plan_only(int phase, int a, int R, int M, int64_t I, int A, int B, int flags, Plan& plan) {
+  cmtfpls_xcov_boundary s{};
+  s.I = I; s.A = A; s.B = B; s.M = M; s.R = R;
+  return build(phase, s, a, flags, nullptr, plan);
+}
+
+static int enqueue(const cmtfpls_xcov_boundary& s, const Plan& plan, hipStream_t st) {
+  for (const Launch& l : plan.launches) {
+    const PlanJob& first = plan.jobs[l.jobs[0]];
+    if (first.kind == kJobScoreS) {
+      const int rc = cmtfpls_score_s_f64(s.mean, 1, s.A, s.B, s.wA, s.wB, s.mw, st);
+      if (rc != CMTFPLS_OK) return rc;
+      continue;
+    }
+    JobTable tab{};
+    size_t lds = 0;
+    int grid = 0;
+    for (size_t j = 0; j < l.jobs.size(); ++j) {
+      const PlanJob& pj = plan.jobs[l.jobs[j]];
+      tab.job[j] = pj.dev;
+      tab.start[j] = grid;
+      grid += pj.blocks;
+      if (pj.lds > lds) lds = pj.lds;
+    }
+    tab.njobs = (int)l.jobs.size();
+    for (int j = tab.njobs; j <= kMaxJobs; ++j) tab.start[j] = grid;
+    if (l.threads == 1024) hipLaunchKernelGGL(job_batch_kernel<1024>, dim3(grid), dim3(1024), lds, st, tab);
+    else hipLaunchKernelGGL(job_batch_kernel<256>, dim3(grid), dim3(256), lds, st, tab);
+  }
+  return check_launch("xcov_boundary");
+}
+
+}
+
+using namespace cmtfpls;
+
+extern "C" {
+
+int cmtfpls_xcov_boundary_launches(int phase, int a, int R, int M, int64_t I, int A, int B, int flags) {
+  Plan plan;
+  if (plan_only(phase, a, R, M, I, A, B, flags, plan) != CMTFPLS_OK) return -1;
+  return (int)plan.launches.size();
+}
+
+int cmtfpls_xcov_boundary_launch_info(int phase, int a, int R, int M, int64_t I, int A, int B, int flags, int launch, int* level, int* threads,
+                                      int* njobs, int* blocks) {
+  Plan plan;
+  const int rc = plan_only(phase, a, R, M, I, A, B, flags, plan);
+  if (rc != CMTFPLS_OK) return rc;
+  if (launch < 0 || launch >= (int)plan.launches.size() || !level || !threads || !njobs || !blocks) {
+    set_error("xcov_boundary_launch_info: bad argument");
+    return CMTFPLS_EINVAL;
+  }
+  const Launch& l = plan.launches[launch];
+  *level = l.level;
+  *threads = l.threads;
+  *njobs = (int)l.jobs.size();
+  *blocks = 0;
+  for (int j : l.jobs) *blocks += plan.jobs[j].blocks;
+  return CMTFPLS_OK;
+}
+
+int cmtfpls_xcov_boundary_job_info(int phase, int a, int R, int M, int64_t I, int A, int B, int flags, int launch, int job, int* kind, int* blocks,
+                                   int* reads, int* n_reads, int* writes, int* n_writes) {
+  Plan plan;
+  const int rc = plan_only(phase, a, R, M, I, A, B, flags, plan);
+  if (rc != CMTFPLS_OK) return rc;
+  if (launch < 0 || launch >= (int)plan.launches.size() || job < 0 || job >= (int)plan.launches[launch].jobs.size() || !kind || !blocks || !reads ||
+      !n_reads || !writes || !n_writes) {
+    set_error("xcov_boundary_job_info: bad argument");
+    return CMTFPLS_EINVAL;
+  }
+  const PlanJob& pj = plan.jobs[plan.launches[launch].jobs[job]];
+  *kind = pj.kind;
+  *blocks = pj.blocks;
+  *n_reads = pj.nr;
+  *n_writes = pj.nw;
+  for (int r = 0; r < pj.nr; ++r) reads[r] = pj.reads[r];
+  for (int w = 0; w < pj.nw; ++w) writes[w] = pj.writes[w];
+  return CMTFPLS_OK;
+}
+
+int cmtfpls_xcov_boundary_buffer_info(int buffer, char* name, size_t n, int* storage, int* version, int* output) {
+  if (buffer < 0 || buffer >= kBufs || !storage || !version || !output) { set_error("xcov_boundary_buffer_info: bad argument"); return CMTFPLS_EINVAL; }
+  if (name && n > 0) {
+    strncpy(name, kBufInfo[buffer].name, n - 1);
+    name[n - 1] = 0;
+  }
+  *storage = kBufInfo[buffer].storage;
+  *version = kBufInfo[buffer].version;
+  *output = kBufInfo[buffer].output;
+  return CMTFPLS_OK;
+}
+
+size_t cmtfpls_xcov_boundary_head_workspace_bytes(int M, int R) {
+  (void)M; (void)R;
+  return 0;
+}
+
+size_t cmtfpls_xcov_boundary_tail_workspace_bytes(int M, int R) {
+  if (M < 1 || M > 64 || R < 1 || R > 64) return 0;
+  return tail_ws(M, R).total * sizeof(double);
+}
+
+int cmtfpls_xcov_boundary_head_f64(const cmtfpls_xcov_boundary* s, int a, int flags, void* ws, size_t ws_bytes, void* stream) {
+  if (!s) { set_error("xcov_boundary_head: bad argument"); return CMTFPLS_EINVAL; }
+  Plan plan;
+  const int rc = build(0, *s, a, flags, nullptr, plan);
+  if (rc != CMTFPLS_OK) return rc;
+  const bool raw = flags & kFlagRaw;
+  if (!s->wA || !s->wB || !s->LA || !s->LB || (raw && (!s->mean || !s->mw)) || (a > 0 && !s->Gw) ||
+      (a > 0 && (flags & kFlagOneRead) && (!s->T || !s->corr))) {
+    set_error("xcov_boundary_head: bad argument");
+    return CMTFPLS_EINVAL;
+  }
+  (void)ws;
+  if (ws_bytes < cmtfpls_xcov_boundary_head_workspace_bytes(s->M, s->R)) { set_error("xcov_boundary_head: workspace too small"); return CMTFPLS_EWORKSPACE; }
+  return enqueue(*s, plan, (hipStream_t)stream);
+}
+
+int cmtfpls_xcov_boundary_tail_f64(const cmtfpls_xcov_boundary* s, int a, int flags, void* ws, size_t ws_bytes, void* stream) {
+  if (!s) { set_error("xcov_boundary_tail: bad argument"); return CMTFPLS_EINVAL; }
+  Plan plan;
+  const int rc = build(1, *s, a, flags, static_cast<double*>(ws), plan);
+  if (rc != CMTFPLS_OK) return rc;
+  const bool raw = flags & kFlagRaw, more = a + 1 < s->R;
+  if (!s->Y || !s->T || !s->U || !s->Q || !s->t || !s->u || !s->q || !s->dot_log || !s->ssq_log || !s->coef || !s->b || !s->G || !s->g || !s->ya ||
+      (more && (!s->ps || !s->Rm || !s->vs || !s->S || !s->c || !s->Gy || !s->q_next || !s->LA || !s->LB || !s->wA || !s->wB)) ||
+      (more && raw && (!s->csum || !s->mean))) {
+    set_error("xcov_boundary_tail: bad argument");
+    return CMTFPLS_EINVAL;
+  }
+  if (!ws || ws_bytes < cmtfpls_xcov_boundary_tail_workspace_bytes(s->M, s->R)) { set_error("xcov_boundary_tail: workspace too small"); return CMTFPLS_EWORKSPACE; }
+  return enqueue(*s, plan, (hipStream_t)stream);
+}
+
+}
diff --git a/cmtf_pls_amd/csrc/small.hip b/cmtf_pls_amd/csrc/small.hip
--- a/cmtf_pls_amd/csrc/small.hip
+++ b/cmtf_pls_amd/csrc/small.hip
@@ -1,4 +1,5 @@
 #include "common.hpp"
+#include "small_jobs.hpp"
 
 namespace cmtfpls {
 
@@ -12,101 +13,26 @@
                                                      const double* __restrict__ B, int ldb, int b,
                                                      int64_t I, double* __restrict__ part, int TR) {
   extern __shared__ double lds[];
-  double* As = lds;
-  double* Bs = lds + TR * a;
-  const int ab = a * b;
-  const int64_t rows_per = (I + gridDim.x - 1) / gridDim.x;
-  const int64_t r0 = (int64_t)blockIdx.x * rows_per;
-  const int64_t r1 = (r0 + rows_per < I) ? r0 + rows_per : I;
-  double acc[16];
-#pragma unroll
-  for (int s = 0; s < 16; ++s) acc[s] = 0.0;
-  for (int64_t rb = r0; rb < r1; rb += TR) {
-    const int nr = (int)((r1 - rb < TR) ? r1 - rb : TR);
-    if (lda == a) {
-      for (int idx = threadIdx.x; idx < nr * a; idx += 256) As[idx] = A[rb * a + idx];
-    } else {
-      for (int idx = threadIdx.x; idx < nr * a; idx += 256) As[idx] = A[(rb + idx / a) * lda + idx % a];
-    }
-    if (ldb == b) {
-      for (int idx = threadIdx.x; idx < nr * b; idx += 256) Bs[idx] = B[rb * b + idx];
-    } else {
-      for (int idx = threadIdx.x; idx < nr * b; idx += 256) Bs[idx] = B[(rb + idx / b) * ldb + idx % b];
-    }
-    __syncthreads();
-#pragma unroll
-    for (int s = 0; s < 16; ++s) {
-      const int o = threadIdx.x + s * 256;
-      if (o < ab) {
-        const int p = o / b, q = o % b;
-        double v = acc[s];
-        for (int r = 0; r < nr; ++r) v = fma(As[r * a + p], Bs[r * b + q], v);
-        acc[s] = v;
-      }
-    }
-    __syncthreads();
-  }
-#pragma unroll
-  for (int s = 0; s < 16; ++s) {
-    const int o = threadIdx.x + s * 256;
-    if (o < ab) part[(int64_t)blockIdx.x * ab + o] = acc[s];
-  }
+  gram_tn_body(blockIdx.x, gridDim.x, A, lda, a, B, ldb, b, I, part, TR, lds);
 }
 
 __global__ __launch_bounds__(256) void reduce_block_kernel(const double* __restrict__ part, int nblk, int ac, int bc,
                                                           double* __restrict__ C, int ldc) {
-  const int o = blockIdx.x * 4 + (threadIdx.x >> 6);
-  const int lane = threadIdx.x & 63;
-  if (o >= ac * bc) return;
-  double s = 0.0;
-  for (int r = lane; r < nblk; r += 64) s += part[(int64_t)r * ac * bc + o];
-  s = wave_sum(s);
-  if (lane == 0) C[(int64_t)(o / bc) * ldc + (o % bc)] = s;
+  reduce_block_body(blockIdx.x, part, nblk, ac, bc, C, ldc);
 }
 
 __global__ __launch_bounds__(256) void gemv_t_kernel(const double* __restrict__ A, int lda, int a0, int ac,
                                                     const double* __restrict__ v, int ldv, int64_t I,
                                                     double* __restrict__ part, int a_total) {
   __shared__ double red[4][16];
-  double acc[16];
-#pragma unroll
-  for (int e = 0; e < 16; ++e) acc[e] = 0.0;
-  for (int64_t i = (int64_t)blockIdx.x * 256 + threadIdx.x; i < I; i += (int64_t)gridDim.x * 256) {
-    const double vi = v[i * ldv];
-    const double* ar = A + i * lda + a0;
-#pragma unroll
-    for (int e = 0; e < 16; ++e)
-      if (e < ac) acc[e] = fma(ar[e], vi, acc[e]);
-  }
-  const int lane = threadIdx.x & 63, wv = threadIdx.x >> 6;
-#pragma unroll
-  for (int e = 0; e < 16; ++e) {
-    const double w = wave_sum(acc[e]);
-    if (lane == 0) red[wv][e] = w;
-  }
-  __syncthreads();
-  if (threadIdx.x < ac) {
-    const int e = threadIdx.x;
-    part[(int64_t)blockIdx.x * a_total + a0 + e] = ((red[0][e] + red[1][e]) + red[2][e]) + red[3][e];
-  }
+  gemv_t_body(blockIdx.x, gridDim.x, A, lda, a0, ac, v, ldv, I, part, a_total, red);
 }
 
 __global__ __launch_bounds__(256) void rowdot_kernel(const double* __restrict__ Y, int ldy, int M, int64_t I,
                                                     const double* __restrict__ q, double* __restrict__ u,
                                                     const double* __restrict__ u_old, double* __restrict__ part) {
   __shared__ double red[16];
-  double d2 = 0.0;
-  for (int64_t i = (int64_t)blockIdx.x * 256 + threadIdx.x; i < I; i += (int64_t)gridDim.x * 256) {
-    const double* yr = Y + i * ldy;
-    double s = 0.0;
-    for (int m = 0; m < M; ++m) s = fma(yr[m], q[m], s);
-    if (u_old) { const double d = u_old[i] - s; d2 = fma(d, d, d2); }
-    u[i] = s;
-  }
-  if (part) {
-    const double s = block_sum(d2, red);
-    if (threadIdx.x == 0) part[blockIdx.x] = s;
-  }
+  rowdot_body(blockIdx.x, gridDim.x, Y, ldy, M, I, q, u, u_old, part, red);
 }
 
 __global__ __launch_bounds__(256) void y_deflate_kernel(double* __restrict__ Y, int ldy, int M, int64_t I,
@@ -114,27 +40,12 @@
                                                        const double* __restrict__ b, const double* __restrict__ q,
                                                        double* __restrict__ part) {
   __shared__ double red[16];
-  double ssq = 0.0;
-  for (int64_t i = (int64_t)blockIdx.x * 256 + threadIdx.x; i < I; i += (int64_t)gridDim.x * 256) {
-    double s = 0.0;
-    for (int r = 0; r < R; ++r) s = fma(T[i * ldt + r], b[r], s);
-    double* yr = Y + i * ldy;
-    for (int m = 0; m < M; ++m) {
-      const double v = yr[m] - s * q[m];
-      yr[m] = v;
-      ssq = fma(v, v, ssq);
-    }
-  }
-  const double s = block_sum(ssq, red);
-  if (threadIdx.x == 0) part[blockIdx.x] = s;
+  y_deflate_body(blockIdx.x, gridDim.x, Y, ldy, M, I, T, ldt, R, b, q, part, red);
 }
 
 __global__ __launch_bounds__(1024) void sum_kernel(const double* __restrict__ in, int64_t n, double* __restrict__ out) {
   __shared__ double red[16];
-  double s = 0.0;
-  for (int64_t i = threadIdx.x; i < n; i += 1024) s += in[i];
-  s = block_sum(s, red);
-  if (threadIdx.x == 0) out[0] = s;
+  sum_body(in, n, out, red);
 }
 
 __global__ __launch_bounds__(1024) void normalize_kernel(double* __restrict__ v, int64_t n, double* __restrict__ nrm) {
@@ -251,16 +162,7 @@
                                                         const double* __restrict__ ya, const double* __restrict__ wA,
                                                         const double* __restrict__ wB, const double* __restrict__ q,
                                                         const double* __restrict__ v) {
-  const int64_t c = (int64_t)blockIdx.x * 256 + threadIdx.x;
-  if (c >= P) return;
-  const double w = wA[c / B] * wB[c % B];
-  const double vc = v[c];
-  for (int m = 0; m < M; ++m) {
-    double sv = S[(int64_t)m * P + c];
-    sv = fma(-ya[m], w, sv);
-    sv = fma(-q[m], vc, sv);
-    S[(int64_t)m * P + c] = sv;
-  }
+  s_downdate_body(blockIdx.x, S, M, P, B, ya, wA, wB, q, v);
 }
 
 __global__ __launch_bounds__(256) void s_contract_kernel(const double* __restrict__ S, int M, int64_t P, const double* __restrict__ q,
@@ -275,22 +177,13 @@
 
 __global__ __launch_bounds__(256) void axpy_scalar_kernel(double* __restrict__ y, int64_t n, const double* __restrict__ a,
                                                          const double* __restrict__ x) {
-  const double av = a[0];
-  for (int64_t i = (int64_t)blockIdx.x * 256 + threadIdx.x; i < n; i += (int64_t)gridDim.x * 256) y[i] = fma(-av, x ? x[i] : 1.0, y[i]);
+  axpy_scalar_body(blockIdx.x, gridDim.x, y, n, a, x);
 }
 
 __global__ __launch_bounds__(256) void kr_axpy_kernel(double* __restrict__ v, int64_t P, int B, const double* __restrict__ WA,
                                                      const double* __restrict__ WB, int ld, int k, const double* __restrict__ coef) {
   __shared__ double cs[64];
-  for (int j = threadIdx.x; j < k; j += 256) cs[j] = coef[j];
-  __syncthreads();
-  const int64_t c = (int64_t)blockIdx.x * 256 + threadIdx.x;
-  if (c >= P) return;
-  const double* __restrict__ wa = WA + (c / B) * ld;
-  const double* __restrict__ wb = WB + (c % B) * ld;
-  double s = 0.0;
-  for (int j = 0; j < k; ++j) s = fma(cs[j] * wa[j], wb[j], s);
-  v[c] -= s;
+  kr_axpy_body(blockIdx.x, v, P, B, WA, WB, ld, k, coef, cs);
 }
 
 __global__ __launch_bounds__(256) void colscale_kernel(double* __restrict__ Z, int64_t P, const double* __restrict__ cnt, double n_samples) {
diff --git a/cmtf_pls_amd/csrc/small_jobs.hpp b/cmtf_pls_amd/csrc/small_jobs.hpp
--- /dev/null
+++ b/cmtf_pls_amd/csrc/small_jobs.hpp
@@ -0,0 +1,248 @@
+#pragma once
+#include "common.hpp"
+
+namespace cmtfpls {
+
+constexpr int kSolveMax = 64;
+constexpr int kSolveLdsDoubles = kSolveMax * (kSolveMax + 1) + 2 * kSolveMax + kSolveMax / 2;
+
+__device__ __forceinline__ void gram_tn_body(int bid, int nblk, const double* __restrict__ A, int lda, int a,
+                                             const double* __restrict__ B, int ldb, int b, int64_t I, double* __restrict__ part, int TR,
+                                             double* lds) {
+  double* As = lds;
+  double* Bs = lds + TR * a;
+  const int ab = a * b;
+  const int64_t rows_per = (I + nblk - 1) / nblk;
+  const int64_t r0 = (int64_t)bid * rows_per;
+  const int64_t r1 = (r0 + rows_per < I) ? r0 + rows_per : I;
+  double acc[16];
+#pragma unroll
+  for (int s = 0; s < 16; ++s) acc[s] = 0.0;
+  for (int64_t rb = r0; rb < r1; rb += TR) {
+    const int nr = (int)((r1 - rb < TR) ? r1 - rb : TR);
+    if (lda == a) {
+      for (int idx = threadIdx.x; idx < nr * a; idx += 256) As[idx] = A[rb * a + idx];
+    } else {
+      for (int idx = threadIdx.x; idx < nr * a; idx += 256) As[idx] = A[(rb + idx / a) * lda + idx % a];
+    }
+    if (ldb == b) {
+      for (int idx = threadIdx.x; idx < nr * b; idx += 256) Bs[idx] = B[rb * b + idx];
+    } else {
+      for (int idx = threadIdx.x; idx < nr * b; idx += 256) Bs[idx] = B[(rb + idx / b) * ldb + idx % b];
+    }
+    __syncthreads();
+#pragma unroll
+    for (int s = 0; s < 16; ++s) {
+      const int o = threadIdx.x + s * 256;
+      if (o < ab) {
+        const int p = o / b, q = o % b;
+        double v = acc[s];
+        for (int r = 0; r < nr; ++r) v = fma(As[r * a + p], Bs[r * b + q], v);
+        acc[s] = v;
+      }
+    }
+    __syncthreads();
+  }
+#pragma unroll
+  for (int s = 0; s < 16; ++s) {
+    const int o = threadIdx.x + s * 256;
+    if (o < ab) part[(int64_t)bid * ab + o] = acc[s];
+  }
+}
+
+__device__ __forceinline__ void reduce_block_body(int bid, const double* __restrict__ part, int nparts, int ac, int bc,
+                                                  double* __restrict__ C, int ldc) {
+  const int o = bid * 4 + (threadIdx.x >> 6);
+  const int lane = threadIdx.x & 63;
+  if (o >= ac * bc) return;
+  double s = 0.0;
+  for (int r = lane; r < nparts; r += 64) s += part[(int64_t)r * ac * bc + o];
+  s = wave_sum(s);
+  if (lane == 0) C[(int64_t)(o / bc) * ldc + (o % bc)] = s;
+}
+
+__device__ __forceinline__ void gemv_t_body(int bid, int nblk, const double* __restrict__ A, int lda, int a0, int ac,
+                                            const double* __restrict__ v, int ldv, int64_t I, double* __restrict__ part, int a_total,
+                                            double (*red)[16]) {
+  double acc[16];
+#pragma unroll
+  for (int e = 0; e < 16; ++e) acc[e] = 0.0;
+  for (int64_t i = (int64_t)bid * 256 + threadIdx.x; i < I; i += (int64_t)nblk * 256) {
+    const double vi = v[i * ldv];
+    const double* ar = A + i * lda + a0;
+#pragma unroll
+    for (int e = 0; e < 16; ++e)
+      if (e < ac) acc[e] = fma(ar[e], vi, acc[e]);
+  }
+  const int lane = threadIdx.x & 63, wv = threadIdx.x >> 6;
+#pragma unroll
+  for (int e = 0; e < 16; ++e) {
+    const double w = wave_sum(acc[e]);
+    if (lane == 0) red[wv][e] = w;
+  }
+  __syncthreads();
+  if (threadIdx.x < ac) {
+    const int e = threadIdx.x;
+    part[(int64_t)bid * a_total + a0 + e] = ((red[0][e] + red[1][e]) + red[2][e]) + red[3][e];
+  }
+}
+
+__device__ __forceinline__ void rowdot_body(int bid, int nblk, const double* __restrict__ Y, int ldy, int M, int64_t I,
+                                            const double* __restrict__ q, double* __restrict__ u, const double* __restrict__ u_old,
+                                            double* __restrict__ part, double* red) {
+  double d2 = 0.0;
+  for (int64_t i = (int64_t)bid * 256 + threadIdx.x; i < I; i += (int64_t)nblk * 256) {
+    const double* yr = Y + i * ldy;
+    double s = 0.0;
+    for (int m = 0; m < M; ++m) s = fma(yr[m], q[m], s);
+    if (u_old) { const double d = u_old[i] - s; d2 = fma(d, d, d2); }
+    u[i] = s;
+  }
+  if (part) {
+    const double s = block_sum(d2, red);
+    if (threadIdx.x == 0) part[bid] = s;
+  }
+}
+
+__device__ __forceinline__ void y_deflate_body(int bid, int nblk, double* __restrict__ Y, int ldy, int M, int64_t I,
+                                               const double* __restrict__ T, int ldt, int R, const double* __restrict__ b,
+                                               const double* __restrict__ q, double* __restrict__ part, double* red) {
+  double ssq = 0.0;
+  for (int64_t i = (int64_t)bid * 256 + threadIdx.x; i < I; i += (int64_t)nblk * 256) {
+    double s = 0.0;
+    for (int r = 0; r < R; ++r) s = fma(T[i * ldt + r], b[r], s);
+    double* yr = Y + i * ldy;
+    for (int m = 0; m < M; ++m) {
+      const double v = yr[m] - s * q[m];
+      yr[m] = v;
+      ssq = fma(v, v, ssq);
+    }
+  }
+  const double s = block_sum(ssq, red);
+  if (threadIdx.x == 0) part[bid] = s;
+}
+
+__device__ __forceinline__ void sum_body(const double* __restrict__ in, int64_t n, double* __restrict__ out, double* red) {
+  double s = 0.0;
+  for (int64_t i = threadIdx.x; i < n; i += 1024) s += in[i];
+  s = block_sum(s, red);
+  if (threadIdx.x == 0) out[0] = s;
+}
+
+__device__ __forceinline__ void s_downdate_body(int bid, double* __restrict__ S, int M, int64_t P, int B, const double* __restrict__ ya,
+                                                const double* __restrict__ wA, const double* __restrict__ wB,
+                                                const double* __restrict__ q, const double* __restrict__ v) {
+  const int64_t c = (int64_t)bid * 256 + threadIdx.x;
+  if (c >= P) return;
+  const double w = wA[c / B] * wB[c % B];
+  const double vc = v[c];
+  for (int m = 0; m < M; ++m) {
+    double sv = S[(int64_t)m * P + c];
+    sv = fma(-ya[m], w, sv);
+    sv = fma(-q[m], vc, sv);
+    S[(int64_t)m * P + c] = sv;
+  }
+}
+
+__device__ __forceinline__ void axpy_scalar_body(int bid, int nblk, double* __restrict__ y, int64_t n, const double* __restrict__ a,
+                                                 const double* __restrict__ x) {
+  const double av = a[0];
+  for (int64_t i = (int64_t)bid * 256 + threadIdx.x; i < n; i += (int64_t)nblk * 256) y[i] = fma(-av, x ? x[i] : 1.0, y[i]);
+}
+
+__device__ __forceinline__ void kr_axpy_body(int bid, double* __restrict__ v, int64_t P, int B, const double* __restrict__ WA,
+                                             const double* __restrict__ WB, int ld, int k, const double* __restrict__ coef, double* cs) {
+  for (int j = threadIdx.x; j < k; j += 256) cs[j] = coef[j];
+  __syncthreads();
+  const int64_t c = (int64_t)bid * 256 + threadIdx.x;
+  if (c >= P) return;
+  const double* __restrict__ wa = WA + (c / B) * ld;
+  const double* __restrict__ wb = WB + (c % B) * ld;
+  double s = 0.0;
+  for (int j = 0; j < k; ++j) s = fma(cs[j] * wa[j], wb[j], s);
+  v[c] -= s;
+}
+
+__device__ __forceinline__ void normal_solve_body(const double* __restrict__ G, const double* __restrict__ g, int k,
+                                                  double* __restrict__ b, int incb, double* lds) {
+  double (*A)[kSolveMax + 1] = reinterpret_cast<double (*)[kSolveMax + 1]>(lds);
+  double* d = lds + kSolveMax * (kSolveMax + 1);
+  double* y = d + kSolveMax;
+  int* dep = reinterpret_cast<int*>(y + kSolveMax);
+  const int i = threadIdx.x;
+  if (i < k) {
+    const double gii = G[(int64_t)i * k + i];
+    d[i] = (gii > 0.0 && isfinite(gii)) ? 1.0 / sqrt(gii) : 0.0;
+    dep[i] = 0;
+  }
+  __syncthreads();
+  if (i < k) {
+    for (int j = 0; j < k; ++j) A[i][j] = G[(int64_t)i * k + j] * d[i] * d[j];
+    y[i] = g[i] * d[i];
+  }
+  __syncthreads();
+  const double tiny = (double)k * 2.220446049250313e-16;
+  for (int c = 0; c < k; ++c) {
+    const double piv = A[c][c];
+    const bool ok = piv > tiny;
+    __syncthreads();
+    if (ok) {
+      const double l = sqrt(piv);
+      if (i == c) A[c][c] = l;
+      if (i > c && i < k) A[i][c] = A[i][c] / l;
+    } else {
+      if (i == c) { A[c][c] = 1.0; dep[c] = 1; }
+      if (i > c && i < k) A[i][c] = 0.0;
+    }
+    __syncthreads();
+    if (ok && i > c && i < k) {
+      const double lic = A[i][c];
+      for (int j = c + 1; j <= i; ++j) A[i][j] -= lic * A[j][c];
+    }
+    __syncthreads();
+  }
+  if (i == 0) {
+    for (int r = 0; r < k; ++r) {
+      double s = y[r];
+      for (int j = 0; j < r; ++j) s -= A[r][j] * y[j];
+      y[r] = dep[r] ? 0.0 : s / A[r][r];
+    }
+    for (int r = k - 1; r >= 0; --r) {
+      double s = y[r];
+      for (int j = r + 1; j < k; ++j) s -= A[j][r] * y[j];
+      y[r] = dep[r] ? 0.0 : s / A[r][r];
+    }
+  }
+  __syncthreads();
+  if (i < k) b[(int64_t)i * incb] = y[i] * d[i];
+}
+
+__device__ __forceinline__ void kr_gram_row_body(const double* __restrict__ L, int n, int R, int a, double* __restrict__ g, int first) {
+  for (int j = threadIdx.x; j < a; j += 256) {
+    double acc = 0.0;
+    int i = 0;
+    for (; i + 16 <= n; i += 16) {
+      double x[16], y[16];
+#pragma unroll
+      for (int u = 0; u < 16; ++u) {
+        x[u] = L[(int64_t)(i + u) * R + j];
+        y[u] = L[(int64_t)(i + u) * R + a];
+      }
+#pragma unroll
+      for (int u = 0; u < 16; ++u) acc = fma(x[u], y[u], acc);
+    }
+    for (; i < n; ++i) acc = fma(L[(int64_t)i * R + j], L[(int64_t)i * R + a], acc);
+    g[j] = (first ? 1.0 : g[j]) * acc;
+  }
+}
+
+__device__ __forceinline__ void copy_strided_body(int bid, int nblk, double* __restrict__ dst, int dstride,
+                                                  const double* __restrict__ src, int sstride, int64_t n) {
+  for (int64_t i = (int64_t)bid * 256 + threadIdx.x; i < n; i += (int64_t)nblk * 256) dst[i * dstride] = src[i * sstride];
+}
+
+__device__ __forceinline__ void fill_unit_body(int bid, int nblk, double* __restrict__ dst, int dstride, int64_t n, int one_at) {
+  for (int64_t i = (int64_t)bid * 256 + threadIdx.x; i < n; i += (int64_t)nblk * 256) dst[i * dstride] = (i == one_at) ? 1.0 : 0.0;
+}
+
+}
diff --git a/cmtf_pls_amd/csrc/solve.hip b/cmtf_pls_amd/csrc/solve.hip
--- a/cmtf_pls_amd/csrc/solve.hip
+++ b/cmtf_pls_amd/csrc/solve.hip
@@ -1,60 +1,12 @@
 #include "common.hpp"
+#include "small_jobs.hpp"
 
 namespace cmtfpls {
 
-constexpr int kSolveMax = 64;
-
 __global__ __launch_bounds__(kSolveMax) void normal_solve_kernel(const double* __restrict__ G, const double* __restrict__ g, int k,
                                                                 double* __restrict__ b, int incb) {
-  __shared__ double A[kSolveMax][kSolveMax + 1];
-  __shared__ double d[kSolveMax], y[kSolveMax];
-  __shared__ int dep[kSolveMax];
-  const int i = threadIdx.x;
-  if (i < k) {
-    const double gii = G[(int64_t)i * k + i];
-    d[i] = (gii > 0.0 && isfinite(gii)) ? 1.0 / sqrt(gii) : 0.0;
-    dep[i] = 0;
-  }
-  __syncthreads();
-  if (i < k) {
-    for (int j = 0; j < k; ++j) A[i][j] = G[(int64_t)i * k + j] * d[i] * d[j];
-    y[i] = g[i] * d[i];
-  }
-  __syncthreads();
-  const double tiny = (double)k * 2.220446049250313e-16;
-  for (int c = 0; c < k; ++c) {
-    const double piv = A[c][c];
-    const bool ok = piv > tiny;
-    __syncthreads();
-    if (ok) {
-      const double l = sqrt(piv);
-      if (i == c) A[c][c] = l;
-      if (i > c && i < k) A[i][c] = A[i][c] / l;
-    } else {
-      if (i == c) { A[c][c] = 1.0; dep[c] = 1; }
-      if (i > c && i < k) A[i][c] = 0.0;
-    }
-    __syncthreads();
-    if (ok && i > c && i < k) {
-      const double lic = A[i][c];
-      for (int j = c + 1; j <= i; ++j) A[i][j] -= lic * A[j][c];
-    }
-    __syncthreads();
-  }
-  if (i == 0) {
-    for (int r = 0; r < k; ++r) {
-      double s = y[r];
-      for (int j = 0; j < r; ++j) s -= A[r][j] * y[j];
-      y[r] = dep[r] ? 0.0 : s / A[r][r];
-    }
-    for (int r = k - 1; r >= 0; --r) {
-      double s = y[r];
-      for (int j = r + 1; j < k; ++j) s -= A[j][r] * y[j];
-      y[r] = dep[r] ? 0.0 : s / A[r][r];
-    }
-  }
-  __syncthreads();
-  if (i < k) b[(int64_t)i * incb] = y[i] * d[i];
+  __shared__ double lds[kSolveLdsDoubles];
+  normal_solve_body(G, g, k, b, incb, lds);
 }
 
 constexpr int kSolveBigMax = 1024;
@@ -147,22 +99,7 @@
 }
 
 __global__ __launch_bounds__(256) void kr_gram_row_kernel(const double* __restrict__ L, int n, int R, int a, double* __restrict__ g, int first) {
-  for (int j = threadIdx.x; j < a; j += 256) {
-    double acc = 0.0;
-    int i = 0;
-    for (; i + 16 <= n; i += 16) {
-      double x[16], y[16];
-#pragma unroll
-      for (int u = 0; u < 16; ++u) {
-        x[u] = L[(int64_t)(i + u) * R + j];
-        y[u] = L[(int64_t)(i + u) * R + a];
-      }
-#pragma unroll
-      for (int u = 0; u < 16; ++u) acc = fma(x[u], y[u], acc);
-    }
-    for (; i < n; ++i) acc = fma(L[(int64_t)i * R + j], L[(int64_t)i * R + a], acc);
-    g[j] = (first ? 1.0 : g[j]) * acc;
-  }
+  kr_gram_row_body(L, n, R, a, g, first);
 }
 
 __global__ __launch_bounds__(256) void khatri_rao_kernel(const double* __restrict__ Am, int na, const double* __restrict__ Bm, int nb,
diff --git a/cmtf_pls_amd/fitrun.py b/cmtf_pls_amd/fitrun.py
--- a/cmtf_pls_amd/fitrun.py
+++ b/cmtf_pls_amd/fitrun.py
@@ -294,10 +294,13 @@
                 be.xcov(self.X2[b], self.Yw, True, out=self.S2[b], mixed=self.mixed)
                 comm.allreduce(self.S2[b])
         self._s_ready = False
+        self._parity = 0
+        self.qc = self.qx[0]
+        if getattr(self, "_next_started", False):
+            self._next_started = False
+            return
         be.gram_tn(self.Y, self.Y, out=self.Gy)
         comm.allreduce(self.Gy)
-        self._parity = 0
-        self.qc = self.qx[0]
         self.qc.zero_()
         self.qc[0] = 1.0
 
@@ -755,6 +758,7 @@
             else:
                 rep["x_passes_per_component"] = "1 read + 1 read + write"
             rep["pipelined"] = bool(getattr(self, "_pipelined", False))
+            rep["native_boundary"] = int(getattr(self, "_nb_done", 0))
             if rep["pipelined"]:
                 rep["pipeline"] = dict(self.pipeline_stats)
             if not rep["pipelined"] and eng.opt.xcov_pipeline:
diff --git a/cmtf_pls_amd/fitrun_xcov.py b/cmtf_pls_amd/fitrun_xcov.py
--- a/cmtf_pls_amd/fitrun_xcov.py
+++ b/cmtf_pls_amd/fitrun_xcov.py
@@ -235,21 +235,63 @@
                 ssqs.append(be.deflate(self.X2[b], blk.A, blk.B, self.t, self.wA[b], self.wB[b]))
         self._log_ssq(a, ssqs, ssqy)
 
+    def _native_boundary(self):
+        if getattr(self, "_nb_off", False):
+            return None
+        call = getattr(self, "_nb_call", None)
+        if call is not None:
+            return call
+        be, blk = self.eng.be, self.blocks[0]
+        if not (self.eng.opt.xcov_native_boundary and hasattr(be, "xcov_boundary")):
+            self._nb_off = True
+            return None
+        if not (len(self.blocks) == 1 and len(blk.shape) == 3 and not blk.has_miss and not self.eng.comm.sharded and self.M <= 64
+                and self.R <= 64 and self.t.data_ptr() == self.Ts.data_ptr() and self.Y.is_contiguous()
+                and self.Y.dtype == torch.float64 and self.S[0].is_contiguous()):
+            return self._native_boundary_off("one order-3 block, unsharded, at most 64 responses and components")
+        R, M = self.R, self.M
+        own = self._nb_bufs = {"mw": be.empty(1), "G": be.empty(R * R), "g": be.empty(R), "ya": be.empty(M), "c": be.empty(R)}
+        bufs = dict(own, Y=self.Y, T=self.T, U=self.U, Q=self.Q, LA=blk.loadings[0], LB=blk.loadings[1], wA=self.wA[0], wB=self.wB[0],
+                    t=self.t, u=self.u, q_next=self.qx[0], Gw=self.Gw, vs=self.vs[0], S=self.S[0], dot_log=self.dot_log,
+                    ssq_log=self.ssq_log, coef=self.coef_dev, b=self.b_dev, Gy=self.Gy)
+        if self.raw:
+            bufs["mean"] = blk.mean
+        if hasattr(self, "ps"):
+            bufs.update(ps=self.ps, Rm=self.Rm, corr=self.corr, csum=self.csum)
+        self._nb_done = 0
+        self._nb_call = be.xcov_boundary(self.I, blk.A, blk.B, M, R, **bufs)
+        return self._nb_call
+
+    def _native_boundary_off(self, why: str) -> None:
+        self._nb_off = True
+        self._nb_call = None
+        self.notes.append("native component boundary declined: " + why)
+        return None
+
     def _finish_xcov_nowrite(self, a: int) -> None:
         be, comm = self.eng.be, self.eng.comm
         self.q = self.qc
         I, R, k = self.I, self.R, a + 1
         nb = len(self.blocks)
-        self._store_loadings(a)
         fused_b = self._fused_b if (getattr(self, "_one_read", False) and k < R) else -1
+        native = self._native_boundary()
+        head = native is not None and native(0, a, self.raw, fused_b >= 0) is not None
+        if native is not None and not head:
+            native = self._native_boundary_off("the library declined the shape")
+        if not head:
+            self._store_loadings(a)
         one_read = False
         for b in [x for x in range(nb) if x != fused_b] + ([fused_b] if fused_b >= 0 else []):
             blk = self.blocks[b]
             mw = None
-            if self.raw:
+            if self.raw and head:
+                mw = self._nb_bufs["mw"]
+            elif self.raw:
                 mw = be.score_s(blk.mean.view(1, -1), blk.A, blk.B, self.wA[b], self.wB[b], be.empty(1))
             g = None
-            if a > 0 and hasattr(be, "kr_gram_row"):
+            if a > 0 and head:
+                g = self.Gw[:a]
+            elif a > 0 and hasattr(be, "kr_gram_row"):
                 for m, L in enumerate(blk.loadings):
                     be.kr_gram_row(L, a, self.Gw, first=(m == 0))
                 g = self.Gw[:a]
@@ -260,7 +302,8 @@
             if b == fused_b:
                 corr = others = None
                 if a > 0:
-                    be.rowdot(self.T[:, :a], g, self.corr, None)
+                    if not head:
+                        be.rowdot(self.T[:, :a], g, self.corr, None)
                     corr = self.corr
                 if nb == 2:
                     others = self.Ts[1 - b]
@@ -282,6 +325,17 @@
         single = self.t.data_ptr() == self.Ts.data_ptr()
         if not single:
             be.scores_mean(self.Ts, self.t)
+        if native is not None and k < R and not one_read:
+            native = self._native_boundary_off("the component took the two-read form (one read switched off, or score_contract declined "
+                                                 "the shape): its down-date sits behind a second pass over X")
+        if native is not None:
+            if native(1, a, self.raw, one_read, q=self.q) is not None:
+                self._nb_done += 1
+                if k < R:
+                    self._s_ready = True
+                    self._next_started = True
+                return
+            self._native_boundary_off("the library declined the shape")
         if one_read:
             comm.allreduce(self.ps)
             if self.raw:
diff --git a/cmtf_pls_amd/options.py b/cmtf_pls_amd/options.py
--- a/cmtf_pls_amd/options.py
+++ b/cmtf_pls_amd/options.py
@@ -18,6 +18,7 @@
     xcov_stats_with_s: bool = True
     xcov_deflate_build: bool = True
     xcov_pipeline: bool = True
+    xcov_native_boundary: bool = True
     capture_collectives: bool = False
     project_split_rows: bool = True
     masked_folds: bool = False
diff --git a/include/cmtfpls.h b/include/cmtfpls.h
--- a/include/cmtfpls.h
+++ b/include/cmtfpls.h
@@ -180,6 +180,30 @@
                           const double* b, const double* q, double* ssq, void* ws, size_t ws_bytes,
                           void* stream);
 int cmtfpls_sum_f64(const double* in, int64_t n, double* out, void* stream);
+
+#define CMTFPLS_XCOV_BOUNDARY_RAW 1
+#define CMTFPLS_XCOV_BOUNDARY_ONE_READ 2
+typedef struct cmtfpls_xcov_boundary {
+  int64_t I;
+  int A, B, M, R;
+  double *Y, *T, *U, *Q, *LA, *LB;
+  double *wA, *wB, *t, *u, *q, *q_next;
+  const double* mean;
+  double *mw, *Gw, *corr;
+  double *ps, *csum, *Rm, *vs, *S;
+  double *dot_log, *ssq_log, *coef, *b;
+  double *G, *g, *ya, *c, *Gy;
+} cmtfpls_xcov_boundary;
+int cmtfpls_xcov_boundary_launches(int phase, int a, int R, int M, int64_t I, int A, int B, int flags);
+int cmtfpls_xcov_boundary_launch_info(int phase, int a, int R, int M, int64_t I, int A, int B, int flags, int launch, int* level,
+                                      int* threads, int* njobs, int* blocks);
+int cmtfpls_xcov_boundary_job_info(int phase, int a, int R, int M, int64_t I, int A, int B, int flags, int launch, int job, int* kind,
+                                   int* blocks, int* reads, int* n_reads, int* writes, int* n_writes);
+int cmtfpls_xcov_boundary_buffer_info(int buffer, char* name, size_t n, int* storage, int* version, int* output);
+size_t cmtfpls_xcov_boundary_head_workspace_bytes(int M, int R);
+size_t cmtfpls_xcov_boundary_tail_workspace_bytes(int M, int R);
+int cmtfpls_xcov_boundary_head_f64(const cmtfpls_xcov_boundary* s, int a, int flags, void* ws, size_t ws_bytes, void* stream);
+int cmtfpls_xcov_boundary_tail_f64(const cmtfpls_xcov_boundary* s, int a, int flags, void* ws, size_t ws_bytes, void* stream);
 
 int cmtfpls_project_rows_f32(const float* X, int64_t I, int A, int B, int R, const double* WA, const double* WB,
                              const double* mean, double* scores, int ld, void* stream);
```

After: 758.8. Within noise of the previous version (-0.1%).
